# nubot-nudt/LCR-Net

Hardware: AMD Instinct MI355X
Metric: scans/s (120k-pt KITTI-shape scan -> 256-D descriptor) (higher is better)
Workload: dtype f32 (K-deep GEMMs, K >= 288 and N >= 64: fp32 operands as bf16 x 3 split, 6 of 9 products on the bf16 matrix cores, fp32 accumulate — error vs fp64 <= the fp32-MFMA kernel's; every other GEMM, KPConv and attention: fp32 MFMA); 1 GPU; configs[1]: batch of 8 synthetic 64-beam scans (~120k pts, 0.3 m voxel -> ~16k pts), voxelise + 3 subsamples + 10 radius searches + KPConv encoder + NetVLAD, seeded random weights; distinct_input_batches=4, streams=pre-processing stream (own host thread, 2 batches ahead) + 2 encoder stream(s), parallelism=scan-parallel x1, all-gather of descriptors

## Files before the change

include/lcr_hip.h:

```cpp
#ifndef LCR_HIP_H
#define LCR_HIP_H
#include <stddef.h>
#include <stdint.h>
#ifdef __cplusplus
extern "C" {
#endif

#define LCR_OK 0
#define LCR_EARG (-1)
#define LCR_ESPACE (-2)
#define LCR_EHIP (-3)

#define LCR_STATUS_KEY_OVERFLOW 1u
#define LCR_STATUS_LEN_MISMATCH 2u
#define LCR_GN_REPLICAS 8

const char* lcr_last_error(void);
void lcr_ktimer_enable(int on);
void lcr_ktimer_sample(int every);
void lcr_ktimer_kinds(unsigned mask);
int lcr_ktimer_read(int kind, int max_records, double* seconds, int64_t* meta);
int lcr_ktimer_read2(int kind, int max_records, double* seconds, double* seconds_kernel, int64_t* meta);
int lcr_stream_spin(int microseconds, void* stream);
int lcr_version(void);

int lcr_grid_subsample_ws_bytes(int64_t n_cap, int B, size_t* bytes);
int lcr_grid_subsample(const float* xyz, const int64_t* len, int B, int64_t n_cap, float voxel,
                       float* out_xyz, int64_t* out_len, uint32_t* status,
                       void* ws, size_t ws_bytes, void* stream);
int lcr_grid_subsample_ex(const float* xyz, const int64_t* len, int B, int64_t n_cap, float voxel, int key_bits_hint,
                          float* out_xyz, int64_t* out_len, uint32_t* status,
                          void* ws, size_t ws_bytes, void* stream);
int lcr_grid_subsample_rows(const float* xyz, int row_floats, const int64_t* len, int B, int64_t n_cap, float voxel, int key_bits_hint,
                            float* out_xyz, int64_t* out_len, uint32_t* status,
                            void* ws, size_t ws_bytes, void* stream);
int lcr_hashmap_order_host(const uint64_t* keys_host, int64_t n, int64_t* order_host);

int lcr_support_grid_ws_bytes(int64_t ns_cap, int B, size_t* bytes);
int lcr_support_grid_build(const float* s, const int64_t* slen, int B, int64_t ns_cap, float radius,
                           uint32_t* status, void* grid_ws, size_t grid_ws_bytes, void* stream);
int lcr_radius_query(const float* q, const int64_t* qlen, int B, int64_t nq_cap,
                     const void* grid_ws, int64_t ns_cap , float radius, int limit,
                     int64_t* out_idx64, int32_t* out_idx32, int32_t* out_cnt, void* stream);
int lcr_radius_query_ordered(const float* q, const int64_t* qlen, int B, int64_t nq_cap,
                             const void* grid_ws, int64_t ns_cap, float radius, int limit,
                             int64_t* out_idx64, int32_t* out_idx32, int32_t* out_cnt, const int32_t* q_order, void* stream);
typedef struct LcrRadiusQuery {
    const float*   q;
    const int64_t* qlen;
    int64_t        nq_cap;
    const void*    grid_ws;
    int64_t        ns_cap;
    float          radius;
    int            limit;
    int32_t*       out_idx32;
    const int32_t* q_order;
} LcrRadiusQuery;
#define LCR_RADIUS_QUERY_MULTI_MAX 12
int lcr_radius_query_multi(const LcrRadiusQuery* list, int n, int B, void* stream);
int lcr_support_grid_build_ex(const float* s, const int64_t* slen, int B, int64_t ns_cap, float radius,
                              uint32_t* status, void* grid_ws, size_t grid_ws_bytes, int32_t* order, void* stream);
int lcr_support_grid_order(const void* grid_ws, int64_t ns_cap, int B, int32_t* order, void* stream);
int lcr_radius_search_ws_bytes(int64_t nq_cap, int64_t ns_cap, int B, size_t* bytes);
int lcr_radius_search(const float* q, const float* s, const int64_t* qlen, const int64_t* slen, int B,
                      int64_t nq_cap, int64_t ns_cap, float radius, int limit,
                      int64_t* out_idx64, int32_t* out_idx32, int32_t* out_cnt, uint32_t* status,
                      void* ws, size_t ws_bytes, void* stream);

#define LCR_MAX_STAGES 8
typedef struct LcrPrecomputeLayout {
  int     num_stages, B, upsampling;
  int64_t n_raw;
  int     limits[LCR_MAX_STAGES];
  int64_t cap[LCR_MAX_STAGES];
  size_t  off_points[LCR_MAX_STAGES];
  size_t  off_lengths[LCR_MAX_STAGES];
  size_t  off_order[LCR_MAX_STAGES];
  size_t  off_neighbors[LCR_MAX_STAGES];
  size_t  off_subsampling[LCR_MAX_STAGES];
  size_t  off_upsampling[LCR_MAX_STAGES];
  size_t  out_bytes, ws_bytes;
} LcrPrecomputeLayout;
int lcr_precompute_layout(int64_t n0, int B, int num_stages, const int* limits, int upsampling, int64_t n_raw,
                          LcrPrecomputeLayout* layout);
int lcr_precompute_batch(const float* points0, const int64_t* lengths0, const LcrPrecomputeLayout* layout, float voxel_size,
                         float radius, float raw_voxel, int key_bits_hint, void* out, size_t out_bytes, void* ws, size_t ws_bytes,
                         int64_t* lengths_host, uint32_t* status_host, void* stream);
int lcr_precompute_batch_rows(const float* points0, int raw_row_floats, const int64_t* lengths0, const LcrPrecomputeLayout* layout,
                              float voxel_size, float radius, float raw_voxel, int key_bits_hint, void* out, size_t out_bytes, void* ws,
                              size_t ws_bytes, int64_t* lengths_host, uint32_t* status_host, void* stream);

int lcr_gemm_f32(const float* A, const float* B, float* C, int64_t M, int N, int K, int transA, int transB,
                 const float* bias, const float* rowdiv, const int64_t* seg_len, int S, int groups, double* stats,
                 void* stream);
int lcr_split_bf16x3(const float* w, int64_t n, uint16_t* planes, void* stream);
int lcr_split_bf16x3_tiles(const float* w, int N, int K, uint16_t* tiles, void* stream);
int lcr_gemm_f32_bsplit(const float* A, const uint16_t* Bs_tiles, float* C, int64_t M, int N, int K, const float* bias, const float* rowdiv,
                        const int64_t* seg_len, int S, int groups, double* stats, void* stream);
int lcr_gemm_f32_anorm(const float* A, const float* B, float* C, int64_t M, int N, int K, const float* bias,
                       const double* a_stats, const float* a_gamma, const float* a_beta, int a_groups, float a_eps,
                       float a_slope, const int64_t* seg_len, int S, int groups, double* stats, void* stream);
int lcr_gemm_f32_batched_ta(const float* A, const float* B, float* C, int64_t M, int N, int count, const int* k_host,
                            const int64_t* a_off_host, const int64_t* b_off_host, const int64_t* c_off_host, void* stream);
int lcr_kpconv_aggregate(const float* s_feats, const uint8_t* s_pos, const float* q_pts, const float* s_pts,
                         const void* idx, int idx_is_64, int64_t M, int64_t Ns, int H, int C,
                         const float* kernel_points_host, float sigma, float* A, float* nn,
                         const int32_t* order , void* stream);
#define LCR_KP_VALID_FIRST 1
int lcr_kpconv_aggregate_ex(const float* s_feats, const uint8_t* s_pos, const float* q_pts, const float* s_pts,
                            const void* idx, int idx_is_64, int64_t M, int64_t Ns, int H, int C,
                            const float* kernel_points_host, float sigma, float* A, float* nn,
                            const int32_t* order, int flags, void* stream);
int lcr_kpconv_fused(const float* s_feats, const uint8_t* s_pos, const float* q_pts, const float* s_pts, const void* idx,
                     int idx_is_64, int64_t M, int64_t Ns, int H, int C, const float* kernel_points_host, float sigma,
                     const float* W, const float* bias, float* out, const int64_t* seg_len, int S, int groups, double* stats,
                     const int32_t* order, void* stream);
int lcr_kpconv_cin1(const float* s_feats, const float* q_pts, const float* s_pts, const void* idx, int idx_is_64,
                    int64_t M, int64_t Ns, int H, const float* kernel_points_host, float sigma, const float* W,
                    const float* bias, int Cout, float* out, const int32_t* order, void* stream);
int lcr_maxpool(const float* x, const void* idx, int idx_is_64, int64_t M, int64_t Ns, int H, int C, float* out,
                const int32_t* order, void* stream);
int lcr_row_positive(const float* x, int64_t N, int C, uint8_t* pos, void* stream);
int lcr_groupnorm_stats(const float* x, int64_t N, int C, int groups, const int64_t* seg_len, int S, double* stats, void* stream);
int lcr_groupnorm_apply(const float* x, const double* stats, const float* gamma, const float* beta, const float* res,
                        const double* res_stats, const float* res_gamma, const float* res_beta, float* y, int64_t N, int C,
                        int groups, const int64_t* seg_len, int S, float eps, float slope, int act, uint8_t* pos, void* stream);

#define LCR_ENC_BLOCKS 10
typedef struct LcrUnaryW {
  const float *w, *b;
  const float *gn_w, *gn_b;
  const uint16_t* w_split;
} LcrUnaryW;
typedef struct LcrBlockW {
  int   cin, cout, strided;
  float sigma;
  const float* kernel_points_host;
  const float *kp_w, *kp_b;
  const float* kp_wt;
  const uint16_t* kp_wt_split;
  const float *normconv_w, *normconv_b;
  LcrUnaryW unary1, unary2, shortcut;
} LcrBlockW;
typedef struct LcrEncoderW {
  int   groups, c1_cout;
  float c1_sigma;
  const float* c1_kernel_points_host;
  const float *c1_w, *c1_b;
  const float *c1_gn_w, *c1_gn_b;
  LcrBlockW blocks[LCR_ENC_BLOCKS];
} LcrEncoderW;
int lcr_encoder_ws_bytes(const LcrEncoderW* W, const int64_t* n_host, int S, size_t* bytes);
int lcr_encoder_forward(const LcrEncoderW* W, const float* feats0, const float* const* points, const int32_t* const* neighbors,
                        const int32_t* const* subsampling, const int32_t* const* order, const int64_t* const* seg_len, int S,
                        const int64_t* n_host, const int64_t* seg_min_rows_host, const int* limits, float* const* out_feats, void* ws,
                        size_t ws_bytes, void* stream);
#define LCR_ENC_LISTS_VALID_FIRST 1u
int lcr_encoder_forward_ex(const LcrEncoderW* W, const float* feats0, const float* const* points, const int32_t* const* neighbors,
                           const int32_t* const* subsampling, const int32_t* const* order, const int64_t* const* seg_len, int S,
                           const int64_t* n_host, const int64_t* seg_min_rows_host, const int* limits, float* const* out_feats,
                           unsigned flags, void* ws, size_t ws_bytes, void* stream);

typedef struct LcrNetvladWeights {
  const float* cluster_weights;
  const float* cluster_weights2;
  const float* hidden1_weights;
  const float *bn1_w, *bn1_b, *bn1_mean, *bn1_var;
  const float *bn2_w, *bn2_b, *bn2_mean, *bn2_var;
  const float* gating_weights;
  const float *gbn_w, *gbn_b, *gbn_mean, *gbn_var;
} LcrNetvladWeights;
int lcr_netvlad_ws_bytes(int64_t n_rows, int S, size_t* bytes);
int lcr_netvlad_forward(const float* feats , const int64_t* seg_len_host, int S,
                        const LcrNetvladWeights* weights_host, float* out , void* ws, size_t ws_bytes, void* stream);

int lcr_rotary_embed(float* x, const float* theta, int64_t N, int heads, void* stream);
int lcr_attention_f32(const float* q, const float* k, const float* v, int64_t Nq, int64_t Nk, int heads, int head_dim,
                      float* out, void* stream);
int lcr_attention_seg_f32(const float* q, const float* k, const float* v, const int64_t* q_len_host, const int64_t* k_len_host, int P,
                          int heads, int head_dim, float* out, void* stream);
int lcr_attention_topk_f32(const float* q, const float* k, const float* v, const int64_t* q_len_host, const int64_t* k_len_host,
                           const int* kk_host, int P, int heads, int head_dim, float* out, void* stream);
int lcr_add_layernorm(const float* a, const float* b, const float* gamma, const float* beta, int64_t N, int D, float eps,
                      float* y, void* stream);
int lcr_relu_inplace(float* x, int64_t n, void* stream);

#define LCR_ROFORMER_MAX_BLOCKS 16
typedef struct LcrLinearW {
  const float *w, *b;
} LcrLinearW;
typedef struct LcrRoformerLayerW {
  LcrLinearW   q, k, v, lin;
  const float *ln1_w, *ln1_b;
  float        ln1_eps;
  LcrLinearW   expand, squeeze;
  const float *ln2_w, *ln2_b;
  float        ln2_eps;
} LcrRoformerLayerW;
typedef struct LcrRoformerW {
  int        d_in, d_model, d_out, heads, num_blocks;
  int        block_is_self[LCR_ROFORMER_MAX_BLOCKS];
  LcrLinearW emb1, emb2, in_proj, out_proj;
  LcrRoformerLayerW layers[LCR_ROFORMER_MAX_BLOCKS];
} LcrRoformerW;
int lcr_roformer_ws_bytes(const LcrRoformerW* W, int64_t n_rows, size_t* bytes);
int lcr_roformer_forward(const LcrRoformerW* W, const float* points, const float* feats, const int64_t* lens0_host, const int64_t* lens1_host,
                         int P, float* out, float* theta_out, void* ws, size_t ws_bytes, void* stream);

int lcr_retrieval_ws_bytes(int64_t Q, int64_t C, size_t* bytes);
int lcr_retrieval_topk(const float* queries , int64_t Q, int64_t q0, const float* database , int64_t C,
                       int D, int k, int exclude, int32_t* out_idx , float* out_d2 ,
                       void* ws, size_t ws_bytes, void* stream);

int lcr_gemm_f32_strided_batched(const float* A, const float* B, float* C, int64_t M, int N, int K, int transA, int transB,
                                 int64_t strideA, int64_t strideB, int64_t strideC, int count, void* stream);

int lcr_vote_shift(const float* xyz, const float* offsets, int64_t N, float max_range, float* out, void* stream);
int lcr_greedy_nms_ws_bytes(int64_t n_total, size_t* bytes);
int lcr_greedy_nms(const float* pts, const int64_t* len, int B, int64_t n_total, float radius, uint8_t* keep,
                   int64_t* out_len, void* ws, void* stream);
int lcr_neighbor_mean(const float* pts, const void* idx, int idx_is_64, int64_t M, int H, int64_t pad, float* out, void* stream);
int lcr_point_to_node_ws_bytes(int64_t N, int M, size_t* bytes);
int lcr_point_to_node_partition(const float* points, int64_t N, const float* nodes, int M, int K, int32_t* p2n, int64_t* knn,
                                uint8_t* knn_mask, uint8_t* node_mask, uint32_t* status, void* ws, size_t ws_bytes, void* stream);

int lcr_point_to_node_partition_stack(const float* points, const int64_t* point_off, const float* nodes, const int64_t* node_off, int C, int K,
                                      int32_t* p2n_out, int64_t* knn, uint8_t* knn_mask, uint8_t* node_mask, uint32_t* status, void* ws,
                                      size_t ws_bytes, void* stream);
int lcr_build_padded_scores(const float* raw, const uint8_t* row_mask, const uint8_t* col_mask, int64_t B, int M, int N,
                            float scale, const float* alpha, float inf_val, float* S, void* stream);
int lcr_log_sinkhorn(float* S, const uint8_t* row_mask, const uint8_t* col_mask, int64_t B, int M, int N, int iters,
                     float inf_val, float* uv_ws, void* stream);
int lcr_log_sinkhorn_ws_floats(int64_t B, int M, int N, size_t* floats);
int lcr_log_sinkhorn_form(int64_t B, int M, int N, int* form);
int lcr_log_sinkhorn_ex(float* S, const uint8_t* row_mask, const uint8_t* col_mask, int64_t B, int M, int N, int iters,
                        float inf_val, float* uv_ws, size_t uv_floats, void* stream);
int lcr_top1_matching_ws_bytes(int64_t B, int M, int N, size_t* bytes);
int lcr_top1_matching(const float* logS, int64_t B, int M, int N, const uint8_t* row_mask, const uint8_t* col_mask,
                      int64_t* total, int32_t* out_bij, float* out_score, void* ws, size_t ws_bytes, void* stream);
int lcr_top1_matching_ex(const float* logS, int64_t B, int M, int N, const uint8_t* row_mask, const uint8_t* col_mask, int mutual,
                         int64_t* total, int32_t* out_bij, float* out_score, void* ws, size_t ws_bytes, void* stream);
int lcr_patch_scores(const float* feats_a, int64_t Na, const float* feats_b, int64_t Nb, int C, const int64_t* idx_a, const int64_t* idx_b,
                     const uint8_t* mask_a, const uint8_t* mask_b, int64_t P, int K, float scale, const float* alpha, float inf_val, float* S,
                     void* stream);
int lcr_topk_matching_ws_bytes(int64_t B, int M, int N, size_t* bytes);
int lcr_topk_matching(const float* logS, int64_t B, int M, int N, const uint8_t* row_mask, const uint8_t* col_mask, int K, int mutual,
                      int64_t* total, int32_t* out_bij, float* out_score, void* ws, size_t ws_bytes, void* stream);
int lcr_topk_matching_ex(const float* logS, int64_t B, int M, int N, const uint8_t* row_mask, const uint8_t* col_mask, int K, int mutual,
                         int use_dustbin, float confidence_threshold, const float* global_scores, int64_t* total, int32_t* out_bij,
                         float* out_score, void* ws, size_t ws_bytes, void* stream);
int lcr_upsample_concat(const float* x, int64_t Nx, int C1, const void* idx, int idx_is_64, int H, const float* skip, int C2,
                        int64_t N, float* out, void* stream);
int lcr_gather_rows(const float* src, int64_t pad, int C, const int64_t* idx, int64_t R, float* out, void* stream);
int lcr_procrustes_batched(const float* src, const float* ref, const float* w, const int32_t* start, int P, float eps, float* T, void* stream);
int lcr_inlier_count(const float* T, int P, const float* src, const float* ref, int n, float radius, const int32_t* start,
                     int min_count, int32_t* counts, int32_t* best, void* stream);
int lcr_lgr_ws_bytes(int64_t n, int H, int S, size_t* bytes);
int lcr_local_global_registration(const float* src, const float* ref, const float* score, int64_t n, const int32_t* hyp_start, int H,
                                  const int32_t* seg_hyp_start, int S, float radius, int min_count, int steps, float* T_out,
                                  float* hyp_out, int32_t* counts_out, int32_t* best_out, void* ws, size_t ws_bytes, void* stream);
int lcr_local_global_registration_ex(const float* src, const float* ref, const float* score, int64_t n, const int32_t* hyp_start, int H,
                                     const int32_t* seg_hyp_start, int S, float radius, int min_count, int steps, int correspondence_limit,
                                     float* T_out, float* hyp_out, int32_t* counts_out, int32_t* best_out, void* ws, size_t ws_bytes,
                                     void* stream);
int lcr_inlier_weights(const float* T_all, const int32_t* sel, const float* src, const float* ref, const float* score, int n,
// ... 19 lines not shown
```

lcr-net_amd/_lib.py:

```python
import ctypes
import os

import torch

_PKG = os.path.dirname(os.path.abspath(__file__))
LIB_PATH = os.path.join(_PKG, "liblcr_hip.so")

_lib = None

c_f32p = ctypes.c_void_p
c_vp = ctypes.c_void_p
c_i64 = ctypes.c_int64
c_int = ctypes.c_int
c_float = ctypes.c_float
c_size_p = ctypes.POINTER(ctypes.c_size_t)
c_size_t = ctypes.c_size_t

_SIGS = {
    "lcr_last_error": (ctypes.c_char_p, []),
    "lcr_version": (c_int, []),
    "lcr_support_grid_ws_bytes": (c_int, [c_i64, c_int, c_size_p]),
    "lcr_support_grid_build": (c_int, [c_vp, c_vp, c_int, c_i64, c_float, c_vp, c_vp, ctypes.c_size_t, c_vp]),
    "lcr_precompute_layout": (c_int, [c_i64, c_int, c_int, c_vp, c_int, c_i64, c_vp]),
    "lcr_precompute_batch": (c_int, [c_vp, c_vp, c_vp, c_float, c_float, c_float, c_int, c_vp, c_size_t, c_vp, c_size_t, c_vp, c_vp, c_vp]),
    "lcr_precompute_batch_rows": (c_int, [c_vp, c_int, c_vp, c_vp, c_float, c_float, c_float, c_int, c_vp, c_size_t, c_vp, c_size_t, c_vp, c_vp, c_vp]),
    "lcr_radius_query_multi": (c_int, [c_vp, c_int, c_int, c_vp]),
    "lcr_radius_query": (c_int, [c_vp, c_vp, c_int, c_i64, c_vp, c_i64, c_float, c_int, c_vp, c_vp, c_vp, c_vp]),
    "lcr_stream_spin": (c_int, [c_int, c_vp]),
    "lcr_radius_query_ordered": (c_int, [c_vp, c_vp, c_int, c_i64, c_vp, c_i64, c_float, c_int, c_vp, c_vp, c_vp, c_vp, c_vp]),
    "lcr_radius_search_ws_bytes": (c_int, [c_i64, c_i64, c_int, c_size_p]),
    "lcr_radius_search": (c_int, [c_vp, c_vp, c_vp, c_vp, c_int, c_i64, c_i64, c_float, c_int, c_vp, c_vp, c_vp, c_vp,
                                  c_vp, ctypes.c_size_t, c_vp]),
    "lcr_grid_subsample_ws_bytes": (c_int, [c_i64, c_int, c_size_p]),
    "lcr_grid_subsample": (c_int, [c_vp, c_vp, c_int, c_i64, c_float, c_vp, c_vp, c_vp, c_vp, ctypes.c_size_t, c_vp]),
    "lcr_grid_subsample_ex": (c_int, [c_vp, c_vp, c_int, c_i64, c_float, c_int, c_vp, c_vp, c_vp, c_vp, ctypes.c_size_t, c_vp]),
    "lcr_grid_subsample_rows": (c_int, [c_vp, c_int, c_vp, c_int, c_i64, c_float, c_int, c_vp, c_vp, c_vp, c_vp, ctypes.c_size_t, c_vp]),
    "lcr_hashmap_order_host": (c_int, [c_vp, c_i64, c_vp]),
    "lcr_gemm_f32": (c_int, [c_vp, c_vp, c_vp, c_i64, c_int, c_int, c_int, c_int, c_vp, c_vp, c_vp, c_int, c_int, c_vp, c_vp]),
    "lcr_gemm_f32_anorm": (c_int, [c_vp, c_vp, c_vp, c_i64, c_int, c_int, c_vp, c_vp, c_vp, c_vp, c_int, c_float, c_float, c_vp, c_int,
                                   c_int, c_vp, c_vp]),
    "lcr_ktimer_enable": (None, [c_int]),
    "lcr_ktimer_sample": (None, [c_int]),
    "lcr_ktimer_kinds": (None, [ctypes.c_uint]),
    "lcr_ktimer_read": (c_int, [c_int, c_int, c_vp, c_vp]),
    "lcr_ktimer_read2": (c_int, [c_int, c_int, c_vp, c_vp, c_vp]),
    "lcr_encoder_ws_bytes": (c_int, [c_vp, c_vp, c_int, c_size_p]),
    "lcr_encoder_forward": (c_int, [c_vp, c_vp, c_vp, c_vp, c_vp, c_vp, c_vp, c_int, c_vp, c_vp, c_vp, c_vp, c_vp, c_size_t, c_vp]),
    "lcr_roformer_ws_bytes": (c_int, [c_vp, c_i64, c_size_p]),
    "lcr_roformer_forward": (c_int, [c_vp, c_vp, c_vp, c_vp, c_vp, c_int, c_vp, c_vp, c_vp, c_size_t, c_vp]),
    "lcr_encoder_forward_ex": (c_int, [c_vp, c_vp, c_vp, c_vp, c_vp, c_vp, c_vp, c_int, c_vp, c_vp, c_vp, c_vp, ctypes.c_uint, c_vp, c_size_t, c_vp]),
    "lcr_kpconv_aggregate": (c_int, [c_vp, c_vp, c_vp, c_vp, c_vp, c_int, c_i64, c_i64, c_int, c_int, c_vp, c_float, c_vp, c_vp, c_vp, c_vp]),
    "lcr_kpconv_fused": (c_int, [c_vp, c_vp, c_vp, c_vp, c_vp, c_int, c_i64, c_i64, c_int, c_int, c_vp, c_float, c_vp, c_vp, c_vp, c_vp, c_int,
                                 c_int, c_vp, c_vp, c_vp]),
    "lcr_kpconv_cin1": (c_int, [c_vp, c_vp, c_vp, c_vp, c_int, c_i64, c_i64, c_int, c_vp, c_float, c_vp, c_vp, c_int, c_vp, c_vp, c_vp]),
    "lcr_maxpool": (c_int, [c_vp, c_vp, c_int, c_i64, c_i64, c_int, c_int, c_vp, c_vp, c_vp]),
    "lcr_support_grid_order": (c_int, [c_vp, c_i64, c_int, c_vp, c_vp]),
    "lcr_row_positive": (c_int, [c_vp, c_i64, c_int, c_vp, c_vp]),
    "lcr_groupnorm_stats": (c_int, [c_vp, c_i64, c_int, c_int, c_vp, c_int, c_vp, c_vp]),
    "lcr_groupnorm_apply": (c_int, [c_vp, c_vp, c_vp, c_vp, c_vp, c_vp, c_vp, c_vp, c_vp, c_i64, c_int, c_int, c_vp, c_int,
                                    c_float, c_float, c_int, c_vp, c_vp]),
    "lcr_rotary_embed": (c_int, [c_vp, c_vp, c_i64, c_int, c_vp]),
    "lcr_attention_f32": (c_int, [c_vp, c_vp, c_vp, c_i64, c_i64, c_int, c_int, c_vp, c_vp]),
    "lcr_attention_seg_f32": (c_int, [c_vp, c_vp, c_vp, c_vp, c_vp, c_int, c_int, c_int, c_vp, c_vp]),
    "lcr_attention_topk_f32": (c_int, [c_vp, c_vp, c_vp, c_vp, c_vp, c_vp, c_int, c_int, c_int, c_vp, c_vp]),
    "lcr_add_layernorm": (c_int, [c_vp, c_vp, c_vp, c_vp, c_i64, c_int, c_float, c_vp, c_vp]),
    "lcr_relu_inplace": (c_int, [c_vp, c_i64, c_vp]),
    "lcr_retrieval_ws_bytes": (c_int, [c_i64, c_i64, c_size_p]),
    "lcr_retrieval_topk": (c_int, [c_vp, c_i64, c_i64, c_vp, c_i64, c_int, c_int, c_int, c_vp, c_vp, c_vp, ctypes.c_size_t, c_vp]),
    "lcr_gemm_f32_strided_batched": (c_int, [c_vp, c_vp, c_vp, c_i64, c_int, c_int, c_int, c_int, c_i64, c_i64, c_i64, c_int, c_vp]),
    "lcr_vote_shift": (c_int, [c_vp, c_vp, c_i64, c_float, c_vp, c_vp]),
    "lcr_greedy_nms_ws_bytes": (c_int, [c_i64, c_size_p]),
    "lcr_greedy_nms": (c_int, [c_vp, c_vp, c_int, c_i64, c_float, c_vp, c_vp, c_vp, c_vp]),
    "lcr_neighbor_mean": (c_int, [c_vp, c_vp, c_int, c_i64, c_int, c_i64, c_vp, c_vp]),
    "lcr_point_to_node_ws_bytes": (c_int, [c_i64, c_int, c_size_p]),
    "lcr_point_to_node_partition": (c_int, [c_vp, c_i64, c_vp, c_int, c_int, c_vp, c_vp, c_vp, c_vp, c_vp, c_vp, ctypes.c_size_t, c_vp]),
    "lcr_point_to_node_partition_stack": (c_int, [c_vp, c_vp, c_vp, c_vp, c_int, c_int, c_vp, c_vp, c_vp, c_vp, c_vp, c_vp, ctypes.c_size_t, c_vp]),
    "lcr_build_padded_scores": (c_int, [c_vp, c_vp, c_vp, c_i64, c_int, c_int, c_float, c_vp, c_float, c_vp, c_vp]),
    "lcr_log_sinkhorn": (c_int, [c_vp, c_vp, c_vp, c_i64, c_int, c_int, c_int, c_float, c_vp, c_vp]),
    "lcr_log_sinkhorn_ws_floats": (c_int, [c_i64, c_int, c_int, c_size_p]),
    "lcr_log_sinkhorn_form": (c_int, [c_i64, c_int, c_int, ctypes.POINTER(c_int)]),
    "lcr_split_bf16x3": (c_int, [c_vp, c_i64, c_vp, c_vp]),
    "lcr_split_bf16x3_tiles": (c_int, [c_vp, c_int, c_int, c_vp, c_vp]),
    "lcr_gemm_f32_bsplit": (c_int, [c_vp, c_vp, c_vp, c_i64, c_int, c_int, c_vp, c_vp, c_vp, c_int, c_int, c_vp, c_vp]),
    "lcr_log_sinkhorn_ex": (c_int, [c_vp, c_vp, c_vp, c_i64, c_int, c_int, c_int, c_float, c_vp, ctypes.c_size_t, c_vp]),
    "lcr_top1_matching_ws_bytes": (c_int, [c_i64, c_int, c_int, c_size_p]),
    "lcr_top1_matching": (c_int, [c_vp, c_i64, c_int, c_int, c_vp, c_vp, c_vp, c_vp, c_vp, c_vp, ctypes.c_size_t, c_vp]),
    "lcr_top1_matching_ex": (c_int, [c_vp, c_i64, c_int, c_int, c_vp, c_vp, c_int, c_vp, c_vp, c_vp, c_vp, ctypes.c_size_t, c_vp]),
    "lcr_topk_matching_ws_bytes": (c_int, [c_i64, c_int, c_int, c_size_p]),
    "lcr_topk_matching": (c_int, [c_vp, c_i64, c_int, c_int, c_vp, c_vp, c_int, c_int, c_vp, c_vp, c_vp, c_vp, ctypes.c_size_t, c_vp]),
    "lcr_patch_scores": (c_int, [c_vp, c_i64, c_vp, c_i64, c_int, c_vp, c_vp, c_vp, c_vp, c_i64, c_int, c_float, c_vp, c_float, c_vp, c_vp]),
    "lcr_topk_matching_ex": (c_int, [c_vp, c_i64, c_int, c_int, c_vp, c_vp, c_int, c_int, c_int, c_float, c_vp, c_vp, c_vp, c_vp, c_vp, ctypes.c_size_t,
                                     c_vp]),
    "lcr_local_global_registration_ex": (c_int, [c_vp, c_vp, c_vp, c_i64, c_vp, c_int, c_vp, c_int, c_float, c_int, c_int, c_int, c_vp, c_vp, c_vp, c_vp,
                                                 c_vp, ctypes.c_size_t, c_vp]),
    "lcr_upsample_concat": (c_int, [c_vp, c_i64, c_int, c_vp, c_int, c_int, c_vp, c_int, c_i64, c_vp, c_vp]),
    "lcr_gather_rows": (c_int, [c_vp, c_i64, c_int, c_vp, c_i64, c_vp, c_vp]),
    "lcr_procrustes_batched": (c_int, [c_vp, c_vp, c_vp, c_vp, c_int, c_float, c_vp, c_vp]),
    "lcr_inlier_count": (c_int, [c_vp, c_int, c_vp, c_vp, c_int, c_float, c_vp, c_int, c_vp, c_vp, c_vp]),
    "lcr_inlier_weights": (c_int, [c_vp, c_vp, c_vp, c_vp, c_vp, c_int, c_float, c_vp, c_vp]),
    "lcr_lgr_ws_bytes": (c_int, [c_i64, c_int, c_int, c_size_p]),
    "lcr_local_global_registration": (c_int, [c_vp, c_vp, c_vp, c_i64, c_vp, c_int, c_vp, c_int, c_float, c_int, c_int, c_vp, c_vp, c_vp, c_vp, c_vp,
                                              ctypes.c_size_t, c_vp]),
    "lcr_netvlad_ws_bytes": (c_int, [c_i64, c_int, c_size_p]),
    "lcr_netvlad_forward": (c_int, [c_vp, c_vp, c_int, c_vp, c_vp, c_vp, ctypes.c_size_t, c_vp]),
    "lcr_ransac_ws_bytes": (c_int, [c_int, c_int, c_size_p]),
    "lcr_ransac_correspondences": (c_int, [c_vp, c_vp, c_vp, c_int, c_float, c_int, c_int, ctypes.c_uint64, c_vp, c_vp, c_vp, c_vp, c_vp, c_vp, c_vp,
                                           c_vp, ctypes.c_size_t, c_vp]),
    "lcr_ransac_sample_host": (c_int, [ctypes.c_uint64, c_i64, c_i64, c_int, c_i64, c_vp]),
    "lcr_icp_ws_bytes": (c_int, [c_int, c_i64, c_i64, c_size_p]),
    "lcr_icp_point_to_point": (c_int, [c_vp, c_vp, c_vp, c_vp, c_int, c_vp, c_float, c_int, ctypes.c_double, ctypes.c_double, c_vp, c_vp, c_vp, c_vp,
                                       c_vp, c_vp, c_vp, c_vp, c_int, c_vp, ctypes.c_size_t, c_vp]),
}


_RELEASES_GIL = {"lcr_roformer_forward", "lcr_precompute_batch", "lcr_precompute_batch_rows", "lcr_encoder_forward", "lcr_encoder_forward_ex", "lcr_ktimer_read",
                 "lcr_ktimer_read2", "lcr_hashmap_order_host", "lcr_ransac_sample_host", "lcr_icp_point_to_point", "lcr_netvlad_forward", "lcr_log_sinkhorn", "lcr_log_sinkhorn_ex",
                 "lcr_local_global_registration", "lcr_local_global_registration_ex", "lcr_retrieval_topk", "lcr_stream_spin"}


def build():
    import importlib.util
    spec = importlib.util.spec_from_file_location("_lcr_build", os.path.join(_PKG, "csrc", "build.py"))
    mod = importlib.util.module_from_spec(spec)
    spec.loader.exec_module(mod)
    return mod.build()


def lib():
    global _lib
    if _lib is None:
        if not os.path.exists(LIB_PATH):
            raise RuntimeError(
                "liblcr_hip.so not found at %s — build it with `python lcr-net_amd/csrc/build.py` "
                "(there is no CPU fallback for the lcr-net_amd hot path)" % LIB_PATH)
        L = ctypes.CDLL(LIB_PATH)
        for name, (res, args) in _SIGS.items():
            if not hasattr(L, name):
                continue
            fn = getattr(L, name)
            fn.restype = res
            fn.argtypes = args
        if os.environ.get("LCR_CTYPES_KEEP_GIL", "1") != "0":
            K = ctypes.PyDLL(LIB_PATH)
            for name, (res, args) in _SIGS.items():
                if name in _RELEASES_GIL or not hasattr(K, name):
                    continue
                fn = getattr(K, name)
                fn.restype = res
                fn.argtypes = args
                setattr(L, name, fn)
        _lib = L
    return _lib


def check(rc, what):
    if rc != 0:
        msg = lib().lcr_last_error()
        raise RuntimeError("%s failed (rc=%d): %s" % (what, rc, msg.decode() if msg else ""))


def ptr(t):
    return ctypes.c_void_p(t.data_ptr()) if t is not None else ctypes.c_void_p(0)


def stream_ptr(device=None):
    idx = device.index if isinstance(device, torch.device) else None
    if idx is None:
        idx = torch.cuda.current_device() if not isinstance(device, int) else device
    return ctypes.c_void_p(torch._C._cuda_getCurrentRawStream(idx))


def require_cuda(*tensors):
    for t in tensors:
        if t is not None and not t.is_cuda:
            raise RuntimeError("lcr-net_amd ops run on the GPU only: got a %s tensor (no CPU fallback)" % t.device)


def workspace(nbytes, device):
    return torch.empty(max(int(nbytes), 256), dtype=torch.uint8, device=device)
```

lcr-net_amd/csrc/encoder.hip:

```cpp
#include <algorithm>
#include <cstdlib>
#include <cstring>

#include "common.h"

#define TURN(call) ([&]() { LaunchTurn turn_; return (call); }())

namespace lcr {

constexpr float ENC_GN_EPS = 1e-5f;
constexpr float ENC_SLOPE = 0.1f;

struct Arena {
  char*  base;
  size_t off, cap;
  template <typename T>
  T* take(size_t n) {
    const size_t o = off;
    off = align_up(off + n * sizeof(T));
    return (base && off <= cap) ? reinterpret_cast<T*>(base + o) : nullptr;
  }
};

struct StageIO {
  const float*   pts;
  const int64_t* seg;
  const int32_t* order;
  int64_t        n;
  int64_t        min_rows;
};

struct StatsPool {
  double* base;
  size_t  off, cap;
  int     S, groups;
  double* take() {
    const size_t n = static_cast<size_t>(GN_REPLICAS) * S * groups * 2;
    if (off + n > cap) return nullptr;
    double* p = base + off;
    off += n;
    return p;
  }
};

static size_t stats_doubles(int S, int groups) { return static_cast<size_t>(GN_REPLICAS) * S * groups * 2 * 44; }

static int unary_raw(const LcrUnaryW& u, const float* x, int64_t n, int cin, int cout, const StageIO& st, StatsPool& sp, Arena& ws,
                     float** y_out, double** stats_out, hipStream_t s) {
  float* y = ws.take<float>(static_cast<size_t>(n) * cout);
  double* stats = sp.take();
  if (!y || !stats) return LCR_ESPACE;
  const bool split = u.w_split && cin >= 288 && cin % 32 == 0 && cout >= 64;
  int rc = split ? TURN(lcr_gemm_f32_bsplit(x, u.w_split, y, n, cout, cin, u.b, nullptr, st.seg, sp.S, sp.groups, stats, s))
                 : TURN(lcr_gemm_f32(x, u.w, y, n, cout, cin, 0, 1, u.b, nullptr, st.seg, sp.S, sp.groups, stats, s));
  *y_out = y;
  *stats_out = stats;
  return rc;
}

static int residual_block(const LcrBlockW& b, const float* s_feats, const StageIO& q, const StageIO& sup, const void* idx, int H,
                          StatsPool& sp, Arena& ws, float* out, unsigned enc_flags, hipStream_t s) {
  const int mid = b.cout / 4, g = sp.groups;
  const int64_t M = q.n, Ns = sup.n;
  int rc;
  const float* x = s_feats;
  uint8_t* pos = ws.take<uint8_t>(static_cast<size_t>(Ns));
  if (!pos) return LCR_ESPACE;
  if (b.unary1.w) {
    float* y1;
    double* st1;
    if ((rc = unary_raw(b.unary1, s_feats, Ns, b.cin, mid, sup, sp, ws, &y1, &st1, s))) return rc;
    float* x1 = ws.take<float>(static_cast<size_t>(Ns) * mid);
    if (!x1) return LCR_ESPACE;
    if ((rc = TURN(lcr_groupnorm_apply(y1, st1, b.unary1.gn_w, b.unary1.gn_b, nullptr, nullptr, nullptr, nullptr, x1, Ns, mid, g, sup.seg, sp.S,
                                  ENC_GN_EPS, ENC_SLOPE, 1, pos, s))))
      return rc;
    x = x1;
  } else if ((rc = TURN(lcr_row_positive(s_feats, Ns, b.cin, pos, s)))) {
    return rc;
  }
  float* A = ws.take<float>(static_cast<size_t>(M) * 15 * mid);
  float* nn = ws.take<float>(static_cast<size_t>(M));
  float* kpo = ws.take<float>(static_cast<size_t>(M) * mid);
  double* stc = sp.take();
  if (!A || !nn || !kpo || !stc) return LCR_ESPACE;
  static const bool vf_env_off = getenv("LCR_KP_VALID_FIRST") && atoi(getenv("LCR_KP_VALID_FIRST")) == 0;
  const int vf_flag = ((enc_flags & LCR_ENC_LISTS_VALID_FIRST) && !vf_env_off) ? LCR_KP_VALID_FIRST : 0;
  static const bool fused32 = getenv("LCR_KPCONV_FUSED") != nullptr;
  if (fused32 && mid == 32 && sp.S <= 64) {
    if ((rc = TURN(lcr_kpconv_fused(x, pos, q.pts, sup.pts, idx, 0, M, Ns, H, mid, b.kernel_points_host, b.sigma, b.kp_w, b.kp_b, kpo, q.seg, sp.S, g,
                                    stc, q.order, s))))
      return rc;
  } else {
    if ((rc = TURN(lcr_kpconv_aggregate_ex(x, pos, q.pts, sup.pts, idx, 0, M, Ns, H, mid, b.kernel_points_host, b.sigma, A, nn, q.order, vf_flag, s)))) return rc;
    if (b.kp_wt_split && mid >= 64) {
      if ((rc = TURN(lcr_gemm_f32_bsplit(A, b.kp_wt_split, kpo, M, mid, 15 * mid, b.kp_b, nn, q.seg, sp.S, g, stc, s)))) return rc;
    } else if ((rc = TURN(b.kp_wt ? lcr_gemm_f32(A, b.kp_wt, kpo, M, mid, 15 * mid, 0, 1, b.kp_b, nn, q.seg, sp.S, g, stc, s)
                                  : lcr_gemm_f32(A, b.kp_w, kpo, M, mid, 15 * mid, 0, 0, b.kp_b, nn, q.seg, sp.S, g, stc, s)))) return rc;
  }
  float* y;
  double* sty;
  static const bool no_anorm = getenv("LCR_NO_NORM_ON_LOAD") != nullptr;
  if (!no_anorm && mid <= 256 && mid % 4 == 0 && b.cout > 32 && q.min_rows >= 64) {
    y = ws.take<float>(static_cast<size_t>(M) * b.cout);
    sty = sp.take();
    if (!y || !sty) return LCR_ESPACE;
    if ((rc = TURN(lcr_gemm_f32_anorm(kpo, b.unary2.w, y, M, b.cout, mid, b.unary2.b, stc, b.normconv_w, b.normconv_b, g, ENC_GN_EPS, ENC_SLOPE,
                                      q.seg, sp.S, g, sty, s))))
      return rc;
  } else {
    float* x2 = ws.take<float>(static_cast<size_t>(M) * mid);
    if (!x2) return LCR_ESPACE;
    if ((rc = TURN(lcr_groupnorm_apply(kpo, stc, b.normconv_w, b.normconv_b, nullptr, nullptr, nullptr, nullptr, x2, M, mid, g, q.seg, sp.S, ENC_GN_EPS,
                                  ENC_SLOPE, 1, nullptr, s))))
      return rc;
    if ((rc = unary_raw(b.unary2, x2, M, mid, b.cout, q, sp, ws, &y, &sty, s))) return rc;
  }
  const float* res = s_feats;
  if (b.strided) {
    float* pooled = ws.take<float>(static_cast<size_t>(M) * b.cin);
    if (!pooled) return LCR_ESPACE;
    if ((rc = TURN(lcr_maxpool(s_feats, idx, 0, M, Ns, H, b.cin, pooled, q.order, s)))) return rc;
    res = pooled;
  }
  const double* str = nullptr;
  if (b.shortcut.w) {
    float* r;
    double* st;
    if ((rc = unary_raw(b.shortcut, res, M, b.cin, b.cout, q, sp, ws, &r, &st, s))) return rc;
    res = r;
    str = st;
  }
  return TURN(lcr_groupnorm_apply(y, sty, b.unary2.gn_w, b.unary2.gn_b, res, str, str ? b.shortcut.gn_w : nullptr, str ? b.shortcut.gn_b : nullptr, out,
                             M, b.cout, g, q.seg, sp.S, ENC_GN_EPS, ENC_SLOPE, 1, nullptr, s));
}

static size_t block_ws_bytes(const LcrBlockW& b, int64_t M, int64_t Ns) {
  Arena a{nullptr, 0, ~size_t(0)};
  const int mid = b.cout / 4;
  a.take<uint8_t>(Ns);
  a.take<float>(static_cast<size_t>(Ns) * mid);
  a.take<float>(static_cast<size_t>(Ns) * mid);
  a.take<float>(static_cast<size_t>(M) * 15 * mid);
  a.take<float>(M);
  a.take<float>(static_cast<size_t>(M) * mid);
  a.take<float>(static_cast<size_t>(M) * mid);
  a.take<float>(static_cast<size_t>(M) * b.cout);
  a.take<float>(static_cast<size_t>(M) * b.cin);
  a.take<float>(static_cast<size_t>(M) * b.cout);
  return a.off;
}

static const int BLOCK_Q[LCR_ENC_BLOCKS] = {0, 1, 1, 1, 2, 2, 2, 3, 3, 3};
static const int BLOCK_S[LCR_ENC_BLOCKS] = {0, 0, 1, 1, 1, 2, 2, 2, 3, 3};

}

using namespace lcr;

extern "C" int lcr_encoder_ws_bytes(const LcrEncoderW* W, const int64_t* n_host, int S, size_t* bytes) {
  if (!W || !n_host || !bytes || S < 1) return LCR_EARG;
  size_t blk = 0, pp = 0;
  for (int i = 0; i < LCR_ENC_BLOCKS; ++i) {
    blk = std::max(blk, block_ws_bytes(W->blocks[i], n_host[BLOCK_Q[i]], n_host[BLOCK_S[i]]));
    pp = std::max(pp, align_up(sizeof(float) * static_cast<size_t>(n_host[BLOCK_Q[i]]) * W->blocks[i].cout));
  }
  pp = std::max(pp, align_up(sizeof(float) * static_cast<size_t>(n_host[0]) * W->c1_cout * 2));
  *bytes = blk + 2 * pp + align_up(sizeof(double) * stats_doubles(S, W->groups)) + 4096;
  return LCR_OK;
}

extern "C" int lcr_encoder_forward(const LcrEncoderW* W, const float* feats0, const float* const* points, const int32_t* const* neighbors,
                                   const int32_t* const* subsampling, const int32_t* const* order, const int64_t* const* seg_len, int S,
                                   const int64_t* n_host, const int64_t* seg_min_rows_host, const int* limits, float* const* out_feats,
                                   void* ws, size_t ws_bytes, void* stream) {
  return lcr_encoder_forward_ex(W, feats0, points, neighbors, subsampling, order, seg_len, S, n_host, seg_min_rows_host, limits, out_feats, 0u, ws,
                                ws_bytes, stream);
}

extern "C" int lcr_encoder_forward_ex(const LcrEncoderW* W, const float* feats0, const float* const* points, const int32_t* const* neighbors,
                                      const int32_t* const* subsampling, const int32_t* const* order, const int64_t* const* seg_len, int S,
                                      const int64_t* n_host, const int64_t* seg_min_rows_host, const int* limits, float* const* out_feats,
                                      unsigned flags, void* ws, size_t ws_bytes, void* stream) {
  if (!W || !feats0 || !points || !neighbors || !subsampling || !seg_len || !n_host || !limits || !out_feats || !ws || S < 1) {
    set_error("lcr_encoder_forward: bad argument");
    return LCR_EARG;
  }
  size_t need = 0;
  lcr_encoder_ws_bytes(W, n_host, S, &need);
  if (ws_bytes < need) {
    set_error("lcr_encoder_forward: workspace too small (%zu < %zu)", ws_bytes, need);
    return LCR_ESPACE;
  }
  hipStream_t s = static_cast<hipStream_t>(stream);
  StageIO st[4];
  for (int i = 0; i < 4; ++i) st[i] = StageIO{points[i], seg_len[i], order ? order[i] : nullptr, n_host[i], seg_min_rows_host ? seg_min_rows_host[i] : 0};
  Arena top{static_cast<char*>(ws), 0, ws_bytes};
  StatsPool sp{top.take<double>(stats_doubles(S, W->groups)), 0, stats_doubles(S, W->groups), S, W->groups};
  size_t pp = 0;
  for (int i = 0; i < LCR_ENC_BLOCKS; ++i) pp = std::max(pp, sizeof(float) * static_cast<size_t>(n_host[BLOCK_Q[i]]) * W->blocks[i].cout);
  pp = std::max(pp, sizeof(float) * static_cast<size_t>(n_host[0]) * W->c1_cout * 2);
  float* ping = reinterpret_cast<float*>(top.take<char>(pp));
  float* pong = reinterpret_cast<float*>(top.take<char>(pp));
  const size_t scratch0 = top.off;
  if (!sp.base || !ping || !pong) return LCR_ESPACE;
  hipMemsetAsync(sp.base, 0, sizeof(double) * sp.cap, s);

  int rc;
  float* cur;
  {
    const int64_t n0 = n_host[0];
    float* raw = ping;
    float* f = ping + static_cast<size_t>(n0) * W->c1_cout;
    double* stt = sp.take();
    if ((rc = TURN(lcr_kpconv_cin1(feats0, st[0].pts, st[0].pts, neighbors[0], 0, n0, n0, limits[0], W->c1_kernel_points_host, W->c1_sigma, W->c1_w,
                              W->c1_b, W->c1_cout, raw, st[0].order, s))))
      return rc;
    if ((rc = TURN(lcr_groupnorm_stats(raw, n0, W->c1_cout, W->groups, st[0].seg, S, stt, s)))) return rc;
    if ((rc = TURN(lcr_groupnorm_apply(raw, stt, W->c1_gn_w, W->c1_gn_b, nullptr, nullptr, nullptr, nullptr, f, n0, W->c1_cout, W->groups, st[0].seg, S,
                                  ENC_GN_EPS, ENC_SLOPE, 1, nullptr, s))))
      return rc;
    cur = f;
  }
  static const int STAGE_LAST[4] = {0, 3, 6, 9};
  for (int i = 0; i < LCR_ENC_BLOCKS; ++i) {
    const int qs = BLOCK_Q[i], ss = BLOCK_S[i];
    const bool strided = qs != ss;
    const void* idx = strided ? static_cast<const void*>(subsampling[ss]) : static_cast<const void*>(neighbors[qs]);
    const int H = limits[ss];
    float* out = nullptr;
    for (int k = 0; k < 4; ++k)
      if (STAGE_LAST[k] == i) out = out_feats[k];
    if (!out) out = (cur >= ping && cur < ping + pp / sizeof(float)) ? pong : ping;
    Arena scratch{static_cast<char*>(ws), scratch0, ws_bytes};
    if ((rc = residual_block(W->blocks[i], cur, st[qs], st[ss], idx, H, sp, scratch, out, flags, s))) {
      if (rc == LCR_ESPACE) set_error("lcr_encoder_forward: block %d ran out of workspace", i);
      return rc;
    }
    cur = out;
  }
  return check_launch("lcr_encoder_forward");
}
```

lcr-net_amd/csrc/gemm_f32.hip:

```cpp
#include <cstdio>
#include <cstdlib>
#include <map>
#include <mutex>
#include <type_traits>

#include "common.h"

namespace lcr {

typedef float floatx16 __attribute__((ext_vector_type(16)));

constexpr int GM_BK = 32;
constexpr int GM_T = 256;

constexpr int GM_MAX_BATCH = 64;
struct GemmBatch {
  int     count;
  int     strided;
  int     k[GM_MAX_BATCH];
  int64_t a_off[GM_MAX_BATCH], b_off[GM_MAX_BATCH], c_off[GM_MAX_BATCH];
};

struct GemmEpilogue {
  const float*   bias;
// ... 411 lines not shown
    lb_t[0].store(Bs[0]);
  } else {
    sstore(0, 0);
  }
  __syncthreads();
  const int half = lane >> 5;
  const int a_off = ARM ? (wm * 32 + (lane & 31)) * LDR + half * 16 : half * (NEWP ? 16 : 1) * LDA + wm * 32 + (lane & 31);
  const int b_off = BRM ? (wn * (32 * NT) + (lane & 31)) * LDR + half * 16 : half * (NEWP ? 16 : 1) * LDB + wn * (32 * NT) + (lane & 31);
  auto fetch4_a = [&](const float* as, int q, float (&o)[4]) {
    if (ARM) {
      const float4 v = *reinterpret_cast<const float4*>(as + 4 * q);
      o[0] = v.x, o[1] = v.y, o[2] = v.z, o[3] = v.w;
    } else {
#pragma unroll
      for (int i = 0; i < 4; ++i) o[i] = as[(4 * q + i) * LDA];
    }
  };
  auto fetch4_b = [&](const float* bs, int q, float (&o)[4]) {
    if (BRM) {
      const float4 v = *reinterpret_cast<const float4*>(bs + 4 * q);
      o[0] = v.x, o[1] = v.y, o[2] = v.z, o[3] = v.w;
    } else {
#pragma unroll
      for (int i = 0; i < 4; ++i) o[i] = bs[(4 * q + i) * LDB];
    }
  };
  if constexpr (SHORT) {
    constexpr int KKS = GM_BK / 2, PFS = 4;
    for (int t = 0; t < nk; ++t) {
      if (t > 0) {
        gload(k_begin + t * GM_BK, 0);
        __syncthreads();
        if constexpr (ANORM) {
          sstore_a0();
          lb_t[0].store(Bs[0]);
        } else {
          sstore(0, 0);
        }
        __syncthreads();
      }
      const float* as = As[0] + a_off;
      const float* bs = Bs[0] + b_off;
      static_assert(NEWP, "the light form is only instantiated for single-accumulator tiles");
      float af[2][4], bf[2][4];
      fetch4_a(as, 0, af[0]);
      fetch4_b(bs, 0, bf[0]);
      fetch4_a(as, 1, af[1]);
      fetch4_b(bs, 1, bf[1]);
#pragma unroll
      for (int q = 0; q < KKS / 4; ++q) {
#pragma unroll
        for (int i = 0; i < 4; ++i) acc[0] = __builtin_amdgcn_mfma_f32_32x32x2f32(af[q & 1][i], bf[q & 1][i], acc[0], 0, 0, 0);
        if (q + 2 < KKS / 4) {
          fetch4_a(as, q + 2, af[q & 1]);
          fetch4_b(bs, q + 2, bf[q & 1]);
        }
      }
    }
  } else {
  constexpr int KK = GM_BK / 2;
  constexpr int PF = NT == 1 ? KK : (NT == 2 ? 8 : 4);
  constexpr int PA = BM * 8 / GM_T, PB = BN * 8 / GM_T;
  constexpr int ST0 = KK - (PA + PB) - 1 > 2 ? (KK - (PA + PB)) / 2 : 1;
  auto step = [&](auto buf_c, auto full_c, int t) {
    constexpr int BUF = decltype(buf_c)::value;
    constexpr bool FULL = decltype(full_c)::value;
    if (FULL || t + 2 < nk) gload(k_begin + (t + 2) * GM_BK, BUF);
    const bool do_store = FULL || t + 1 < nk;
    const float* as = As[BUF] + a_off;
    const float* bs = Bs[BUF] + b_off;
    float af[PF], bf[PF][NT];
    if constexpr (NEWP) {
#pragma unroll
      for (int q = 0; q < KK / 4; ++q) {
        float a4[4], b4[4];
        fetch4_a(as, q, a4);
        fetch4_b(bs, q, b4);
#pragma unroll
        for (int i = 0; i < 4; ++i) {
          af[4 * q + i] = a4[i];
          bf[4 * q + i][0] = b4[i];
        }
      }
    } else {
#pragma unroll
      for (int d = 0; d < PF; ++d) {
        af[d] = as[d * 2 * LDA];
#pragma unroll
        for (int j = 0; j < NT; ++j) bf[d][j] = bs[d * 2 * LDB + j * 32];
      }
    }
    __builtin_amdgcn_sched_barrier(0);
#pragma unroll
    for (int kk = 0; kk < KK; ++kk) {
      const int sl = kk % PF;
#pragma unroll
      for (int j = 0; j < NT; ++j) {
        if (NACC == 2 && (kk & 1)) acc2[j] = __builtin_amdgcn_mfma_f32_32x32x2f32(af[sl], bf[sl][j], acc2[j], 0, 0, 0);
        else acc[j] = __builtin_amdgcn_mfma_f32_32x32x2f32(af[sl], bf[sl][j], acc[j], 0, 0, 0);
      }
      if (kk + PF < KK) {
        af[sl] = as[(kk + PF) * 2 * LDA];
#pragma unroll
        for (int j = 0; j < NT; ++j) bf[sl][j] = bs[(kk + PF) * 2 * LDB + j * 32];
      }
      const int piece = kk - ST0;
      if (do_store && piece >= 0 && piece < PA + PB) {
        if (piece < PA) {
          if (TA) la_n[1 - BUF].store_piece(As[1 - BUF], piece);
          else la_t[1 - BUF].store_piece(As[1 - BUF], piece);
        } else {
          if (TB) lb_t[1 - BUF].store_piece(Bs[1 - BUF], piece - PA);
          else lb_n[1 - BUF].store_piece(Bs[1 - BUF], piece - PA);
        }
      }
    }
    __syncthreads();
  };
  int t = 0;
  for (; t + 3 < nk; t += 2) {
    step(std::integral_constant<int, 0>{}, std::true_type{}, t);
    step(std::integral_constant<int, 1>{}, std::true_type{}, t + 1);
  }
  for (; t < nk; t += 2) {
    step(std::integral_constant<int, 0>{}, std::false_type{}, t);
    if (t + 1 >= nk) break;
    step(std::integral_constant<int, 1>{}, std::false_type{}, t + 1);
  }

  }

  if (NACC == 2) {
#pragma unroll
    for (int j = 0; j < NT; ++j)
#pragma unroll
      for (int r = 0; r < 16; ++r) acc[j][r] += acc2[j][r];
  }

  gemm_epilogue<BM, BN, WM, WN, NT>(acc, C, M, N, m0, n0, m_tile, ep, bias_v, blk_first, blk_seg_start, blk_seg_end, wm, wn, lane);
}

template <int N_OUTSTANDING>
__device__ __forceinline__ void wait_vmcnt() {
  asm volatile("s_waitcnt vmcnt(%0)" ::"n"(N_OUTSTANDING) : "memory");
}
__device__ __forceinline__ void glds16(const float* base, unsigned off, unsigned lds_dst) {
  unsigned keep;
  asm volatile("s_mov_b32 %0, m0\n\ts_mov_b32 m0, %3\n\ts_nop 0\n\tglobal_load_lds_dwordx4 %1, %2\n\ts_mov_b32 m0, %0"
               : "=&s"(keep)
               : "v"(off), "s"(base), "s"(lds_dst)
               : "memory");
}

template <int BM, int BN, int WM, int WN>
__global__ __launch_bounds__(GM_T, (BM == 64 ? 3 : 2)) void k_gemm_f32_deep(const float* __restrict__ A, const float* __restrict__ B, float* __restrict__ C,
                                                            int64_t M, int N, int K, GemmEpilogue ep) {
  static_assert(WM * WN == 4 && BM == 32 * WM && BN == 32 * WN, "one 32x32 accumulator per wavefront");
  constexpr int LA = BM / 32, LB = BN / 32, LPW = LA + LB;
  constexpr int STAGE_A = BM * 128, STAGE = (BM + BN) * 128;
  constexpr int NS = 3;
  __shared__ __attribute__((aligned(1024))) char lds[NS * STAGE];
  const int lane = threadIdx.x & 63, w = __builtin_amdgcn_readfirstlane(threadIdx.x >> 6);
  const int wm = w / WN, wn = w % WN;
  const int ntn = (N + BN - 1) / BN;
  const int xcd = blockIdx.x & 7, slot = blockIdx.x >> 3;
  const int64_t m_tile = static_cast<int64_t>(slot / ntn) * 8 + xcd;
  const int64_t m0 = m_tile * BM;
  const int n0 = (slot % ntn) * BN;
  if (m0 >= M) return;
  const unsigned lds_base = static_cast<unsigned>(reinterpret_cast<uintptr_t>(lds));

  unsigned oa[LA], ob[LB];
#pragma unroll
  for (int j = 0; j < LA; ++j) {
    const int row = (w * LA + j) * 8 + (lane >> 3);
    const int c = (lane & 7) ^ ((row >> 1) & 7);
    int64_t gr = m0 + row;
    gr = gr < M ? gr : M - 1;
    oa[j] = static_cast<unsigned>((gr * K + c * 4) * 4);
  }
#pragma unroll
  for (int j = 0; j < LB; ++j) {
    const int row = (w * LB + j) * 8 + (lane >> 3);
    const int c = (lane & 7) ^ ((row >> 1) & 7);
    int gr = n0 + row;
    gr = gr < N ? gr : N - 1;
    ob[j] = static_cast<unsigned>((static_cast<int64_t>(gr) * K + c * 4) * 4);
  }
  const unsigned dst_a = lds_base + w * LA * 1024, dst_b = lds_base + STAGE_A + w * LB * 1024;
  const float* Ak = A;
  const float* Bk = B;
  auto issue_one = [&](int stage, int j) {
    if (j < LA) glds16(Ak, oa[j], dst_a + stage * STAGE + j * 1024);
    else glds16(Bk, ob[j - LA], dst_b + stage * STAGE + (j - LA) * 1024);
  };
  auto advance = [&] {
    Ak += GM_BK;
    Bk += GM_BK;
  };
  auto issue = [&](int stage) {
#pragma unroll
    for (int j = 0; j < LPW; ++j) issue_one(stage, j);
    advance();
  };

  const int half = lane >> 5;
  const int ra = wm * 32 + (lane & 31), rb = wn * 32 + (lane & 31);
  int offa[4], offb[4];
#pragma unroll
  for (int q = 0; q < 4; ++q) {
    offa[q] = ra * 128 + (((4 * half + q) ^ ((ra >> 1) & 7)) << 4);
    offb[q] = STAGE_A + rb * 128 + (((4 * half + q) ^ ((rb >> 1) & 7)) << 4);
  }
  float4 fa[4], fb[4];
  floatx16 acc;
#pragma unroll
  for (int r = 0; r < 16; ++r) acc[r] = 0.f;
  const int nk = K / GM_BK;

  issue(0);
  if (nk > 1) issue(1);
  if (nk > 2) issue(2);
  float bias_v[1];
  {
    const int col = n0 + wn * 32 + (lane & 31);
    bias_v[0] = (ep.bias && col < N) ? ep.bias[col] : 0.f;
  }
  int blk_first = 0;
  int64_t blk_seg_start = 0, blk_seg_end = 0;
  if (ep.stats != nullptr) {
    blk_seg_end = ep.seg_len[0];
    while (blk_first + 1 < ep.S && m0 >= blk_seg_end) {
      ++blk_first;
      blk_seg_start = blk_seg_end;
      blk_seg_end += ep.seg_len[blk_first];
    }
  }
  if (nk > 2) wait_vmcnt<2 * LPW>();
  else if (nk > 1) wait_vmcnt<LPW>();
  else wait_vmcnt<0>();
  __syncthreads();
#pragma unroll
  for (int q = 0; q < 4; ++q) {
    fa[q] = *reinterpret_cast<const float4*>(lds + offa[q]);
    fb[q] = *reinterpret_cast<const float4*>(lds + offb[q]);
  }

  auto mfma = [&](float a, float b) { acc = __builtin_amdgcn_mfma_f32_32x32x2f32(a, b, acc, 0, 0, 0); };
  auto mfma4 = [&](const float4& a, const float4& b) {
    mfma(a.x, b.x);
    mfma(a.y, b.y);
    mfma(a.z, b.z);
    mfma(a.w, b.w);
  };
  auto pin = [] { __builtin_amdgcn_sched_barrier(0); };
  auto step = [&](auto st_c, auto full_c, int t) {
    constexpr int ST = decltype(st_c)::value;
    constexpr bool FULL = decltype(full_c)::value;
    constexpr int NXT = (ST + 1) % NS;
    float4 na[4], nb[4];
    mfma4(fa[0], fb[0]);
    const bool more = FULL || t + 1 < nk;
    const bool load = FULL || t + 3 < nk;
    pin();
    if (more) {
      if (FULL || t + 2 < nk) wait_vmcnt<LPW>();
      else wait_vmcnt<0>();
      __syncthreads();
    }
    const float a1[4] = {fa[1].x, fa[1].y, fa[1].z, fa[1].w}, b1[4] = {fb[1].x, fb[1].y, fb[1].z, fb[1].w};
    const float a2[4] = {fa[2].x, fa[2].y, fa[2].z, fa[2].w}, b2[4] = {fb[2].x, fb[2].y, fb[2].z, fb[2].w};
#pragma unroll
    for (int q = 0; q < 4; ++q) {
      if (more) {
        na[q] = *reinterpret_cast<const float4*>(lds + NXT * STAGE + offa[q]);
        nb[q] = *reinterpret_cast<const float4*>(lds + NXT * STAGE + offb[q]);
      }
      pin();
      mfma(a1[q], b1[q]);
      pin();
    }
#pragma unroll
    for (int q = 0; q < 4; ++q) {
      if (more && load) {
#pragma unroll
        for (int j = q; j < LPW; j += 4) issue_one(ST, j);
      }
      pin();
      mfma(a2[q], b2[q]);
      pin();
    }
    if (more && load) advance();
    mfma4(fa[3], fb[3]);
    if (more) {
#pragma unroll
      for (int q = 0; q < 4; ++q) fa[q] = na[q], fb[q] = nb[q];
    }
  };
  using I0 = std::integral_constant<int, 0>;
  using I1 = std::integral_constant<int, 1>;
  using I2 = std::integral_constant<int, 2>;
  int t = 0;
  for (; t + 6 <= nk; t += 3) {
    step(I0{}, std::true_type{}, t);
    step(I1{}, std::true_type{}, t + 1);
    step(I2{}, std::true_type{}, t + 2);
  }
  for (; t < nk; t += 3) {
    step(I0{}, std::false_type{}, t);
    if (t + 1 < nk) step(I1{}, std::false_type{}, t + 1);
    if (t + 2 < nk) step(I2{}, std::false_type{}, t + 2);
  }

  floatx16 accs[1] = {acc};
  gemm_epilogue<BM, BN, WM, WN, 1>(accs, C, M, N, m0, n0, m_tile, ep, bias_v, blk_first, blk_seg_start, blk_seg_end, wm, wn, lane);
}

template <int BM, int BN, int WM, int WN>
static int launch_gemm_deep(const float* A, const float* B, float* C, int64_t M, int N, int K, const GemmEpilogue& ep, hipStream_t st) {
  const int mt8 = (div_up(M, BM) + 7) / 8 * 8;
  LCR_LAUNCH_TIMED((k_gemm_f32_deep<BM, BN, WM, WN>), dim3(mt8 * div_up(N, BN)), dim3(GM_T), 0, st, A, B, C, M, N, K, ep);
  return check_launch("lcr_gemm_f32");
}

typedef __bf16 bf16x8_t __attribute__((ext_vector_type(8)));
typedef __bf16 bf16x2_t __attribute__((ext_vector_type(2)));
typedef float f32x2_t __attribute__((ext_vector_type(2)));
typedef float f32x4_t __attribute__((ext_vector_type(4)));
typedef uint32_t u32x4_t __attribute__((ext_vector_type(4)));

__device__ __forceinline__ uint32_t pk_bf16(float a, float b) {
  f32x2_t v = {a, b};
  return __builtin_bit_cast(uint32_t, __builtin_convertvector(v, bf16x2_t));
}
__device__ __forceinline__ void split2(float x0, float x1, uint32_t& h1, uint32_t& h2, uint32_t& h3) {
  h1 = pk_bf16(x0, x1);
  const float r0 = fsub(x0, __uint_as_float(h1 << 16)), r1 = fsub(x1, __uint_as_float(h1 & 0xffff0000u));
  h2 = pk_bf16(r0, r1);
  const float s0 = fsub(r0, __uint_as_float(h2 << 16)), s1 = fsub(r1, __uint_as_float(h2 & 0xffff0000u));
  h3 = pk_bf16(s0, s1);
}

__global__ __launch_bounds__(256) void k_split_bf16x3(const float* __restrict__ w, int64_t n, uint16_t* __restrict__ planes) {
  for (int64_t i = (blockIdx.x * static_cast<int64_t>(blockDim.x) + threadIdx.x) * 2; i < n; i += static_cast<int64_t>(gridDim.x) * blockDim.x * 2) {
    const float x0 = w[i], x1 = i + 1 < n ? w[i + 1] : 0.f;
    uint32_t h1, h2, h3;
    split2(x0, x1, h1, h2, h3);
    planes[i] = static_cast<uint16_t>(h1), planes[n + i] = static_cast<uint16_t>(h2), planes[2 * n + i] = static_cast<uint16_t>(h3);
    if (i + 1 < n) planes[i + 1] = static_cast<uint16_t>(h1 >> 16), planes[n + i + 1] = static_cast<uint16_t>(h2 >> 16), planes[2 * n + i + 1] = static_cast<uint16_t>(h3 >> 16);
  }
}

__global__ __launch_bounds__(256) void k_split_bf16x3_tiles(const float* __restrict__ w, int N, int K, uint16_t* __restrict__ tiles) {
  const int KS = K / GM_BK;
  const int64_t blk = blockIdx.x;
  const int ct = static_cast<int>(blk / KS), ks = static_cast<int>(blk % KS);
  const int row = threadIdx.x >> 2, kc = threadIdx.x & 3;
  const int n = ct * 64 + row;
  u32x4_t p1 = {0u, 0u, 0u, 0u}, p2 = p1, p3 = p1;
  if (n < N) {
    const float* src = w + static_cast<int64_t>(n) * K + ks * GM_BK + kc * 8;
    const float4 x0 = ld4(src), x1 = ld4(src + 4);
    uint32_t h1, h2, h3;
    split2(x0.x, x0.y, h1, h2, h3), p1.x = h1, p2.x = h2, p3.x = h3;
    split2(x0.z, x0.w, h1, h2, h3), p1.y = h1, p2.y = h2, p3.y = h3;
    split2(x1.x, x1.y, h1, h2, h3), p1.z = h1, p2.z = h2, p3.z = h3;
    split2(x1.z, x1.w, h1, h2, h3), p1.w = h1, p2.w = h2, p3.w = h3;
  }
  char* dst = reinterpret_cast<char*>(tiles) + blk * 12288 + row * 64 + ((kc ^ ((row >> 2) & 3)) << 4);
  *reinterpret_cast<u32x4_t*>(dst) = p1;
  *reinterpret_cast<u32x4_t*>(dst + 4096) = p2;
  *reinterpret_cast<u32x4_t*>(dst + 8192) = p3;
}

template <int ABL, int NWM, int D = 2>
__global__ __launch_bounds__(128 * NWM, 2) void k_gemm_f32_bsplit_p(const float* __restrict__ A, const uint16_t* __restrict__ Bs, float* __restrict__ C,
                                                             int64_t M, int N, int K, GemmEpilogue ep) {
  constexpr int BM = 32 * NWM, BN = 64, RS = 64, T = 128 * NWM, PLA = BM * RS, STGA = 3 * PLA, PL = 64 * RS;
  constexpr int NPB = (768 + T - 1) / T;
  constexpr int STG = 3 * PL + (NPB * T - 768) * 16;
  __shared__ __attribute__((aligned(16))) char sA[2 * STGA];
  __shared__ __attribute__((aligned(16))) char sB[2 * STG];
  const int lane = threadIdx.x & 63, w = __builtin_amdgcn_readfirstlane(threadIdx.x >> 6);
  const int wm = w >> 1, wn = w & 1;
  const int ntn = (N + BN - 1) / BN;
  const int xcd = blockIdx.x & 7, slot = blockIdx.x >> 3;
  const int64_t m_tile = static_cast<int64_t>(slot / ntn) * 8 + xcd;
  const int64_t m0 = m_tile * BM;
  const int n0 = (slot % ntn) * BN;
  if (m0 >= M) return;
  const int srow = threadIdx.x >> 3, spc = threadIdx.x & 7;
  const float* ap[2];
  int soff[2];
#pragma unroll
  for (int j = 0; j < 2; ++j) {
    const int r = srow + j * (T / 8);
    int64_t ga = m0 + r;
    ga = ga < M ? ga : M - 1;
    ap[j] = A + ga * K + spc * 4;
    soff[j] = r * RS + (((spc >> 1) ^ ((r >> 2) & 3)) << 4) + (spc & 1) * 8;
  }
  const char* bp = reinterpret_cast<const char*>(Bs) + static_cast<int64_t>(n0 / 64) * (K / GM_BK) * 12288;
  int bsrc[NPB], bdst[NPB];
#pragma unroll
  for (int j = 0; j < NPB; ++j) {
    const int q = threadIdx.x + T * j;
    bsrc[j] = (q < 768 ? q : threadIdx.x) * 16;
    bdst[j] = q * 16;
  }
  const int fsw = ((lane & 31) >> 2) & 3, fc0 = ((lane >> 5) ^ fsw) << 4, fc1 = (((lane >> 5) + 2) ^ fsw) << 4;
  const int fa = (wm * 32 + (lane & 31)) * RS, fb = (wn * 32 + (lane & 31)) * RS;
  floatx16 acc, acc2;
#pragma unroll
  for (int r = 0; r < 16; ++r) acc[r] = 0.f, acc2[r] = 0.f;
  const int nk = K / GM_BK;
  f32x4_t ra[D][2];
  u32x4_t rb[D][NPB];
  auto fetch = [&](auto st_c, int t) {
    constexpr int st = decltype(st_c)::value;
    const int tt = t < nk ? t : nk - 1;
    ra[st][0] = *reinterpret_cast<const f32x4_t*>(ap[0] + tt * GM_BK), ra[st][1] = *reinterpret_cast<const f32x4_t*>(ap[1] + tt * GM_BK);
#pragma unroll
    for (int j = 0; j < NPB; ++j) rb[st][j] = *reinterpret_cast<const u32x4_t*>(bp + static_cast<int64_t>(tt) * 12288 + bsrc[j]);
  };
  auto park = [&](auto st_c, int lds_stage) {
    constexpr int st = decltype(st_c)::value;
    char* da = sA + lds_stage * STGA;
    char* db = sB + lds_stage * STG;
#pragma unroll
    for (int j = 0; j < 2; ++j) {
      uint32_t h1, h2, h3, g1, g2, g3;
      if constexpr (ABL & 2) {
        h1 = __float_as_uint(ra[st][j].x), h2 = __float_as_uint(ra[st][j].y), h3 = h1, g1 = __float_as_uint(ra[st][j].z), g2 = __float_as_uint(ra[st][j].w), g3 = g1;
      } else {
        split2(ra[st][j].x, ra[st][j].y, h1, h2, h3);
        split2(ra[st][j].z, ra[st][j].w, g1, g2, g3);
      }
      if constexpr (ABL & 4) {
        asm volatile("" ::"v"(h1), "v"(h2), "v"(h3), "v"(g1), "v"(g2), "v"(g3));
      } else {
        *reinterpret_cast<uint2*>(da + soff[j]) = make_uint2(h1, g1);
        *reinterpret_cast<uint2*>(da + PLA + soff[j]) = make_uint2(h2, g2);
        *reinterpret_cast<uint2*>(da + 2 * PLA + soff[j]) = make_uint2(h3, g3);
      }
    }
#pragma unroll
    for (int j = 0; j < NPB; ++j) {
      const u32x4_t v = rb[st][j];
      if constexpr (ABL & 4) {
        asm volatile("" ::"v"(v));
      } else {
        *reinterpret_cast<u32x4_t*>(db + bdst[j]) = v;
      }
    }
  };
  using I0 = std::integral_constant<int, 0>;
  fetch(I0{}, 0);
  if constexpr (D > 1) fetch(std::integral_constant<int, 1 % D>{}, 1);
  if constexpr (D > 2) fetch(std::integral_constant<int, 2 % D>{}, 2);
  if constexpr (D > 3) fetch(std::integral_constant<int, 3 % D>{}, 3);
  float bias_v[1];
  {
    const int col = n0 + wn * 32 + (lane & 31);
    bias_v[0] = (ep.bias && col < N) ? ep.bias[col] : 0.f;
  }
  int blk_first = 0;
  int64_t blk_seg_start = 0, blk_seg_end = 0;
  if (ep.stats != nullptr) {
    blk_seg_end = ep.seg_len[0];
    while (blk_first + 1 < ep.S && m0 >= blk_seg_end) {
      ++blk_first;
      blk_seg_start = blk_seg_end;
      blk_seg_end += ep.seg_len[blk_first];
    }
  }
  park(I0{}, 0);
  fetch(I0{}, D);
  __syncthreads();
  auto step = [&](auto lds_c, auto reg_c, int t) {
    constexpr int P = decltype(lds_c)::value;
    using NX = std::integral_constant<int, (decltype(reg_c)::value + 1) % D>;
    const char* la = sA + P * STGA + fa;
    const char* lb = sB + P * STG + fb;
    bf16x8_t a0[3], b0[3], a1[3], b1[3];
    auto mm = [&](const bf16x8_t& x, const bf16x8_t& y, floatx16& c) {
      if constexpr (ABL & 1) {
        asm volatile("" ::"v"(x), "v"(y));
      } else {
        c = __builtin_amdgcn_mfma_f32_32x32x16_bf16(x, y, c, 0, 0, 0);
      }
    };
    if constexpr (ABL & 16) {
      u32x4_t z = {static_cast<uint32_t>(t), 0u, 0u, 0u};
      asm volatile("" : "+v"(z));
#pragma unroll
      for (int p = 0; p < 3; ++p) a0[p] = b0[p] = a1[p] = b1[p] = __builtin_bit_cast(bf16x8_t, z);
      (void)la, (void)lb;
    } else {
#pragma unroll
      for (int p = 0; p < 3; ++p) {
        a0[p] = __builtin_bit_cast(bf16x8_t, *reinterpret_cast<const u32x4_t*>(la + p * PLA + fc0));
        b0[p] = __builtin_bit_cast(bf16x8_t, *reinterpret_cast<const u32x4_t*>(lb + p * PL + fc0));
      }
#pragma unroll
      for (int p = 0; p < 3; ++p) {
        a1[p] = __builtin_bit_cast(bf16x8_t, *reinterpret_cast<const u32x4_t*>(la + p * PLA + fc1));
        b1[p] = __builtin_bit_cast(bf16x8_t, *reinterpret_cast<const u32x4_t*>(lb + p * PL + fc1));
      }
    }
    mm(a0[2], b0[0], acc);
    mm(a0[0], b0[2], acc2);
    mm(a0[1], b0[1], acc);
    mm(a0[1], b0[0], acc2);
    mm(a0[0], b0[1], acc);
    mm(a0[0], b0[0], acc2);
    park(NX{}, P ^ 1);
    mm(a1[2], b1[0], acc);
    mm(a1[0], b1[2], acc2);
    mm(a1[1], b1[1], acc);
    mm(a1[1], b1[0], acc2);
    mm(a1[0], b1[1], acc);
    mm(a1[0], b1[0], acc2);
    if constexpr (!(ABL & 8)) fetch(NX{}, t + 1 + D);
    __syncthreads();
  };
  static_assert(D == 2 || D == 4, "register stages");
  using I1 = std::integral_constant<int, 1>;
  using I2 = std::integral_constant<int, 2>;
  using I3 = std::integral_constant<int, 3>;
  int t = 0;
  if constexpr (D == 2) {
    for (; t + 2 <= nk; t += 2) {
      step(I0{}, I0{}, t);
      step(I1{}, I1{}, t + 1);
    }
    if (t < nk) step(I0{}, I0{}, t);
  } else {
    for (; t + 4 <= nk; t += 4) {
      step(I0{}, I0{}, t);
      step(I1{}, I1{}, t + 1);
      step(I0{}, I2{}, t + 2);
      step(I1{}, I3{}, t + 3);
    }
    if (t < nk) step(I0{}, I0{}, t);
    if (t + 1 < nk) step(I1{}, I1{}, t + 1);
    if (t + 2 < nk) step(I0{}, I2{}, t + 2);
  }
#pragma unroll
  for (int r = 0; r < 16; ++r) acc[r] += acc2[r];
  floatx16 accs[1] = {acc};
  gemm_epilogue<BM, BN, NWM, 2, 1>(accs, C, M, N, m0, n0, m_tile, ep, bias_v, blk_first, blk_seg_start, blk_seg_end, wm, wn, lane);
}

struct GemmStreamK {
  float*    partial;
  uint32_t* arrived;
  int       U;
};

template <int BM, int BN, int WM, int WN>
__global__ __launch_bounds__(GM_T, 3) void k_gemm_f32_sk(const float* __restrict__ A, const float* __restrict__ B, float* __restrict__ C,
                                                         int64_t M, int N, int K, GemmEpilogue ep, GemmStreamK sk) {
  static_assert(WM * WN == 4 && BM == 32 * WM, "one 32-row MFMA tile per wavefront along M");
  constexpr int LDA = BM + 1, LDB = BN + 4;
  constexpr int NT = BN / (32 * WN);
  __shared__ __attribute__((aligned(16))) float As[2][GM_BK * LDA];
  __shared__ __attribute__((aligned(16))) float Bs[2][GM_BK * LDB];
  const int lane = threadIdx.x & 63, w = __builtin_amdgcn_readfirstlane(threadIdx.x >> 6);
  const int wm = w / WN, wn = w % WN;
  const int ntn = (N + BN - 1) / BN;
  const int64_t mt = (M + BM - 1) / BM;
  const int xcd = blockIdx.x & 7, u = blockIdx.x >> 3;
  const int64_t mt_x = mt > xcd ? (mt - xcd + 7) / 8 : 0;
  const int nk = (K + GM_BK - 1) / GM_BK;
// ... 194 lines not shown

static int launch_gemm_sk(const float* A, const float* B, float* C, int64_t M, int N, int K, const GemmEpilogue& ep, hipStream_t st) {
  const int cus = sk_cu_count();
  const int64_t iters = static_cast<int64_t>(div_up(M, 64)) * div_up(N, 64) * div_up(K, GM_BK);
  int per_cu = 3;
  while (per_cu > 1 && iters / (static_cast<int64_t>(cus) * per_cu) < 24) --per_cu;
  if (getenv("LCR_SK_PER_CU")) per_cu = atoi(getenv("LCR_SK_PER_CU"));
  int U = cus * per_cu / 8;
  if (U < 1) U = 1;
  if (8 * U > SK_MAX_GRID) U = SK_MAX_GRID / 8;
  int dev = 0;
  hipGetDevice(&dev);
  GemmStreamK sk;
  {
    std::lock_guard<std::mutex> lk(g_sk_mu);
    SkScratch& sc = g_sk_scratch[{dev, st}];
    if (!sc.partial) {
      if (hipMalloc(reinterpret_cast<void**>(&sc.partial), sizeof(float) * 2 * 16 * GM_T * SK_MAX_GRID) != hipSuccess ||
          hipMalloc(reinterpret_cast<void**>(&sc.arrived), sizeof(uint32_t) * SK_MAX_TILES) != hipSuccess) {
        set_error("lcr_gemm_f32: cannot allocate the stream-K scratch");
        return LCR_EHIP;
      }
      hipMemsetAsync(sc.arrived, 0, sizeof(uint32_t) * SK_MAX_TILES, st);
    }
    sk.partial = sc.partial;
    sk.arrived = sc.arrived;
    sk.U = U;
  }
  LCR_LAUNCH_TIMED((k_gemm_f32_sk<64, 64, 2, 2>), dim3(8 * U), dim3(GM_T), 0, st, A, B, C, M, N, K, ep, sk);
  return check_launch("lcr_gemm_f32");
}

}

using namespace lcr;

static int g_force_tile = 0;
extern "C" void lcr_gemm_debug_force_tile(int t) { g_force_tile = t; }
static int g_force_streamk = -1;
static int g_force_deep = -1;
extern "C" void lcr_gemm_debug_deep(int mode) { g_force_deep = mode; }
extern "C" void lcr_gemm_debug_streamk(int mode) { g_force_streamk = mode; }

static int gemm_impl(const float* A, const float* B, float* C, int64_t M, int N, int K, int transA, int transB, const float* bias,
                     const float* rowdiv, const int64_t* seg_len, int S, int groups, double* stats, void* stream);

extern "C" int lcr_gemm_f32_anorm(const float* A, const float* B, float* C, int64_t M, int N, int K, const float* bias,
                                  const double* a_stats, const float* a_gamma, const float* a_beta, int a_groups, float a_eps,
                                  float a_slope, const int64_t* seg_len, int S, int groups, double* stats, void* stream) {
  if (!A || !B || !C || M < 0 || N <= 32 || K <= 0 || K > AN_KMAX || K % 4 != 0 || !a_stats || !a_gamma || !a_beta || a_groups < 1 ||
      K % a_groups != 0 || a_groups > 64 || !seg_len || S < 1 || reinterpret_cast<uintptr_t>(A) % 16 != 0 || reinterpret_cast<uintptr_t>(B) % 16 != 0) {
    set_error("lcr_gemm_f32_anorm: needs 32 < N, K <= 256, K % 4 == 0, a_groups dividing K, a segment table and 16-byte aligned operands");
    return LCR_EARG;
  }
  if (stats) {
    const int gs = groups >= 1 && N % groups == 0 ? N / groups : 3;
    if ((gs & (gs - 1)) != 0) {
      set_error("lcr_gemm_f32_anorm: statistics need groups dividing N into power-of-two sized groups");
      return LCR_EARG;
    }
  }
  hipStream_t st = static_cast<hipStream_t>(stream);
  KernelTimerScope timed(KT_GEMM, st, M, N, K);
  if (M == 0) return LCR_OK;
  GemmEpilogue ep{bias, nullptr, seg_len, S, groups, stats};
  ANorm an{a_stats, a_gamma, a_beta, a_groups, a_eps, a_slope};
  const int mt8 = (div_up(M, 64) + 7) / 8 * 8;
  LCR_LAUNCH_TIMED((k_gemm_f32<64, 64, 2, 2, false, true, true, true, true>), dim3(mt8 * div_up(N, 64)), dim3(GM_T), 0, st, A, B, C, M,
                     N, K, ep, GemmBatch{}, an);
  return check_launch("lcr_gemm_f32_anorm");
}

extern "C" int lcr_gemm_f32(const float* A, const float* B, float* C, int64_t M, int N, int K, int transA, int transB, const float* bias,
                            const float* rowdiv, const int64_t* seg_len, int S, int groups, double* stats, void* stream) {
  return gemm_impl(A, B, C, M, N, K, transA, transB, bias, rowdiv, seg_len, S, groups, stats, stream);
}

static int gemm_impl(const float* A, const float* B, float* C, int64_t M, int N, int K, int transA, int transB, const float* bias,
                     const float* rowdiv, const int64_t* seg_len, int S, int groups, double* stats, void* stream) {
  if (!A || !B || !C || M < 0 || N <= 0 || K <= 0) {
    set_error("lcr_gemm_f32: bad argument");
    return LCR_EARG;
  }
  if (stats && (!seg_len || S < 1 || groups < 1 || N % groups != 0)) {
    set_error("lcr_gemm_f32: statistics need seg_len, S >= 1 and groups dividing N");
    return LCR_EARG;
  }
  if (stats) {
    const int gs = N / groups;
    if ((gs & (gs - 1)) != 0) {
      set_error("lcr_gemm_f32: channels per group must be a power of two");
      return LCR_EARG;
    }
  }
  hipStream_t st = static_cast<hipStream_t>(stream);
  KernelTimerScope timed(KT_GEMM, st, M, N, K);
  if (M == 0) return LCR_OK;
  GemmEpilogue ep{bias, rowdiv, seg_len, S, groups, stats};
  const int64_t lda = transA ? M : K, ldb = transB ? K : N;
  const bool vec = (lda % 4 == 0) && (ldb % 4 == 0) && (reinterpret_cast<uintptr_t>(A) % 16 == 0) && (reinterpret_cast<uintptr_t>(B) % 16 == 0);
  if (!vec) return launch_gemm<128, 64, 4, 1, false>(A, B, C, M, N, K, transA, transB, ep, st);
  switch (g_force_tile) {
    case 1: return launch_gemm<128, 128, 4, 1, true>(A, B, C, M, N, K, transA, transB, ep, st);
    case 2: return launch_gemm<128, 64, 4, 1, true>(A, B, C, M, N, K, transA, transB, ep, st);
    case 3: return launch_gemm<128, 32, 4, 1, true>(A, B, C, M, N, K, transA, transB, ep, st);
    case 4: return launch_gemm<64, 64, 2, 2, true>(A, B, C, M, N, K, transA, transB, ep, st);
    case 5: return launch_gemm<64, 128, 2, 2, true>(A, B, C, M, N, K, transA, transB, ep, st);
    default: break;
  }
  const int64_t b128 = (M + 127) / 128, nb128 = (N + 127) / 128;
  static const bool no_short = getenv("LCR_GEMM_NO_SHORT") != nullptr;
  static const int short_k = getenv("LCR_GEMM_SHORT_K") ? atoi(getenv("LCR_GEMM_SHORT_K")) : 256;
  static const int deep_env = getenv("LCR_GEMM_DEEP") ? atoi(getenv("LCR_GEMM_DEEP")) : 1;
  const int deep_mode = g_force_deep >= 0 ? g_force_deep : deep_env;
  const bool deep_ok = !transA && transB && K % GM_BK == 0 && !g_force_tile && M * K < (int64_t(1) << 30) && static_cast<int64_t>(N) * K < (int64_t(1) << 30);
  auto deep = [&] {
    if (N <= 32) return launch_gemm_deep<128, 32, 4, 1>(A, B, C, M, N, K, ep, st);
    return launch_gemm_deep<64, 64, 2, 2>(A, B, C, M, N, K, ep, st);
  };
  if (deep_mode == 2 && deep_ok) return deep();
  if (!no_short && K <= short_k && !transA) {
    if (N <= 32) return launch_gemm<128, 32, 4, 1, true, true>(A, B, C, M, N, K, transA, transB, ep, st);
    return launch_gemm<64, 64, 2, 2, true, true>(A, B, C, M, N, K, transA, transB, ep, st);
  }
  if (deep_mode && deep_ok) return deep();
  if (N <= 32) return launch_gemm<128, 32, 4, 1, true>(A, B, C, M, N, K, transA, transB, ep, st);
  static const int sk_env = getenv("LCR_GEMM_STREAMK") ? atoi(getenv("LCR_GEMM_STREAMK")) : 0;
  const int sk_mode = g_force_streamk >= 0 ? g_force_streamk : sk_env;
  const bool sk_legal = !transA && !transB && K >= 64 && static_cast<int64_t>(div_up(M, 64)) * div_up(N, 64) <= SK_MAX_TILES;
  if (sk_mode && sk_legal && (sk_mode == 2 || sk_worth(M, N, K))) return launch_gemm_sk(A, B, C, M, N, K, ep, st);
  if (K >= 512 && b128 * nb128 >= 512) return launch_gemm<128, 128, 4, 1, true>(A, B, C, M, N, K, transA, transB, ep, st);
  return launch_gemm<64, 64, 2, 2, true>(A, B, C, M, N, K, transA, transB, ep, st);
}

extern "C" int lcr_split_bf16x3(const float* w, int64_t n, uint16_t* planes, void* stream) {
  if (!w || !planes || n < 0) {
    set_error("lcr_split_bf16x3: bad argument");
    return LCR_EARG;
  }
  if (n == 0) return LCR_OK;
  hipLaunchKernelGGL(k_split_bf16x3, dim3(min(div_up(n, 512), 2048)), dim3(256), 0, static_cast<hipStream_t>(stream), w, n, planes);
  return check_launch("lcr_split_bf16x3");
}

extern "C" int lcr_split_bf16x3_tiles(const float* w, int N, int K, uint16_t* tiles, void* stream) {
  if (!w || !tiles || N < 1 || K < GM_BK || K % GM_BK != 0 || reinterpret_cast<uintptr_t>(w) % 16 != 0 || reinterpret_cast<uintptr_t>(tiles) % 16 != 0) {
    set_error("lcr_split_bf16x3_tiles: needs K %% 32 == 0 and 16-byte aligned buffers");
    return LCR_EARG;
  }
  hipLaunchKernelGGL(k_split_bf16x3_tiles, dim3(div_up(N, 64) * (K / GM_BK)), dim3(256), 0, static_cast<hipStream_t>(stream), w, N, K, tiles);
  return check_launch("lcr_split_bf16x3_tiles");
}

extern "C" int lcr_gemm_f32_bsplit(const float* A, const uint16_t* Bs, float* C, int64_t M, int N, int K, const float* bias, const float* rowdiv,
                                   const int64_t* seg_len, int S, int groups, double* stats, void* stream) {
  if (!A || !Bs || !C || M < 0 || N <= 0 || K <= 0 || K % GM_BK != 0 || reinterpret_cast<uintptr_t>(A) % 16 != 0 || reinterpret_cast<uintptr_t>(Bs) % 16 != 0 ||
      K < GM_BK) {
    set_error("lcr_gemm_f32_bsplit: needs K %% 32 == 0 and 16-byte aligned operands");
    return LCR_EARG;
  }
  if (stats && (!seg_len || S < 1 || groups < 1 || N % groups != 0 || ((N / groups) & (N / groups - 1)) != 0)) {
    set_error("lcr_gemm_f32_bsplit: statistics need seg_len, S >= 1 and groups dividing N into power-of-two sized groups");
    return LCR_EARG;
  }
  hipStream_t st = static_cast<hipStream_t>(stream);
  KernelTimerScope timed(KT_GEMM, st, M, N, K);
  if (M == 0) return LCR_OK;
  GemmEpilogue ep{bias, rowdiv, seg_len, S, groups, stats};
  const int mt8 = (div_up(M, 64) + 7) / 8 * 8;
  static const int abl = getenv("LCR_SPLIT_ABL") ? atoi(getenv("LCR_SPLIT_ABL")) : 0;
  const dim3 grid(mt8 * div_up(N, 64)), block(256);
  switch (abl) {
    case 1: LCR_LAUNCH_TIMED((k_gemm_f32_bsplit_p<1, 2>), grid, block, 0, st, A, Bs, C, M, N, K, ep); break;
    case 2: LCR_LAUNCH_TIMED((k_gemm_f32_bsplit_p<2, 2>), grid, block, 0, st, A, Bs, C, M, N, K, ep); break;
    case 4: LCR_LAUNCH_TIMED((k_gemm_f32_bsplit_p<4, 2>), grid, block, 0, st, A, Bs, C, M, N, K, ep); break;
    case 8: LCR_LAUNCH_TIMED((k_gemm_f32_bsplit_p<8, 2>), grid, block, 0, st, A, Bs, C, M, N, K, ep); break;
    case 16: LCR_LAUNCH_TIMED((k_gemm_f32_bsplit_p<16, 2>), grid, block, 0, st, A, Bs, C, M, N, K, ep); break;
    case 23: LCR_LAUNCH_TIMED((k_gemm_f32_bsplit_p<23, 2>), grid, block, 0, st, A, Bs, C, M, N, K, ep); break;
    case 30: LCR_LAUNCH_TIMED((k_gemm_f32_bsplit_p<30, 2>), grid, block, 0, st, A, Bs, C, M, N, K, ep); break;
    default: LCR_LAUNCH_TIMED((k_gemm_f32_bsplit_p<0, 2>), grid, block, 0, st, A, Bs, C, M, N, K, ep); break;
  }
  return check_launch("lcr_gemm_f32_bsplit");
}

extern "C" int lcr_gemm_f32_batched_ta(const float* A, const float* B, float* C, int64_t M, int N, int count, const int* k_host,
                                       const int64_t* a_off_host, const int64_t* b_off_host, const int64_t* c_off_host, void* stream) {
  if (!A || !B || !C || M <= 0 || N <= 0 || count < 1 || count > GM_MAX_BATCH || !k_host || !a_off_host || !b_off_host || !c_off_host) {
    set_error("lcr_gemm_f32_batched_ta: bad argument (count <= %d)", GM_MAX_BATCH);
    return LCR_EARG;
  }
  GemmBatch bt = {};
  bt.count = count;
  for (int i = 0; i < count; ++i) {
    bt.k[i] = k_host[i];
    bt.a_off[i] = a_off_host[i];
    bt.b_off[i] = b_off_host[i];
    bt.c_off[i] = c_off_host[i];
    if (a_off_host[i] % 4 || b_off_host[i] % 4 || k_host[i] < 1) {
      set_error("lcr_gemm_f32_batched_ta: offsets must be multiples of 4 floats and K >= 1");
      return LCR_EARG;
    }
  }
  if ((M % 4) || (N % 4)) {
    set_error("lcr_gemm_f32_batched_ta: M and N must be multiples of 4");
    return LCR_EARG;
  }
  GemmEpilogue ep{nullptr, nullptr, nullptr, 0, 0, nullptr};
  return launch_gemm<64, 64, 2, 2, true>(A, B, C, M, N,  1, 1, 0, ep, static_cast<hipStream_t>(stream), &bt);
}

extern "C" int lcr_gemm_f32_strided_batched(const float* A, const float* B, float* C, int64_t M, int N, int K, int transA, int transB,
                                            int64_t strideA, int64_t strideB, int64_t strideC, int count, void* stream) {
  if (!A || !B || !C || M <= 0 || N <= 0 || K <= 0 || count < 1 || count > 65535 || (strideA % 4) || (strideB % 4)) {
    set_error("lcr_gemm_f32_strided_batched: bad argument");
    return LCR_EARG;
  }
  const int64_t lda = transA ? M : K, ldb = transB ? K : N;
  if ((lda % 4) || (ldb % 4)) {
    set_error("lcr_gemm_f32_strided_batched: leading dimensions must be multiples of 4");
    return LCR_EARG;
  }
  GemmBatch bt = {};
  bt.count = count;
  bt.strided = 1;
  bt.k[0] = K;
  bt.a_off[0] = strideA;
  bt.b_off[0] = strideB;
  bt.c_off[0] = strideC;
  GemmEpilogue ep{nullptr, nullptr, nullptr, 0, 0, nullptr};
  static const int batch_tile = getenv("LCR_GEMM_BATCH_TILE") ? atoi(getenv("LCR_GEMM_BATCH_TILE")) : 64;
  if (batch_tile == 128 && M >= 128 && N >= 128) return launch_gemm<128, 128, 4, 1, true>(A, B, C, M, N, K, transA, transB, ep, static_cast<hipStream_t>(stream), &bt);
  static const bool batch_short = !(getenv("LCR_GEMM_BATCH_SHORT") && atoi(getenv("LCR_GEMM_BATCH_SHORT")) == 0);
  if (batch_short && K <= 256 && !transA) return launch_gemm<64, 64, 2, 2, true, true>(A, B, C, M, N, K, transA, transB, ep, static_cast<hipStream_t>(stream), &bt);
  return launch_gemm<64, 64, 2, 2, true>(A, B, C, M, N, K, transA, transB, ep, static_cast<hipStream_t>(stream), &bt);
}
```

lcr-net_amd/csrc/kpconv.hip:

```cpp
#include <algorithm>
#include <cstdlib>

#include "common.h"

namespace lcr {

constexpr int KP_K = 15;
constexpr int KP_HMAX = 128;
constexpr int KP_WAVES = 4;

struct KPoints {
  float p[KP_K][3];
};

__device__ __forceinline__ void wave_lds_sync() {
  __builtin_amdgcn_fence(__ATOMIC_RELEASE, "wavefront");
  __builtin_amdgcn_wave_barrier();
  __builtin_amdgcn_fence(__ATOMIC_ACQUIRE, "wavefront");
}

typedef float floatx4 __attribute__((ext_vector_type(4)));

struct XcdBand {
  int64_t begin, end, stride;
};
__device__ __forceinline__ XcdBand xcd_band(int64_t M, int wave_in_block, int waves_per_block) {
  const int xcd = blockIdx.x & 7, slot = blockIdx.x >> 3, nslots = gridDim.x >> 3;
  const int64_t per = (M + 7) / 8;
  XcdBand b;
  b.begin = xcd * per + static_cast<int64_t>(slot) * waves_per_block + wave_in_block;
  b.end = min(M, (xcd + 1) * per);
  b.stride = static_cast<int64_t>(nslots) * waves_per_block;
  return b;
}

template <int V> struct VecOf;
template <> struct VecOf<4> { typedef float4 type; };
template <> struct VecOf<2> { typedef float2 type; };
__device__ __forceinline__ float vget(const float4& v, int i) { return i == 0 ? v.x : i == 1 ? v.y : i == 2 ? v.z : v.w; }
__device__ __forceinline__ float vget(const float2& v, int i) { return i == 0 ? v.x : v.y; }
__device__ __forceinline__ float4 vmake(const float (&a)[4]) { return make_float4(a[0], a[1], a[2], a[3]); }
__device__ __forceinline__ float2 vmake(const float (&a)[2]) { return make_float2(a[0], a[1]); }

template <typename IdxT, int C, bool OFF32>
__global__ __launch_bounds__(KP_WAVES * 64) void k_kpconv_aggregate_vec(const float* __restrict__ s_feats, const uint8_t* __restrict__ s_pos,
                                                                        const float* __restrict__ q_pts, const float* __restrict__ s_pts,
                                                                        const IdxT* __restrict__ idx, int64_t M, int64_t Ns, int H, KPoints kp,
                                                                        float sigma, float* __restrict__ A, float* __restrict__ nn,
                                                                        const int32_t* __restrict__ order, int valid_first) {
  constexpr int V = C >= 64 ? 4 : 2;
  constexpr int NL = C / (16 * V);
  constexpr int D = NL == 1 ? 4 : 2;
  typedef typename VecOf<V>::type VecT;
  constexpr int PAD = 4 * D + 4;
  __shared__ __attribute__((aligned(16))) float4 s_rel[KP_WAVES][KP_HMAX + PAD];
  const int lane = threadIdx.x & 63, w = __builtin_amdgcn_readfirstlane(threadIdx.x >> 6);
  const int sub = lane >> 4, col = lane & 15;
  const float inv_sigma = 1.f / sigma;
  float kx = 0.f, ky = 0.f, kz = 0.f;
#pragma unroll
  for (int k = 0; k < KP_K; ++k)
    if (col == k) {
      kx = kp.p[k][0];
      ky = kp.p[k][1];
      kz = kp.p[k][2];
    }
  const XcdBand band = xcd_band(M, w, KP_WAVES);
  for (int64_t t = band.begin; t < band.end; t += band.stride) {
    const int64_t m = order ? order[t] : t;
    const float qx = q_pts[3 * m], qy = q_pts[3 * m + 1], qz = q_pts[3 * m + 2];
    int n = 0, cnt = 0;
    for (int h0 = 0; h0 < H; h0 += 64) {
      const int h = h0 + lane;
      bool ok, positive = false;
      uint64_t mk;
      if (OFF32 && sizeof(IdxT) == 4) {
        const uint32_t ju = h < H ? static_cast<uint32_t>(reinterpret_cast<const int32_t*>(idx)[static_cast<uint32_t>(m) * static_cast<uint32_t>(H) + static_cast<uint32_t>(h)])
                                  : static_cast<uint32_t>(Ns);
        ok = ju < static_cast<uint32_t>(Ns);
        mk = wave_ballot(ok);
        if (ok) {
          const int slot = n + mbcnt_lt(mk);
          const float* sp = reinterpret_cast<const float*>(reinterpret_cast<const char*>(s_pts) + ju * 12u);
          s_rel[w][slot] = make_float4(sp[0] - qx, sp[1] - qy, sp[2] - qz, __uint_as_float(ju * static_cast<uint32_t>(C * 4)));
          positive = s_pos[ju] != 0;
        }
      } else {
        int64_t j = Ns;
        if (h < H) j = static_cast<int64_t>(idx[m * H + h]);
        ok = j >= 0 && j < Ns;
        mk = wave_ballot(ok);
        if (ok) {
          const int slot = n + mbcnt_lt(mk);
          s_rel[w][slot] = make_float4(s_pts[3 * j] - qx, s_pts[3 * j + 1] - qy, s_pts[3 * j + 2] - qz,
                                       __uint_as_float(OFF32 ? static_cast<uint32_t>(j) * static_cast<uint32_t>(C * 4) : static_cast<uint32_t>(j)));
          positive = s_pos[j] != 0;
        }
      }
      n += __popcll(mk);
      cnt += __popcll(wave_ballot(positive));
      if (valid_first && mk != ~0ull) break;
    }
    if (lane < PAD) s_rel[w][n + lane] = make_float4(1e6f, 1e6f, 1e6f, __uint_as_float(0u));
    wave_lds_sync();

    floatx4 acc[NL][V];
#pragma unroll
    for (int q = 0; q < NL; ++q)
#pragma unroll
      for (int v = 0; v < V; ++v) acc[q][v] = floatx4{0.f, 0.f, 0.f, 0.f};
    const int steps = (n + 3) >> 2;
    float4 p[D];
    VecT f[D][NL];
    auto fetch = [&](int s, float4& pp, VecT (&ff)[NL]) {
      pp = s_rel[w][4 * s + sub];
      if (OFF32) {
        const uint32_t off = __float_as_uint(pp.w) + static_cast<uint32_t>(V * col * 4);
#pragma unroll
        for (int q = 0; q < NL; ++q) ff[q] = *reinterpret_cast<const VecT*>(reinterpret_cast<const char*>(s_feats) + (off + static_cast<uint32_t>(q * 16 * V * 4)));
      } else {
        const float* r = s_feats + static_cast<int64_t>(__float_as_uint(pp.w)) * C + V * col;
#pragma unroll
        for (int q = 0; q < NL; ++q) ff[q] = *reinterpret_cast<const VecT*>(r + q * 16 * V);
      }
    };
    if (n > 0) {
      auto compute = [&](int s, const float4& pp, const VecT (&ff)[NL]) {
        const float ex = pp.x - kx, ey = pp.y - ky, ez = pp.z - kz;
        const float wv = fmaxf(fmaf(-__builtin_amdgcn_sqrtf(fmaf(ez, ez, fmaf(ey, ey, ex * ex))), inv_sigma, 1.f), 0.f);
#pragma unroll
        for (int q = 0; q < NL; ++q)
#pragma unroll
          for (int v = 0; v < V; ++v) acc[q][v] = __builtin_amdgcn_mfma_f32_16x16x4f32(wv, vget(ff[q], v), acc[q][v], 0, 0, 0);
      };
#pragma unroll
      for (int d = 0; d < D; ++d) fetch(d, p[d], f[d]);
      int s0 = 0;
      for (; s0 + D <= steps; s0 += D) {
#pragma unroll
        for (int d = 0; d < D; ++d) {
          compute(s0 + d, p[d], f[d]);
          fetch(s0 + d + D, p[d], f[d]);
        }
      }
#pragma unroll
      for (int d = 0; d < D - 1; ++d)
        if (s0 + d < steps) compute(s0 + d, p[d], f[d]);
    }
    float* out = A + m * (KP_K * C) + V * col;
#pragma unroll
    for (int r = 0; r < 4; ++r) {
      const int k = 4 * sub + r;
      if (k < KP_K) {
#pragma unroll
        for (int q = 0; q < NL; ++q) {
          float a[V];
#pragma unroll
          for (int v = 0; v < V; ++v) a[v] = acc[q][v][r];
          *reinterpret_cast<VecT*>(out + k * C + q * 16 * V) = vmake(a);
        }
      }
    }
    if (lane == 0) nn[m] = static_cast<float>(cnt > 1 ? cnt : 1);
    wave_lds_sync();
  }
}

constexpr int KF_C = 32, KF_Q = 16, KF_QW = KF_Q / KP_WAVES, KF_KK = KP_K * KF_C, KF_LD = KF_KK + 4, KF_KW = KF_KK / KP_WAVES;
constexpr int KF_MAX_SEG = 64;

template <typename IdxT>
__global__ __launch_bounds__(KP_WAVES * 64, 3) void k_kpconv_fused32(const float* __restrict__ s_feats, const uint8_t* __restrict__ s_pos,
                                                                     const float* __restrict__ q_pts, const float* __restrict__ s_pts,
                                                                     const IdxT* __restrict__ idx, int64_t M, int64_t Ns, int H, KPoints kp,
                                                                     float sigma, const float* __restrict__ W, const float* __restrict__ bias,
                                                                     float* __restrict__ out, const int64_t* __restrict__ seg_len, int S,
                                                                     int groups, double* __restrict__ stats, const int32_t* __restrict__ order) {
  constexpr int C = KF_C, V = 2, D = 4;
  __shared__ __attribute__((aligned(16))) float s_D[KF_Q * KF_LD];
  __shared__ __attribute__((aligned(16))) float s_P[KP_WAVES][KF_Q][C];
  __shared__ __attribute__((aligned(16))) float4 s_rel[KP_WAVES][KP_HMAX + 8];
  __shared__ int64_t s_m[KF_Q], s_start[KF_MAX_SEG + 1];
  __shared__ float s_nn[KF_Q];
  __shared__ int s_seg[KF_Q];
  const int lane = threadIdx.x & 63, w = __builtin_amdgcn_readfirstlane(threadIdx.x >> 6);
  const int sub = lane >> 4, col = lane & 15;
  const float inv_sigma = 1.f / sigma;
  float kx = 0.f, ky = 0.f, kz = 0.f;
#pragma unroll
  for (int k = 0; k < KP_K; ++k)
    if (col == k) {
      kx = kp.p[k][0];
      ky = kp.p[k][1];
      kz = kp.p[k][2];
    }
  const bool real_k = col < KP_K;
  if (threadIdx.x == 0) {
    int64_t o = 0;
    for (int i = 0; i < S; ++i) {
      s_start[i] = o;
      o += seg_len ? seg_len[i] : M;
    }
    s_start[S] = o;
  }
  float breg[KF_KW / 4][2];
  {
    const float* wr = W + static_cast<int64_t>(KF_KW * w + (KF_KW / 4) * sub) * C + col;
#pragma unroll
    for (int st = 0; st < KF_KW / 4; ++st) {
      breg[st][0] = wr[st * C];
      breg[st][1] = wr[st * C + 16];
    }
  }
  const int eq = threadIdx.x >> 4, ec = (threadIdx.x & 15) * 2;
  const float2 bias2 = bias ? *reinterpret_cast<const float2*>(bias + ec) : make_float2(0.f, 0.f);
  int my_seg = -1;
  double rs[2] = {0.0, 0.0}, rss[2] = {0.0, 0.0};
  const int gs = stats ? C / groups : 1;
  double* rep = stats ? stats + static_cast<int64_t>(blockIdx.x % GN_REPLICAS) * S * groups * 2 : nullptr;
  auto flush_thread = [&]() {
    if (my_seg < 0 || !rep) return;
#pragma unroll
    for (int j = 0; j < 2; ++j) {
      double* d = rep + (static_cast<int64_t>(my_seg) * groups + (ec + j) / gs) * 2;
      atomicAdd(d, rs[j]);
      atomicAdd(d + 1, rss[j]);
    }
  };
  __syncthreads();

  const int xcd = blockIdx.x & 7, slot = blockIdx.x >> 3, nslots = gridDim.x >> 3;
  const int64_t per = (M + 7) / 8;
  const int64_t band_begin = xcd * per, band_end = min(M, band_begin + per);
  for (int64_t t0 = band_begin + static_cast<int64_t>(slot) * KF_Q; t0 < band_end; t0 += static_cast<int64_t>(nslots) * KF_Q) {
    for (int i = 0; i < KF_QW; ++i) {
      const int ql = w * KF_QW + i;
      const int64_t t = t0 + ql;
      if (t >= band_end) {
        if (lane == 0) s_m[ql] = -1;
        continue;
      }
      const int64_t m = order ? order[t] : t;
      const float qx = q_pts[3 * m], qy = q_pts[3 * m + 1], qz = q_pts[3 * m + 2];
      int n = 0, cnt = 0;
      for (int h0 = 0; h0 < H; h0 += 64) {
        const int h = h0 + lane;
        int64_t j = Ns;
        if (h < H) j = static_cast<int64_t>(idx[m * H + h]);
        const bool ok = j >= 0 && j < Ns;
        const uint64_t mk = wave_ballot(ok);
        bool positive = false;
        if (ok) {
          const int sl = n + mbcnt_lt(mk);
          s_rel[w][sl] = make_float4(s_pts[3 * j] - qx, s_pts[3 * j + 1] - qy, s_pts[3 * j + 2] - qz, __uint_as_float(static_cast<uint32_t>(j)));
          positive = s_pos[j] != 0;
        }
        n += __popcll(mk);
        cnt += __popcll(wave_ballot(positive));
      }
      wave_lds_sync();
      floatx4 acc[V];
#pragma unroll
      for (int v = 0; v < V; ++v) acc[v] = floatx4{0.f, 0.f, 0.f, 0.f};
      const int steps = (n + 3) >> 2;
      float4 p[D];
      float2 f[D];
      auto fetch = [&](int st, float4& pp, float2& ff) {
        const int h = 4 * st + sub;
        pp = s_rel[w][h < n ? h : n - 1];
        ff = *reinterpret_cast<const float2*>(s_feats + static_cast<int64_t>(__float_as_uint(pp.w)) * C + V * col);
      };
      if (n > 0) {
        auto compute = [&](int st, const float4& pp, const float2& ff) {
          const float ex = pp.x - kx, ey = pp.y - ky, ez = pp.z - kz;
          float wv = fmaxf(fmaf(-__builtin_amdgcn_sqrtf(fmaf(ez, ez, fmaf(ey, ey, ex * ex))), inv_sigma, 1.f), 0.f);
          wv = (real_k && 4 * st + sub < n) ? wv : 0.f;
          acc[0] = __builtin_amdgcn_mfma_f32_16x16x4f32(wv, ff.x, acc[0], 0, 0, 0);
          acc[1] = __builtin_amdgcn_mfma_f32_16x16x4f32(wv, ff.y, acc[1], 0, 0, 0);
        };
#pragma unroll
        for (int d = 0; d < D; ++d) fetch(d, p[d], f[d]);
        int s0 = 0;
        for (; s0 + D <= steps; s0 += D) {
#pragma unroll
          for (int d = 0; d < D; ++d) {
            compute(s0 + d, p[d], f[d]);
            fetch(s0 + d + D, p[d], f[d]);
          }
        }
#pragma unroll
        for (int d = 0; d < D - 1; ++d)
          if (s0 + d < steps) compute(s0 + d, p[d], f[d]);
      }
      float* drow = s_D + ql * KF_LD + V * col;
#pragma unroll
      for (int r = 0; r < 4; ++r) {
        const int k = 4 * sub + r;
        if (k < KP_K) *reinterpret_cast<float2*>(drow + k * C) = make_float2(acc[0][r], acc[1][r]);
      }
      if (lane == 0) {
        int sg = 0;
        while (sg + 1 < S && m >= s_start[sg + 1]) ++sg;
        s_m[ql] = m;
        s_nn[ql] = static_cast<float>(cnt > 1 ? cnt : 1);
        s_seg[ql] = sg;
      }
// ... 146 lines not shown
      a[15] += f > 0.f ? 1.f : 0.f;
      const float dx = px - qx, dy = py - qy, dz = pz - qz;
#pragma unroll
      for (int k = 0; k < KP_K; ++k) {
        const float ex = dx - kp.p[k][0], ey = dy - kp.p[k][1], ez = dz - kp.p[k][2];
        a[k] = fmaf(fmaxf(fmaf(-__builtin_amdgcn_sqrtf(fmaf(ez, ez, fmaf(ey, ey, ex * ex))), inv_sigma, 1.f), 0.f), f, a[k]);
      }
    };
    if (r0.j >= 0 && r0.j < Ns) add(n0.f, n0.x, n0.y, n0.z);
    for (int h = lane + 64; h < H; h += 64) {
      const int64_t j = static_cast<int64_t>(idx[m * H + h]);
      if (j >= 0 && j < Ns) add(s_feats[j], s_pts[3 * j], s_pts[3 * j + 1], s_pts[3 * j + 2]);
    }
    {
      const bool u5 = lane & 32, u4 = lane & 16, u3 = lane & 8, u2 = lane & 4;
      float b8[8], b4[4], b2[2], b1;
#pragma unroll
      for (int i = 0; i < 8; ++i) b8[i] = (u5 ? a[i + 8] : a[i]) + __shfl_xor(u5 ? a[i] : a[i + 8], 32);
#pragma unroll
      for (int i = 0; i < 4; ++i) b4[i] = (u4 ? b8[i + 4] : b8[i]) + __shfl_xor(u4 ? b8[i] : b8[i + 4], 16);
#pragma unroll
      for (int i = 0; i < 2; ++i) b2[i] = (u3 ? b4[i + 2] : b4[i]) + __shfl_xor(u3 ? b4[i] : b4[i + 2], 8);
      b1 = (u2 ? b2[1] : b2[0]) + __shfl_xor(u2 ? b2[0] : b2[1], 4);
      b1 += __shfl_xor(b1, 2);
      b1 += __shfl_xor(b1, 1);
      if ((lane & 3) == 0) s_a[w][(u5 ? 8 : 0) + (u4 ? 4 : 0) + (u3 ? 2 : 0) + (u2 ? 1 : 0)] = b1;
    }
    wave_lds_sync();
    const float cntf = s_a[w][15];
    const float div = cntf > 1.f ? cntf : 1.f;
    float av[KP_K];
#pragma unroll
    for (int k = 0; k < KP_K; ++k) av[k] = s_a[w][k];
#pragma unroll
    for (int q = 0; q < MAXO; ++q) {
      const int o = lane + 64 * q;
      if (o < Cout) {
        float v = 0.f;
#pragma unroll
        for (int k = 0; k < KP_K; ++k) v = fmaf(av[k], wreg[q][k], v);
        v = v / div;
        if (bias) v += breg[q];
        out[m * Cout + o] = v;
      }
    }
    wave_lds_sync();
    r0 = r1;
    n0 = n1;
    r1 = r2;
  }
}

template <typename IdxT>
__global__ __launch_bounds__(256) void k_maxpool(const float* __restrict__ x, const IdxT* __restrict__ idx, int64_t M, int64_t Ns, int H, int C,
                                                 float* __restrict__ out, const int32_t* __restrict__ order) {
  __shared__ int32_t s_idx[4][KP_HMAX];
  const int lane = threadIdx.x & 63, w = __builtin_amdgcn_readfirstlane(threadIdx.x >> 6);
  const XcdBand band = xcd_band(M, w, 4);
  for (int64_t t = band.begin; t < band.end; t += band.stride) {
    const int64_t m = order ? order[t] : t;
    int n = 0;
    bool any_shadow = false;
    for (int h0 = 0; h0 < H; h0 += 64) {
      const int h = h0 + lane;
      int64_t j = Ns;
      if (h < H) j = static_cast<int64_t>(idx[m * H + h]);
      const bool ok = j >= 0 && j < Ns;
      const uint64_t mk = wave_ballot(ok);
      if (ok) s_idx[w][n + mbcnt_lt(mk)] = static_cast<int32_t>(j);
      any_shadow |= (wave_ballot(h < H && !ok) != 0ull);
      n += __popcll(mk);
    }
    wave_lds_sync();
    const float init = any_shadow ? 0.f : -INFINITY;
    if ((C & 255) == 0) {
      for (int c = lane * 4; c < C; c += 256) {
        float4 v = make_float4(init, init, init, init);
        for (int h0 = 0; h0 < n; h0 += 8) {
          float4 f[8];
#pragma unroll
          for (int u = 0; u < 8; ++u)
            f[u] = *reinterpret_cast<const float4*>(x + static_cast<int64_t>(s_idx[w][h0 + u < n ? h0 + u : n - 1]) * C + c);
#pragma unroll
          for (int u = 0; u < 8; ++u) {
            v.x = fmaxf(v.x, f[u].x);
            v.y = fmaxf(v.y, f[u].y);
            v.z = fmaxf(v.z, f[u].z);
            v.w = fmaxf(v.w, f[u].w);
          }
        }
        *reinterpret_cast<float4*>(out + m * C + c) = v;
      }
    } else if ((C & 127) == 0) {
      for (int c = lane * 2; c < C; c += 128) {
        float2 v = make_float2(init, init);
        for (int h0 = 0; h0 < n; h0 += 8) {
          float2 f[8];
#pragma unroll
          for (int u = 0; u < 8; ++u)
            f[u] = *reinterpret_cast<const float2*>(x + static_cast<int64_t>(s_idx[w][h0 + u < n ? h0 + u : n - 1]) * C + c);
#pragma unroll
          for (int u = 0; u < 8; ++u) {
            v.x = fmaxf(v.x, f[u].x);
            v.y = fmaxf(v.y, f[u].y);
          }
        }
        *reinterpret_cast<float2*>(out + m * C + c) = v;
      }
    } else {
      for (int c = lane; c < C; c += 64) {
        float v = init;
        for (int h0 = 0; h0 < n; h0 += 8) {
          float f[8];
#pragma unroll
          for (int u = 0; u < 8; ++u) f[u] = x[static_cast<int64_t>(s_idx[w][h0 + u < n ? h0 + u : n - 1]) * C + c];
#pragma unroll
          for (int u = 0; u < 8; ++u) v = fmaxf(v, f[u]);
        }
        out[m * C + c] = v;
      }
    }
    wave_lds_sync();
  }
}

__global__ __launch_bounds__(256) void k_row_pos(const float* __restrict__ x, int64_t N, int C, uint8_t* __restrict__ pos) {
  const int lane = threadIdx.x & 63, w = __builtin_amdgcn_readfirstlane(threadIdx.x >> 6);
  for (int64_t n = static_cast<int64_t>(blockIdx.x) * 4 + w; n < N; n += static_cast<int64_t>(gridDim.x) * 4) {
    float s = 0.f;
    for (int c = lane; c < C; c += 64) s += x[n * C + c];
    s = wave_sum(s);
    if (lane == 0) pos[n] = s > 0.f ? 1 : 0;
  }
}

static KPoints load_kp(const float* kp_host) {
  KPoints k;
  for (int i = 0; i < KP_K; ++i)
    for (int d = 0; d < 3; ++d) k.p[i][d] = kp_host[3 * i + d];
  return k;
}

static int grid_for(int64_t rows, int per_block) { return static_cast<int>(std::min<int64_t>((rows + per_block - 1) / per_block, 256 * 16)); }
static int grid_for_xcd(int64_t rows, int per_block) {
  const int64_t per_xcd = ((rows + 7) / 8 + per_block - 1) / per_block;
  return 8 * static_cast<int>(std::max<int64_t>(1, std::min<int64_t>(per_xcd, 256 * 2)));
}

static int g_agg_force_off64 = 0;

template <typename IdxT>
static int launch_aggregate(const float* s_feats, const uint8_t* s_pos, const float* q_pts, const float* s_pts, const IdxT* idx, int64_t M,
                            int64_t Ns, int H, int C, const KPoints& kp, float sigma, float* A, float* nn, const int32_t* order, int vf,
                            hipStream_t st) {
  dim3 grid(grid_for_xcd(M, KP_WAVES)), block(KP_WAVES * 64);
  const bool off32 = Ns * C < (int64_t(1) << 30) && M * H < (int64_t(1) << 30) && !g_agg_force_off64;
#define LCR_AGG(CC)                                                                                                                          \
  if (off32) LCR_LAUNCH_TIMED((k_kpconv_aggregate_vec<IdxT, CC, true>), grid, block, 0, st, s_feats, s_pos, q_pts, s_pts, idx, M, Ns, H, kp, sigma, A, nn, order, vf); \
  else LCR_LAUNCH_TIMED((k_kpconv_aggregate_vec<IdxT, CC, false>), grid, block, 0, st, s_feats, s_pos, q_pts, s_pts, idx, M, Ns, H, kp, sigma, A, nn, order, vf);      \
  break
  switch (C) {
    case 32: LCR_AGG(32);
    case 64: LCR_AGG(64);
    case 128: LCR_AGG(128);
    case 256: LCR_AGG(256);
    default: set_error("lcr_kpconv_aggregate: C must be 32, 64, 128 or 256 (got %d)", C); return LCR_EARG;
  }
#undef LCR_AGG
  return check_launch("lcr_kpconv_aggregate");
}

}

using namespace lcr;

extern "C" void lcr_kpconv_debug_off64(int on) { g_agg_force_off64 = on; }

extern "C" int lcr_kpconv_aggregate(const float* s_feats, const uint8_t* s_pos, const float* q_pts, const float* s_pts, const void* idx,
                                    int idx_is_64, int64_t M, int64_t Ns, int H, int C, const float* kernel_points_host, float sigma,
                                    float* A, float* nn, const int32_t* order, void* stream) {
  return lcr_kpconv_aggregate_ex(s_feats, s_pos, q_pts, s_pts, idx, idx_is_64, M, Ns, H, C, kernel_points_host, sigma, A, nn, order, 0, stream);
}

extern "C" int lcr_kpconv_aggregate_ex(const float* s_feats, const uint8_t* s_pos, const float* q_pts, const float* s_pts, const void* idx,
                                       int idx_is_64, int64_t M, int64_t Ns, int H, int C, const float* kernel_points_host, float sigma,
                                       float* A, float* nn, const int32_t* order, int flags, void* stream) {
  if (!s_feats || !s_pos || !q_pts || !s_pts || !idx || !kernel_points_host || !A || !nn || M < 0 || Ns < 0 || H < 1 || H > KP_HMAX ||
      !(sigma > 0.f)) {
    set_error("lcr_kpconv_aggregate: bad argument (H must be in [1,%d])", KP_HMAX);
    return LCR_EARG;
  }
  if (M == 0) return LCR_OK;
  const KPoints kp = load_kp(kernel_points_host);
  hipStream_t st = static_cast<hipStream_t>(stream);
  KernelTimerScope timed(KT_AGGREGATE, st, M, Ns, H, C, idx_is_64 ? 8 : 4);
  const int vf = (flags & LCR_KP_VALID_FIRST) ? 1 : 0;
  return idx_is_64 ? launch_aggregate(s_feats, s_pos, q_pts, s_pts, static_cast<const int64_t*>(idx), M, Ns, H, C, kp, sigma, A, nn, order, vf, st)
                   : launch_aggregate(s_feats, s_pos, q_pts, s_pts, static_cast<const int32_t*>(idx), M, Ns, H, C, kp, sigma, A, nn, order, vf, st);
}

extern "C" int lcr_kpconv_fused(const float* s_feats, const uint8_t* s_pos, const float* q_pts, const float* s_pts, const void* idx,
                                int idx_is_64, int64_t M, int64_t Ns, int H, int C, const float* kernel_points_host, float sigma,
                                const float* W, const float* bias, float* out, const int64_t* seg_len, int S, int groups, double* stats,
                                const int32_t* order, void* stream) {
  if (!s_feats || !s_pos || !q_pts || !s_pts || !idx || !kernel_points_host || !W || !out || M < 0 || Ns < 0 || H < 1 || H > KP_HMAX ||
      !(sigma > 0.f) || C != KF_C) {
    set_error("lcr_kpconv_fused: bad argument (C must be %d, H in [1,%d])", KF_C, KP_HMAX);
    return LCR_EARG;
  }
  if (stats && (!seg_len || S < 1 || S > KF_MAX_SEG || groups < 1 || C % groups != 0)) {
    set_error("lcr_kpconv_fused: statistics need seg_len, 1 <= S <= %d and groups dividing C", KF_MAX_SEG);
    return LCR_EARG;
  }
  if (M == 0) return LCR_OK;
  const KPoints kp = load_kp(kernel_points_host);
  hipStream_t st = static_cast<hipStream_t>(stream);
  KernelTimerScope timed(KT_KPCONV_FUSED, st, M, Ns, H, C, idx_is_64 ? 8 : 4);
  static const int n_cu = [] {
    int dev = 0, cus = 0;
    if (hipGetDevice(&dev) != hipSuccess || hipDeviceGetAttribute(&cus, hipDeviceAttributeMultiprocessorCount, dev) != hipSuccess || cus <= 0)
      cus = 256;
    return cus;
  }();
  const int64_t tiles_per_band = ((M + 7) / 8 + KF_Q - 1) / KF_Q;
  const int grid = 8 * static_cast<int>(std::max<int64_t>(1, std::min<int64_t>(tiles_per_band, (3 * n_cu + 7) / 8)));
  const int Sx = stats ? S : 1;
  if (idx_is_64)
    hipLaunchKernelGGL((k_kpconv_fused32<int64_t>), dim3(grid), dim3(KP_WAVES * 64), 0, st, s_feats, s_pos, q_pts, s_pts,
                       static_cast<const int64_t*>(idx), M, Ns, H, kp, sigma, W, bias, out, stats ? seg_len : nullptr, Sx, groups, stats, order);
  else
    hipLaunchKernelGGL((k_kpconv_fused32<int32_t>), dim3(grid), dim3(KP_WAVES * 64), 0, st, s_feats, s_pos, q_pts, s_pts,
                       static_cast<const int32_t*>(idx), M, Ns, H, kp, sigma, W, bias, out, stats ? seg_len : nullptr, Sx, groups, stats, order);
  return check_launch("lcr_kpconv_fused");
}

extern "C" int lcr_kpconv_cin1(const float* s_feats, const float* q_pts, const float* s_pts, const void* idx, int idx_is_64, int64_t M,
                               int64_t Ns, int H, const float* kernel_points_host, float sigma, const float* W, const float* bias, int Cout,
                               float* out, const int32_t* order, void* stream) {
  if (!s_feats || !q_pts || !s_pts || !idx || !kernel_points_host || !W || !out || M < 0 || H < 1 || Cout < 1 || Cout > 256 || !(sigma > 0.f)) {
    set_error("lcr_kpconv_cin1: bad argument");
    return LCR_EARG;
  }
  if (M == 0) return LCR_OK;
  const KPoints kp = load_kp(kernel_points_host);
  hipStream_t st = static_cast<hipStream_t>(stream);
  dim3 grid(grid_for_xcd(M, KP_WAVES)), block(KP_WAVES * 64);
#define LCR_CIN1(IDX, MAXO) \
  hipLaunchKernelGGL((k_kpconv_cin1<IDX, MAXO>), grid, block, 0, st, s_feats, q_pts, s_pts, static_cast<const IDX*>(idx), M, Ns, H, kp, sigma, W, bias, Cout, out, order)
  if (idx_is_64) {
    if (Cout <= 64) LCR_CIN1(int64_t, 1);
    else LCR_CIN1(int64_t, 4);
  } else {
    if (Cout <= 64) LCR_CIN1(int32_t, 1);
    else LCR_CIN1(int32_t, 4);
  }
#undef LCR_CIN1
  return check_launch("lcr_kpconv_cin1");
}

extern "C" int lcr_maxpool(const float* x, const void* idx, int idx_is_64, int64_t M, int64_t Ns, int H, int C, float* out,
                           const int32_t* order, void* stream) {
  if (!x || !idx || !out || M < 0 || H < 1 || H > KP_HMAX || C < 1) {
    set_error("lcr_maxpool: bad argument");
    return LCR_EARG;
  }
  if (M == 0) return LCR_OK;
  hipStream_t st = static_cast<hipStream_t>(stream);
  dim3 grid(grid_for_xcd(M, 4)), block(256);
  if (idx_is_64) hipLaunchKernelGGL((k_maxpool<int64_t>), grid, block, 0, st, x, static_cast<const int64_t*>(idx), M, Ns, H, C, out, order);
  else hipLaunchKernelGGL((k_maxpool<int32_t>), grid, block, 0, st, x, static_cast<const int32_t*>(idx), M, Ns, H, C, out, order);
  return check_launch("lcr_maxpool");
}

extern "C" int lcr_row_positive(const float* x, int64_t N, int C, uint8_t* pos, void* stream) {
  if (!x || !pos || N < 0 || C < 1) {
    set_error("lcr_row_positive: bad argument");
    return LCR_EARG;
  }
  if (N == 0) return LCR_OK;
  hipLaunchKernelGGL(k_row_pos, dim3(grid_for(N, 4)), dim3(256), 0, static_cast<hipStream_t>(stream), x, N, C, pos);
  return check_launch("lcr_row_positive");
}
```

lcr-net_amd/functional.py:

```python
import ctypes
import os
import threading

import numpy as np
import torch

from . import _lib

GN_EPS = 1e-5
GN_REPLICAS = 8


class KernelTimer:
    KINDS = {"gemm": 0, "kpconv_aggregate": 1, "radius_query": 2, "attention": 3, "kpconv_fused": 4, "sinkhorn": 5}

    def __init__(self, names):
        self.names = set(names)
        self._cache = None

    def summary(self):
        return {k: [(b, m) for b, _, m in v] for k, v in self.records().items()}

    def records(self):
        if self._cache is None:
            out = {}
            L = _lib.lib()
            for name in self.names:
                kind = self.KINDS[name]
                n = L.lcr_ktimer_read2(kind, 0, None, None, None)
                sec = (ctypes.c_double * max(n, 1))()
                ksec = (ctypes.c_double * max(n, 1))()
                meta = (ctypes.c_int64 * (5 * max(n, 1)))()
                L.lcr_ktimer_read2(kind, n, ctypes.cast(sec, ctypes.c_void_p), ctypes.cast(ksec, ctypes.c_void_p), ctypes.cast(meta, ctypes.c_void_p))
                width = 3 if name == "gemm" else 5
                out[name] = [(sec[i], ksec[i] if ksec[i] >= 0 else None, tuple(int(meta[5 * i + k]) for k in range(width))) for i in range(n)]
            self._cache = out
        return self._cache


def set_timer(timer, sample_every=1):
    _lib.lib().lcr_ktimer_sample(int(sample_every))
    mask = 0
    for name in (timer.names if timer is not None else ()):
        mask |= 1 << KernelTimer.KINDS[name]
    _lib.lib().lcr_ktimer_kinds(mask if timer is not None else 0xffffffff)
    _lib.lib().lcr_ktimer_enable(1 if timer is not None else 0)


def _timed(name, fn, meta=None):
    return fn()


def _seg(seg_len, n, device):
    if seg_len is None:
        return torch.full((1,), int(n), dtype=torch.int64, device=device)
    return seg_len


def host_values(values, dtype, device):
    return torch.tensor(values, dtype=dtype).pin_memory().to(device, non_blocking=True)


def host_tensor(t, device):
    if not torch.is_tensor(t):
        t = torch.from_numpy(t)
    return t.pin_memory().to(device, non_blocking=True)


def _idx_args(idx):
    if idx.dtype == torch.int64:
        return 1
    if idx.dtype == torch.int32:
        return 0
    raise RuntimeError("neighbor indices must be int32 or int64")


class _StatsArena(threading.local):
    buf = None
    off = 0


_ARENA = _StatsArena()


class stats_arena:

    def __init__(self, device, entries=1 << 18):
        self.device, self.entries = device, entries

    def __enter__(self):
        self.prev = (_ARENA.buf, _ARENA.off)
        _ARENA.buf = torch.zeros(self.entries, dtype=torch.float64, device=self.device)
        _ARENA.off = 0
        return self

    def __exit__(self, *exc):
        _ARENA.buf, _ARENA.off = self.prev
        return False


def _zero_stats(S, groups, device):
    n = GN_REPLICAS * S * groups * 2
    buf = _ARENA.buf
    if buf is not None and buf.device == device and _ARENA.off + n <= buf.numel():
        v = buf[_ARENA.off:_ARENA.off + n].view(GN_REPLICAS, S, groups, 2)
        _ARENA.off += n
        return v
    return torch.zeros((GN_REPLICAS, S, groups, 2), dtype=torch.float64, device=device)


def gemm(a, b, trans_b=False, trans_a=False, bias=None, rowdiv=None, seg_len=None, groups=0):
    _lib.require_cuda(a, b)
    assert a.dtype == torch.float32 and b.dtype == torch.float32 and a.is_contiguous() and b.is_contiguous()
    M, K = (a.shape[1], a.shape[0]) if trans_a else (a.shape[0], a.shape[1])
    N = b.shape[0] if trans_b else b.shape[1]
    assert (b.shape[1] if trans_b else b.shape[0]) == K, "inner dimensions differ"
    c = torch.empty((M, N), dtype=torch.float32, device=a.device)
    stats = None
    S = 0
    if groups:
        seg_len = _seg(seg_len, M, a.device)
        S = seg_len.numel()
        stats = _zero_stats(S, groups, a.device)
    _timed("gemm", lambda: _lib.check(_lib.lib().lcr_gemm_f32(
        _lib.ptr(a), _lib.ptr(b), _lib.ptr(c), M, N, K, int(trans_a), int(trans_b), _lib.ptr(bias), _lib.ptr(rowdiv),
        _lib.ptr(seg_len) if groups else None, S, int(groups), _lib.ptr(stats), _lib.stream_ptr(a.device)), "lcr_gemm_f32"),
        meta=(M, N, K))
    return c, stats


_GEMM_SPLIT = [os.environ.get("LCR_GEMM_SPLIT", "1") not in ("", "0")]


def gemm_split_enabled():
    return _GEMM_SPLIT[0]


def set_gemm_split(on):
    _GEMM_SPLIT[0] = bool(on)


def gemm_split_ok(N, K):
    return K >= 288 and K % 32 == 0 and N >= 64


derived_lock = threading.RLock()


class WeightStamp:
    __slots__ = ("ref", "ptr", "ver", "dev")

    def __init__(self, t):
        import weakref
        self.ref, self.ptr, self.ver, self.dev = weakref.ref(t), t.data_ptr(), t._version, t.device

    def same(self, t):
        return self.ref is not None and self.ref() is t and self.ptr == t.data_ptr() and self.ver == t._version and self.dev == t.device

    def __reduce__(self):
        return (_dead_stamp, ())


def _dead_stamp():
    s = WeightStamp.__new__(WeightStamp)
    s.ref, s.ptr, s.ver, s.dev = None, 0, -1, None
    return s


def drop_derived(module, *names):
    for n in names:
        if n in module.__dict__:
            module.__dict__[n] = None



def publish_derived(t):
    torch.cuda.current_stream(t.device).synchronize()
    return t


def split_bf16x3(w):
    w = w.detach().contiguous()
    N, K = w.shape
    assert K % 32 == 0
    tiles = torch.empty(((N + 63) // 64, K // 32, 3, 64, 32), dtype=torch.int16, device=w.device)
    _lib.check(_lib.lib().lcr_split_bf16x3_tiles(_lib.ptr(w), int(N), int(K), _lib.ptr(tiles), _lib.stream_ptr(w.device)), "lcr_split_bf16x3_tiles")
    tiles.lcr_n = int(N)
    return tiles


def unsplit_bf16x3(tiles):
    CT, KS = tiles.shape[0], tiles.shape[1]
    t = tiles.view(CT, KS, 3, 64, 4, 8)
    row = torch.arange(64, device=tiles.device)
    phys = torch.arange(4, device=tiles.device)[None, :] ^ ((row >> 2) & 3)[:, None]
    t = torch.gather(t, 4, phys.view(1, 1, 1, 64, 4, 1).expand(CT, KS, 3, 64, 4, 8))
    t = t.reshape(CT, KS, 3, 64, 32).permute(2, 0, 3, 1, 4).reshape(3, CT * 64, KS * 32)
    return t[:, :tiles.lcr_n].contiguous().view(torch.bfloat16).float()


def gemm_bsplit(a, planes, bias=None, rowdiv=None, seg_len=None, groups=0):
    _lib.require_cuda(a, planes)
    assert a.dtype == torch.float32 and a.is_contiguous() and planes.dtype == torch.int16 and planes.is_contiguous() and planes.dim() == 5
    M, K = a.shape
    N = planes.lcr_n
    assert planes.shape[1] * 32 == K and planes.shape[0] == (N + 63) // 64, "inner dimensions differ"
    c = torch.empty((M, N), dtype=torch.float32, device=a.device)
    stats, S = None, 0
    if groups:
        seg_len = _seg(seg_len, M, a.device)
        S = seg_len.numel()
        stats = _zero_stats(S, groups, a.device)
    _lib.check(_lib.lib().lcr_gemm_f32_bsplit(_lib.ptr(a), _lib.ptr(planes), _lib.ptr(c), M, N, K, _lib.ptr(bias), _lib.ptr(rowdiv),
                                              _lib.ptr(seg_len) if groups else None, S, int(groups), _lib.ptr(stats), _lib.stream_ptr(a.device)),
               "lcr_gemm_f32_bsplit")
    return c, stats


ANORM_MAX_K, ANORM_MIN_SEG_ROWS = 256, 64


def gemm_anorm_ok(K, N):
    return K <= ANORM_MAX_K and K % 4 == 0 and N > 32


def gemm_anorm(a, a_stats, a_gamma, a_beta, a_groups, weight, bias=None, seg_len=None, groups=0, slope=0.1):
    _lib.require_cuda(a, weight)
    assert a.dtype == torch.float32 and weight.dtype == torch.float32 and a.is_contiguous() and weight.is_contiguous()
    M, K = a.shape
    N = weight.shape[0]
    assert weight.shape[1] == K and gemm_anorm_ok(K, N)
    c = torch.empty((M, N), dtype=torch.float32, device=a.device)
    seg_len = _seg(seg_len, M, a.device)
    S = seg_len.numel()
    stats = _zero_stats(S, groups, a.device) if groups else None
    _timed("gemm", lambda: _lib.check(_lib.lib().lcr_gemm_f32_anorm(
        _lib.ptr(a), _lib.ptr(weight), _lib.ptr(c), M, N, K, _lib.ptr(bias), _lib.ptr(a_stats), _lib.ptr(a_gamma), _lib.ptr(a_beta),
        int(a_groups), GN_EPS, float(slope), _lib.ptr(seg_len), S, int(groups), _lib.ptr(stats), _lib.stream_ptr(a.device)),
        "lcr_gemm_f32_anorm"), meta=(M, N, K))
    return c, stats


def groupnorm_stats(x, groups, seg_len=None):
    seg_len = _seg(seg_len, x.shape[0], x.device)
    stats = _zero_stats(seg_len.numel(), groups, x.device)
    _lib.check(_lib.lib().lcr_groupnorm_stats(_lib.ptr(x), x.shape[0], x.shape[1], groups, _lib.ptr(seg_len), seg_len.numel(),
                                              _lib.ptr(stats), _lib.stream_ptr(x.device)), "lcr_groupnorm_stats")
    return stats


def groupnorm_apply(x, stats, gamma, beta, groups, seg_len=None, res=None, res_norm=None, slope=0.1, act=True, want_pos=False):
    seg_len = _seg(seg_len, x.shape[0], x.device)
    y = torch.empty_like(x)
    pos = torch.empty((x.shape[0],), dtype=torch.uint8, device=x.device) if want_pos else None
    rs, rg, rb = res_norm if res_norm is not None else (None, None, None)
    _lib.check(_lib.lib().lcr_groupnorm_apply(_lib.ptr(x), _lib.ptr(stats), _lib.ptr(gamma), _lib.ptr(beta), _lib.ptr(res), _lib.ptr(rs),
                                              _lib.ptr(rg), _lib.ptr(rb), _lib.ptr(y), x.shape[0], x.shape[1], groups, _lib.ptr(seg_len),
                                              seg_len.numel(), GN_EPS, float(slope), int(act), _lib.ptr(pos),
                                              _lib.stream_ptr(x.device)), "lcr_groupnorm_apply")
    return (y, pos) if want_pos else y


def row_positive(x):
    pos = torch.empty((x.shape[0],), dtype=torch.uint8, device=x.device)
    _lib.check(_lib.lib().lcr_row_positive(_lib.ptr(x), x.shape[0], x.shape[1], _lib.ptr(pos), _lib.stream_ptr(x.device)), "lcr_row_positive")
    return pos


def _kp_host(kernel_points):
    kp = np.ascontiguousarray(kernel_points, dtype=np.float32)
    assert kp.shape == (15, 3)
    return kp


def kpconv_aggregate(s_feats, s_pos, q_points, s_points, idx, kernel_points_host, sigma, order=None):
    _lib.require_cuda(s_feats, q_points, s_points, idx)
    M, H = idx.shape
    Ns, C = s_feats.shape
    assert idx.is_contiguous() and s_feats.is_contiguous() and q_points.is_contiguous() and s_points.is_contiguous()
    A = torch.empty((M, 15 * C), dtype=torch.float32, device=s_feats.device)
    nn = torch.empty((M,), dtype=torch.float32, device=s_feats.device)
    kp = _kp_host(kernel_points_host)
    _timed("kpconv_aggregate", lambda: _lib.check(_lib.lib().lcr_kpconv_aggregate(
        _lib.ptr(s_feats), _lib.ptr(s_pos), _lib.ptr(q_points), _lib.ptr(s_points), _lib.ptr(idx), _idx_args(idx), M, Ns, H, C,
        ctypes.c_void_p(kp.ctypes.data), float(sigma), _lib.ptr(A), _lib.ptr(nn), _lib.ptr(order), _lib.stream_ptr(s_feats.device)),
        "lcr_kpconv_aggregate"), meta=(M, Ns, H, C, idx.element_size()))
    return A, nn


KPCONV_FUSED_C = 32


def kpconv_fused(s_feats, s_pos, q_points, s_points, idx, kernel_points_host, sigma, weights, bias, seg_len=None, groups=0, order=None):
    _lib.require_cuda(s_feats, q_points, s_points, idx)
    M, H = idx.shape
    Ns, C = s_feats.shape
    assert C == KPCONV_FUSED_C and tuple(weights.shape) == (15, C, C) and weights.is_contiguous()
    assert idx.is_contiguous() and s_feats.is_contiguous() and q_points.is_contiguous() and s_points.is_contiguous()
    out = torch.empty((M, C), dtype=torch.float32, device=s_feats.device)
    stats, S = None, 0
    if groups:
        seg_len = _seg(seg_len, M, s_feats.device)
        S = seg_len.numel()
        stats = _zero_stats(S, groups, s_feats.device)
    kp = _kp_host(kernel_points_host)
    _timed("kpconv_fused", lambda: _lib.check(_lib.lib().lcr_kpconv_fused(
        _lib.ptr(s_feats), _lib.ptr(s_pos), _lib.ptr(q_points), _lib.ptr(s_points), _lib.ptr(idx), _idx_args(idx), M, Ns, H, C,
        ctypes.c_void_p(kp.ctypes.data), float(sigma), _lib.ptr(weights), _lib.ptr(bias), _lib.ptr(out),
        _lib.ptr(seg_len) if groups else None, S, int(groups), _lib.ptr(stats), _lib.ptr(order), _lib.stream_ptr(s_feats.device)),
        "lcr_kpconv_fused"), meta=(M, Ns, H, C, idx.element_size()))
    return out, stats


def kpconv_cin1(s_feats, q_points, s_points, idx, kernel_points_host, sigma, weights, bias, order=None):
    M, H = idx.shape
    Ns = s_feats.shape[0]
    Cout = weights.shape[-1]
    out = torch.empty((M, Cout), dtype=torch.float32, device=s_feats.device)
    kp = _kp_host(kernel_points_host)
    _lib.check(_lib.lib().lcr_kpconv_cin1(_lib.ptr(s_feats), _lib.ptr(q_points), _lib.ptr(s_points), _lib.ptr(idx), _idx_args(idx), M, Ns, H,
                                          ctypes.c_void_p(kp.ctypes.data), float(sigma), _lib.ptr(weights), _lib.ptr(bias), Cout,
                                          _lib.ptr(out), _lib.ptr(order), _lib.stream_ptr(s_feats.device)), "lcr_kpconv_cin1")
    return out


def maxpool(x, idx, order=None):
    M, H = idx.shape
    out = torch.empty((M, x.shape[1]), dtype=torch.float32, device=x.device)
    _lib.check(_lib.lib().lcr_maxpool(_lib.ptr(x), _lib.ptr(idx), _idx_args(idx), M, x.shape[0], H, x.shape[1], _lib.ptr(out),
                                      _lib.ptr(order), _lib.stream_ptr(x.device)), "lcr_maxpool")
    return out


class NetvladWeights(ctypes.Structure):
    _fields_ = [(n, ctypes.c_void_p) for n in (
        "cluster_weights", "cluster_weights2", "hidden1_weights", "bn1_w", "bn1_b", "bn1_mean", "bn1_var",
        "bn2_w", "bn2_b", "bn2_mean", "bn2_var", "gating_weights", "gbn_w", "gbn_b", "gbn_mean", "gbn_var")]


def netvlad_forward(feats, seg_len_host, weights_struct):
    _lib.require_cuda(feats)
    seg = np.ascontiguousarray(seg_len_host, dtype=np.int64)
    S = int(seg.shape[0])
    assert int(seg.sum()) == feats.shape[0] and feats.shape[1] == 1024 and feats.is_contiguous()
    nbytes = ctypes.c_size_t(0)
    _lib.check(_lib.lib().lcr_netvlad_ws_bytes(feats.shape[0], S, ctypes.byref(nbytes)), "lcr_netvlad_ws_bytes")
    ws = _lib.workspace(nbytes.value, feats.device)
    out = torch.empty((S, 256), dtype=torch.float32, device=feats.device)
    _lib.check(_lib.lib().lcr_netvlad_forward(_lib.ptr(feats), ctypes.c_void_p(seg.ctypes.data), S, ctypes.byref(weights_struct),
                                              _lib.ptr(out), _lib.ptr(ws), ws.numel(), _lib.stream_ptr(feats.device)),
               "lcr_netvlad_forward")
    return out


def linear(x, weight, bias=None, relu=False):
    y = gemm(x.contiguous(), weight, trans_b=True, bias=bias)[0]
    if relu:
        _lib.check(_lib.lib().lcr_relu_inplace(_lib.ptr(y), y.numel(), _lib.stream_ptr(y.device)), "lcr_relu_inplace")
    return y


def relu_(x):
    _lib.check(_lib.lib().lcr_relu_inplace(_lib.ptr(x), x.numel(), _lib.stream_ptr(x.device)), "lcr_relu_inplace")
    return x


def rotary_embed_(x, theta, heads):
    assert x.is_contiguous() and theta.is_contiguous() and x.shape[1] == heads * 32 and theta.shape[1] == heads * 16
    _lib.check(_lib.lib().lcr_rotary_embed(_lib.ptr(x), _lib.ptr(theta), x.shape[0], heads, _lib.stream_ptr(x.device)), "lcr_rotary_embed")
    return x


def attention(q, k, v, heads, q_lens=None, k_lens=None):
    assert q.is_contiguous() and k.is_contiguous() and v.is_contiguous()
    out = torch.empty_like(q)
    if q_lens is not None:
        P = len(q_lens)
        assert len(k_lens) == P and sum(q_lens) == q.shape[0] and sum(k_lens) == k.shape[0]
        ql, kl = (ctypes.c_int64 * P)(*[int(x) for x in q_lens]), (ctypes.c_int64 * P)(*[int(x) for x in k_lens])
        _lib.check(_lib.lib().lcr_attention_seg_f32(_lib.ptr(q), _lib.ptr(k), _lib.ptr(v), ctypes.cast(ql, ctypes.c_void_p),
                                                    ctypes.cast(kl, ctypes.c_void_p), P, heads, q.shape[1] // heads, _lib.ptr(out),
                                                    _lib.stream_ptr(q.device)), "lcr_attention_seg_f32")
        return out
    _lib.check(_lib.lib().lcr_attention_f32(_lib.ptr(q), _lib.ptr(k), _lib.ptr(v), q.shape[0], k.shape[0], heads, q.shape[1] // heads,
                                            _lib.ptr(out), _lib.stream_ptr(q.device)), "lcr_attention_f32")
    return out


ATTENTION_TOPK_MAX_KEYS = 4096


def attention_topk(q, k, v, heads, q_lens, k_lens, kks):
    assert q.is_contiguous() and k.is_contiguous() and v.is_contiguous()
    P = len(q_lens)
    assert len(k_lens) == P and len(kks) == P and sum(q_lens) == q.shape[0] and sum(k_lens) == k.shape[0]
    out = torch.empty_like(q)
    ql, kl = (ctypes.c_int64 * P)(*[int(x) for x in q_lens]), (ctypes.c_int64 * P)(*[int(x) for x in k_lens])
    kk = (ctypes.c_int * P)(*[int(x) for x in kks])
    _lib.check(_lib.lib().lcr_attention_topk_f32(_lib.ptr(q), _lib.ptr(k), _lib.ptr(v), ctypes.cast(ql, ctypes.c_void_p), ctypes.cast(kl, ctypes.c_void_p),
                                                 ctypes.cast(kk, ctypes.c_void_p), P, heads, q.shape[1] // heads, _lib.ptr(out), _lib.stream_ptr(q.device)),
               "lcr_attention_topk_f32")
    return out


def add_layernorm(a, b, gamma, beta, eps=1e-5):
    y = torch.empty_like(a)
    _lib.check(_lib.lib().lcr_add_layernorm(_lib.ptr(a), _lib.ptr(b), _lib.ptr(gamma), _lib.ptr(beta), a.shape[0], a.shape[1], float(eps),
                                            _lib.ptr(y), _lib.stream_ptr(a.device)), "lcr_add_layernorm")
    return y


def _L():
    return _lib.lib()


def _sp(t):
    return _lib.stream_ptr(t.device)


def vote_shift(xyz, offsets, max_range):
    out = torch.empty_like(xyz)
    _lib.check(_L().lcr_vote_shift(_lib.ptr(xyz.contiguous()), _lib.ptr(offsets.contiguous()), xyz.shape[0], float(max_range), _lib.ptr(out),
                                   _sp(xyz)), "lcr_vote_shift")
    return out


def greedy_nms(points, lengths, radius):
    n, B = points.shape[0], lengths.numel()
    keep = torch.empty((n,), dtype=torch.uint8, device=points.device)
    out_len = torch.empty((B,), dtype=torch.int64, device=points.device)
    nbytes = ctypes.c_size_t(0)
    _lib.check(_L().lcr_greedy_nms_ws_bytes(n, ctypes.byref(nbytes)), "lcr_greedy_nms_ws_bytes")
    ws = _lib.workspace(nbytes.value, points.device)
    _lib.check(_L().lcr_greedy_nms(_lib.ptr(points.contiguous()), _lib.ptr(lengths), B, n, float(radius), _lib.ptr(keep), _lib.ptr(out_len),
                                   _lib.ptr(ws), _sp(points)), "lcr_greedy_nms")
# ... 289 lines not shown
```

lcr-net_amd/modules/kpconv/kpconv.py:

```python
import math
import os

import torch
import torch.nn as nn

from ... import functional as F
from ...weights import base_kernel_points


_FUSED = bool(os.environ.get("LCR_KPCONV_FUSED"))


class KPConv(nn.Module):
    def __init__(self, in_channels, out_channels, kernel_size, radius, sigma, bias=False, dimension=3, inf=1e6, eps=1e-9):
        super().__init__()
        assert kernel_size == 15 and dimension == 3, "the HIP path implements the 15-point rigid 3-D kernel of the reference config"
        self.kernel_size, self.in_channels, self.out_channels = kernel_size, in_channels, out_channels
        self.radius, self.sigma, self.dimension = radius, sigma, dimension
        self.inf, self.eps = inf, eps
        self.weights = nn.Parameter(torch.zeros(kernel_size, in_channels, out_channels))
        if bias:
            self.bias = nn.Parameter(torch.zeros(out_channels))
        else:
            self.register_parameter("bias", None)
        nn.init.kaiming_uniform_(self.weights, a=math.sqrt(5))
        if self.bias is not None:
            fan_in, _ = nn.init._calculate_fan_in_and_fan_out(self.weights)
            bound = 1 / math.sqrt(fan_in)
            nn.init.uniform_(self.bias, -bound, bound)
        self.register_buffer("kernel_points", torch.from_numpy(base_kernel_points() * radius).float())
        self._kp_cache = None
        self._wt_cache = None

    def weights_t(self):
        w = self.weights
        c = self._wt_cache
        if c is None or not c[0].same(w):
            with F.derived_lock:
                c = self._wt_cache
                if c is None or not c[0].same(w):
                    wt = w.detach().reshape(self.kernel_size * self.in_channels, self.out_channels).t().contiguous()
                    c = self._wt_cache = (F.WeightStamp(w), F.publish_derived(wt) if wt.is_cuda else wt)
        return c[1]

    def weights_t_split(self):
        wt = self.weights_t()
        c = getattr(self, "_wts_cache", None)
        if c is None or c[0] is not wt:
            with F.derived_lock:
                c = getattr(self, "_wts_cache", None)
                if c is None or c[0] is not wt:
                    c = self._wts_cache = (wt, F.publish_derived(F.split_bf16x3(wt)))
        return c[1]

    def kernel_points_host(self):
        kp = self.kernel_points
        c = self._kp_cache
        if c is None or not c[0].same(kp):
            c = self._kp_cache = (F.WeightStamp(kp), kp.detach().cpu().numpy().copy())
        return c[1]

    def _apply(self, fn, *args, **kwargs):
        F.drop_derived(self, "_kp_cache", "_wt_cache", "_wts_cache")
        return super()._apply(fn, *args, **kwargs)

    def forward_raw(self, s_feats, q_points, s_points, neighbor_indices, s_pos=None, seg_len=None, groups=0, order=None):
        kp = self.kernel_points_host()
        if self.in_channels == 1:
            out = F.kpconv_cin1(s_feats.contiguous().view(-1), q_points, s_points, neighbor_indices, kp, self.sigma,
                                self.weights, self.bias, order=order)
            stats = F.groupnorm_stats(out, groups, seg_len) if groups else None
            return out, stats
        if s_pos is None:
            s_pos = F.row_positive(s_feats)
        if (_FUSED and self.in_channels == self.out_channels == F.KPCONV_FUSED_C and neighbor_indices.shape[1] <= 128
                and (seg_len is None or seg_len.numel() <= 64)):
            return F.kpconv_fused(s_feats, s_pos, q_points, s_points, neighbor_indices, kp, self.sigma, self.weights, self.bias,
                                  seg_len=seg_len, groups=groups, order=order)
        A, nn_cnt = F.kpconv_aggregate(s_feats, s_pos, q_points, s_points, neighbor_indices, kp, self.sigma, order=order)
        wt = self.weights_t()
        if F.gemm_split_enabled() and F.gemm_split_ok(wt.shape[0], wt.shape[1]):
            return F.gemm_bsplit(A, self.weights_t_split(), bias=self.bias, rowdiv=nn_cnt, seg_len=seg_len, groups=groups)
        return F.gemm(A, wt, trans_b=True, bias=self.bias, rowdiv=nn_cnt, seg_len=seg_len, groups=groups)

    def forward(self, s_feats, q_points, s_points, neighbor_indices):
        return self.forward_raw(s_feats, q_points, s_points, neighbor_indices)[0]

    def __repr__(self):
        return (f"KPConv(kernel_size: {self.kernel_size}, in_channels: {self.in_channels}, out_channels: {self.out_channels}, "
                f"radius: {self.radius:g}, sigma: {self.sigma:g}, bias: {self.bias is not None})")
```

Before: 2883 scans/s.

## Skip zero kernel-point blocks in KPConv GEMM via per-row aggregation masks

The KPConv aggregation kernel now emits a 15-bit per-row mask marking which kernel-point blocks of the aggregated A matrix are nonzero. The deep fp32 GEMM and the bf16x3 split GEMM read that mask and replace loads of all-zero K-blocks with a shared zero buffer or an out-of-range buffer load, which cuts global memory traffic for A. The MFMA work is unchanged. This costs an extra mask write in the aggregation kernel, a per-tile branch and mask reads in the GEMMs, and extra template instantiations. A gate function decides when the masked path is used.

```diff
diff --git a/include/lcr_hip.h b/include/lcr_hip.h
--- a/include/lcr_hip.h
+++ b/include/lcr_hip.h
@@ -97,6 +97,12 @@
 int lcr_split_bf16x3_tiles(const float* w, int N, int K, uint16_t* tiles, void* stream);
 int lcr_gemm_f32_bsplit(const float* A, const uint16_t* Bs_tiles, float* C, int64_t M, int N, int K, const float* bias, const float* rowdiv,
                         const int64_t* seg_len, int S, int groups, double* stats, void* stream);
+int lcr_gemm_f32_masked(const float* A, const float* B, float* C, int64_t M, int N, int K, const float* bias, const float* rowdiv,
+                        const int64_t* seg_len, int S, int groups, double* stats, const uint16_t* row_mask, int block_k, void* stream);
+int lcr_gemm_f32_bsplit_masked(const float* A, const uint16_t* Bs_tiles, float* C, int64_t M, int N, int K, const float* bias,
+                               const float* rowdiv, const int64_t* seg_len, int S, int groups, double* stats, const uint16_t* row_mask,
+                               int block_k, void* stream);
+int lcr_kpconv_mask_ok(int64_t M, int N, int K, int split);
 int lcr_gemm_f32_anorm(const float* A, const float* B, float* C, int64_t M, int N, int K, const float* bias,
                        const double* a_stats, const float* a_gamma, const float* a_beta, int a_groups, float a_eps,
                        float a_slope, const int64_t* seg_len, int S, int groups, double* stats, void* stream);
@@ -111,6 +117,10 @@
                             const void* idx, int idx_is_64, int64_t M, int64_t Ns, int H, int C,
                             const float* kernel_points_host, float sigma, float* A, float* nn,
                             const int32_t* order, int flags, void* stream);
+int lcr_kpconv_aggregate_mask(const float* s_feats, const uint8_t* s_pos, const float* q_pts, const float* s_pts,
+                              const void* idx, int idx_is_64, int64_t M, int64_t Ns, int H, int C,
+                              const float* kernel_points_host, float sigma, float* A, float* nn, uint16_t* mask,
+                              const int32_t* order, int flags, void* stream);
 int lcr_kpconv_fused(const float* s_feats, const uint8_t* s_pos, const float* q_pts, const float* s_pts, const void* idx,
                      int idx_is_64, int64_t M, int64_t Ns, int H, int C, const float* kernel_points_host, float sigma,
                      const float* W, const float* bias, float* out, const int64_t* seg_len, int S, int groups, double* stats,
diff --git a/lcr-net_amd/_lib.py b/lcr-net_amd/_lib.py
--- a/lcr-net_amd/_lib.py
+++ b/lcr-net_amd/_lib.py
@@ -50,6 +50,8 @@
     "lcr_roformer_forward": (c_int, [c_vp, c_vp, c_vp, c_vp, c_vp, c_int, c_vp, c_vp, c_vp, c_size_t, c_vp]),
     "lcr_encoder_forward_ex": (c_int, [c_vp, c_vp, c_vp, c_vp, c_vp, c_vp, c_vp, c_int, c_vp, c_vp, c_vp, c_vp, ctypes.c_uint, c_vp, c_size_t, c_vp]),
     "lcr_kpconv_aggregate": (c_int, [c_vp, c_vp, c_vp, c_vp, c_vp, c_int, c_i64, c_i64, c_int, c_int, c_vp, c_float, c_vp, c_vp, c_vp, c_vp]),
+    "lcr_kpconv_aggregate_mask": (c_int, [c_vp, c_vp, c_vp, c_vp, c_vp, c_int, c_i64, c_i64, c_int, c_int, c_vp, c_float, c_vp, c_vp, c_vp, c_vp,
+                                          c_int, c_vp]),
     "lcr_kpconv_fused": (c_int, [c_vp, c_vp, c_vp, c_vp, c_vp, c_int, c_i64, c_i64, c_int, c_int, c_vp, c_float, c_vp, c_vp, c_vp, c_vp, c_int,
                                  c_int, c_vp, c_vp, c_vp]),
     "lcr_kpconv_cin1": (c_int, [c_vp, c_vp, c_vp, c_vp, c_int, c_i64, c_i64, c_int, c_vp, c_float, c_vp, c_vp, c_int, c_vp, c_vp, c_vp]),
@@ -82,6 +84,9 @@
     "lcr_split_bf16x3": (c_int, [c_vp, c_i64, c_vp, c_vp]),
     "lcr_split_bf16x3_tiles": (c_int, [c_vp, c_int, c_int, c_vp, c_vp]),
     "lcr_gemm_f32_bsplit": (c_int, [c_vp, c_vp, c_vp, c_i64, c_int, c_int, c_vp, c_vp, c_vp, c_int, c_int, c_vp, c_vp]),
+    "lcr_gemm_f32_bsplit_masked": (c_int, [c_vp, c_vp, c_vp, c_i64, c_int, c_int, c_vp, c_vp, c_vp, c_int, c_int, c_vp, c_vp, c_int, c_vp]),
+    "lcr_gemm_f32_masked": (c_int, [c_vp, c_vp, c_vp, c_i64, c_int, c_int, c_vp, c_vp, c_vp, c_int, c_int, c_vp, c_vp, c_int, c_vp]),
+    "lcr_kpconv_mask_ok": (c_int, [c_i64, c_int, c_int, c_int]),
     "lcr_log_sinkhorn_ex": (c_int, [c_vp, c_vp, c_vp, c_i64, c_int, c_int, c_int, c_float, c_vp, ctypes.c_size_t, c_vp]),
     "lcr_top1_matching_ws_bytes": (c_int, [c_i64, c_int, c_int, c_size_p]),
     "lcr_top1_matching": (c_int, [c_vp, c_i64, c_int, c_int, c_vp, c_vp, c_vp, c_vp, c_vp, c_vp, ctypes.c_size_t, c_vp]),
diff --git a/lcr-net_amd/csrc/encoder.hip b/lcr-net_amd/csrc/encoder.hip
--- a/lcr-net_amd/csrc/encoder.hip
+++ b/lcr-net_amd/csrc/encoder.hip
@@ -82,8 +82,9 @@
   float* A = ws.take<float>(static_cast<size_t>(M) * 15 * mid);
   float* nn = ws.take<float>(static_cast<size_t>(M));
   float* kpo = ws.take<float>(static_cast<size_t>(M) * mid);
+  uint16_t* kmask = ws.take<uint16_t>(static_cast<size_t>(M));
   double* stc = sp.take();
-  if (!A || !nn || !kpo || !stc) return LCR_ESPACE;
+  if (!A || !nn || !kpo || !kmask || !stc) return LCR_ESPACE;
   static const bool vf_env_off = getenv("LCR_KP_VALID_FIRST") && atoi(getenv("LCR_KP_VALID_FIRST")) == 0;
   const int vf_flag = ((enc_flags & LCR_ENC_LISTS_VALID_FIRST) && !vf_env_off) ? LCR_KP_VALID_FIRST : 0;
   static const bool fused32 = getenv("LCR_KPCONV_FUSED") != nullptr;
@@ -92,9 +93,17 @@
                                     stc, q.order, s))))
       return rc;
   } else {
-    if ((rc = TURN(lcr_kpconv_aggregate_ex(x, pos, q.pts, sup.pts, idx, 0, M, Ns, H, mid, b.kernel_points_host, b.sigma, A, nn, q.order, vf_flag, s)))) return rc;
-    if (b.kp_wt_split && mid >= 64) {
-      if ((rc = TURN(lcr_gemm_f32_bsplit(A, b.kp_wt_split, kpo, M, mid, 15 * mid, b.kp_b, nn, q.seg, sp.S, g, stc, s)))) return rc;
+    const bool split = b.kp_wt_split && mid >= 64;
+    if (!((split || b.kp_wt) && lcr_kpconv_mask_ok(M, mid, 15 * mid, split))) kmask = nullptr;
+    if ((rc = TURN(lcr_kpconv_aggregate_mask(x, pos, q.pts, sup.pts, idx, 0, M, Ns, H, mid, b.kernel_points_host, b.sigma, A, nn, kmask, q.order, vf_flag,
+                                             s))))
+      return rc;
+    if (split) {
+      if ((rc = TURN(kmask ? lcr_gemm_f32_bsplit_masked(A, b.kp_wt_split, kpo, M, mid, 15 * mid, b.kp_b, nn, q.seg, sp.S, g, stc, kmask, mid, s)
+                           : lcr_gemm_f32_bsplit(A, b.kp_wt_split, kpo, M, mid, 15 * mid, b.kp_b, nn, q.seg, sp.S, g, stc, s))))
+        return rc;
+    } else if (kmask) {
+      if ((rc = TURN(lcr_gemm_f32_masked(A, b.kp_wt, kpo, M, mid, 15 * mid, b.kp_b, nn, q.seg, sp.S, g, stc, kmask, mid, s)))) return rc;
     } else if ((rc = TURN(b.kp_wt ? lcr_gemm_f32(A, b.kp_wt, kpo, M, mid, 15 * mid, 0, 1, b.kp_b, nn, q.seg, sp.S, g, stc, s)
                                   : lcr_gemm_f32(A, b.kp_w, kpo, M, mid, 15 * mid, 0, 0, b.kp_b, nn, q.seg, sp.S, g, stc, s)))) return rc;
   }
@@ -144,6 +153,7 @@
   a.take<float>(static_cast<size_t>(M) * 15 * mid);
   a.take<float>(M);
   a.take<float>(static_cast<size_t>(M) * mid);
+  a.take<uint16_t>(static_cast<size_t>(M));
   a.take<float>(static_cast<size_t>(M) * mid);
   a.take<float>(static_cast<size_t>(M) * b.cout);
   a.take<float>(static_cast<size_t>(M) * b.cin);
diff --git a/lcr-net_amd/csrc/gemm_f32.hip b/lcr-net_amd/csrc/gemm_f32.hip
--- a/lcr-net_amd/csrc/gemm_f32.hip
+++ b/lcr-net_amd/csrc/gemm_f32.hip
@@ -587,9 +587,19 @@
                : "memory");
 }
 
-template <int BM, int BN, int WM, int WN>
+__device__ __forceinline__ void glds16_v(const float* addr, unsigned lds_dst) {
+  unsigned keep;
+  asm volatile("s_mov_b32 %0, m0\n\ts_mov_b32 m0, %2\n\ts_nop 0\n\tglobal_load_lds_dwordx4 %1, off\n\ts_mov_b32 m0, %0"
+               : "=&s"(keep)
+               : "v"(addr), "s"(lds_dst)
+               : "memory");
+}
+__device__ __attribute__((aligned(16))) float g_zero16[4];
+
+template <int BM, int BN, int WM, int WN, bool MASK = false>
 __global__ __launch_bounds__(GM_T, (BM == 64 ? 3 : 2)) void k_gemm_f32_deep(const float* __restrict__ A, const float* __restrict__ B, float* __restrict__ C,
-                                                            int64_t M, int N, int K, GemmEpilogue ep) {
+                                                            int64_t M, int N, int K, GemmEpilogue ep, const uint16_t* __restrict__ amask,
+                                                            int kshift) {
   static_assert(WM * WN == 4 && BM == 32 * WM && BN == 32 * WN, "one 32x32 accumulator per wavefront");
   constexpr int LA = BM / 32, LB = BN / 32, LPW = LA + LB;
   constexpr int STAGE_A = BM * 128, STAGE = (BM + BN) * 128;
@@ -606,6 +616,7 @@
   const unsigned lds_base = static_cast<unsigned>(reinterpret_cast<uintptr_t>(lds));
 
   unsigned oa[LA], ob[LB];
+  uint32_t rmask[MASK ? LA : 1];
 #pragma unroll
   for (int j = 0; j < LA; ++j) {
     const int row = (w * LA + j) * 8 + (lane >> 3);
@@ -613,6 +624,7 @@
     int64_t gr = m0 + row;
     gr = gr < M ? gr : M - 1;
     oa[j] = static_cast<unsigned>((gr * K + c * 4) * 4);
+    if constexpr (MASK) rmask[j] = amask[gr];
   }
 #pragma unroll
   for (int j = 0; j < LB; ++j) {
@@ -625,13 +637,25 @@
   const unsigned dst_a = lds_base + w * LA * 1024, dst_b = lds_base + STAGE_A + w * LB * 1024;
   const float* Ak = A;
   const float* Bk = B;
+  int kt = 0;
   auto issue_one = [&](int stage, int j) {
-    if (j < LA) glds16(Ak, oa[j], dst_a + stage * STAGE + j * 1024);
-    else glds16(Bk, ob[j - LA], dst_b + stage * STAGE + (j - LA) * 1024);
+    if (j < LA) {
+      if constexpr (MASK) {
+        const float* src = ((rmask[j] >> (kt >> kshift)) & 1u)
+                               ? reinterpret_cast<const float*>(reinterpret_cast<const char*>(A) + (oa[j] + static_cast<unsigned>(kt * GM_BK * 4)))
+                               : g_zero16;
+        glds16_v(src, dst_a + stage * STAGE + j * 1024);
+      } else {
+        glds16(Ak, oa[j], dst_a + stage * STAGE + j * 1024);
+      }
+    } else {
+      glds16(Bk, ob[j - LA], dst_b + stage * STAGE + (j - LA) * 1024);
+    }
   };
   auto advance = [&] {
     Ak += GM_BK;
     Bk += GM_BK;
+    if constexpr (MASK) ++kt;
   };
   auto issue = [&](int stage) {
 #pragma unroll
@@ -752,9 +776,13 @@
 }
 
 template <int BM, int BN, int WM, int WN>
-static int launch_gemm_deep(const float* A, const float* B, float* C, int64_t M, int N, int K, const GemmEpilogue& ep, hipStream_t st) {
+static int launch_gemm_deep(const float* A, const float* B, float* C, int64_t M, int N, int K, const GemmEpilogue& ep, hipStream_t st,
+                            const uint16_t* amask = nullptr, int kshift = 0) {
   const int mt8 = (div_up(M, BM) + 7) / 8 * 8;
-  LCR_LAUNCH_TIMED((k_gemm_f32_deep<BM, BN, WM, WN>), dim3(mt8 * div_up(N, BN)), dim3(GM_T), 0, st, A, B, C, M, N, K, ep);
+  if (amask)
+    LCR_LAUNCH_TIMED((k_gemm_f32_deep<BM, BN, WM, WN, true>), dim3(mt8 * div_up(N, BN)), dim3(GM_T), 0, st, A, B, C, M, N, K, ep, amask, kshift);
+  else
+    LCR_LAUNCH_TIMED((k_gemm_f32_deep<BM, BN, WM, WN>), dim3(mt8 * div_up(N, BN)), dim3(GM_T), 0, st, A, B, C, M, N, K, ep, amask, kshift);
   return check_launch("lcr_gemm_f32");
 }
 
@@ -808,9 +836,10 @@
   *reinterpret_cast<u32x4_t*>(dst + 8192) = p3;
 }
 
-template <int ABL, int NWM, int D = 2>
+template <int ABL, int NWM, int D = 2, bool MASK = false>
 __global__ __launch_bounds__(128 * NWM, 2) void k_gemm_f32_bsplit_p(const float* __restrict__ A, const uint16_t* __restrict__ Bs, float* __restrict__ C,
-                                                             int64_t M, int N, int K, GemmEpilogue ep) {
+                                                             int64_t M, int N, int K, GemmEpilogue ep, const uint16_t* __restrict__ amask,
+                                                             int kshift) {
   constexpr int BM = 32 * NWM, BN = 64, RS = 64, T = 128 * NWM, PLA = BM * RS, STGA = 3 * PLA, PL = 64 * RS;
   constexpr int NPB = (768 + T - 1) / T;
   constexpr int STG = 3 * PL + (NPB * T - 768) * 16;
@@ -827,12 +856,19 @@
   const int srow = threadIdx.x >> 3, spc = threadIdx.x & 7;
   const float* ap[2];
   int soff[2];
+  uint32_t aoff[2], rmask[2];
 #pragma unroll
   for (int j = 0; j < 2; ++j) {
     const int r = srow + j * (T / 8);
     int64_t ga = m0 + r;
     ga = ga < M ? ga : M - 1;
     ap[j] = A + ga * K + spc * 4;
+    if constexpr (MASK) {
+      aoff[j] = static_cast<uint32_t>((ga * K + spc * 4) * 4);
+      rmask[j] = amask[ga];
+    } else {
+      aoff[j] = rmask[j] = 0;
+    }
     soff[j] = r * RS + (((spc >> 1) ^ ((r >> 2) & 3)) << 4) + (spc & 1) * 8;
   }
   const char* bp = reinterpret_cast<const char*>(Bs) + static_cast<int64_t>(n0 / 64) * (K / GM_BK) * 12288;
@@ -851,10 +887,21 @@
   const int nk = K / GM_BK;
   f32x4_t ra[D][2];
   u32x4_t rb[D][NPB];
+  __amdgpu_buffer_rsrc_t arsrc;
+  if constexpr (MASK) arsrc = __builtin_amdgcn_make_buffer_rsrc(const_cast<float*>(A), 0, static_cast<int>(M * K * 4), 0x00020000);
   auto fetch = [&](auto st_c, int t) {
     constexpr int st = decltype(st_c)::value;
     const int tt = t < nk ? t : nk - 1;
-    ra[st][0] = *reinterpret_cast<const f32x4_t*>(ap[0] + tt * GM_BK), ra[st][1] = *reinterpret_cast<const f32x4_t*>(ap[1] + tt * GM_BK);
+    if constexpr (MASK) {
+      const int kb = tt >> kshift;
+#pragma unroll
+      for (int j = 0; j < 2; ++j) {
+        const uint32_t o = ((rmask[j] >> kb) & 1u) ? aoff[j] + static_cast<uint32_t>(tt * GM_BK * 4) : 0x80000000u;
+        ra[st][j] = __builtin_bit_cast(f32x4_t, __builtin_amdgcn_raw_buffer_load_b128(arsrc, static_cast<int>(o), 0, 0));
+      }
+    } else {
+      ra[st][0] = *reinterpret_cast<const f32x4_t*>(ap[0] + tt * GM_BK), ra[st][1] = *reinterpret_cast<const f32x4_t*>(ap[1] + tt * GM_BK);
+    }
 #pragma unroll
     for (int j = 0; j < NPB; ++j) rb[st][j] = *reinterpret_cast<const u32x4_t*>(bp + static_cast<int64_t>(tt) * 12288 + bsrc[j]);
   };
@@ -1355,8 +1402,8 @@
   return check_launch("lcr_split_bf16x3_tiles");
 }
 
-extern "C" int lcr_gemm_f32_bsplit(const float* A, const uint16_t* Bs, float* C, int64_t M, int N, int K, const float* bias, const float* rowdiv,
-                                   const int64_t* seg_len, int S, int groups, double* stats, void* stream) {
+static int bsplit_impl(const float* A, const uint16_t* Bs, float* C, int64_t M, int N, int K, const float* bias, const float* rowdiv,
+                       const int64_t* seg_len, int S, int groups, double* stats, const uint16_t* amask, int kshift, void* stream) {
   if (!A || !Bs || !C || M < 0 || N <= 0 || K <= 0 || K % GM_BK != 0 || reinterpret_cast<uintptr_t>(A) % 16 != 0 || reinterpret_cast<uintptr_t>(Bs) % 16 != 0 ||
       K < GM_BK) {
     set_error("lcr_gemm_f32_bsplit: needs K %% 32 == 0 and 16-byte aligned operands");
@@ -1373,17 +1420,76 @@
   const int mt8 = (div_up(M, 64) + 7) / 8 * 8;
   static const int abl = getenv("LCR_SPLIT_ABL") ? atoi(getenv("LCR_SPLIT_ABL")) : 0;
   const dim3 grid(mt8 * div_up(N, 64)), block(256);
+  if (amask) {
+    LCR_LAUNCH_TIMED((k_gemm_f32_bsplit_p<0, 2, 2, true>), grid, block, 0, st, A, Bs, C, M, N, K, ep, amask, kshift);
+    return check_launch("lcr_gemm_f32_bsplit_masked");
+  }
   switch (abl) {
-    case 1: LCR_LAUNCH_TIMED((k_gemm_f32_bsplit_p<1, 2>), grid, block, 0, st, A, Bs, C, M, N, K, ep); break;
-    case 2: LCR_LAUNCH_TIMED((k_gemm_f32_bsplit_p<2, 2>), grid, block, 0, st, A, Bs, C, M, N, K, ep); break;
-    case 4: LCR_LAUNCH_TIMED((k_gemm_f32_bsplit_p<4, 2>), grid, block, 0, st, A, Bs, C, M, N, K, ep); break;
-    case 8: LCR_LAUNCH_TIMED((k_gemm_f32_bsplit_p<8, 2>), grid, block, 0, st, A, Bs, C, M, N, K, ep); break;
-    case 16: LCR_LAUNCH_TIMED((k_gemm_f32_bsplit_p<16, 2>), grid, block, 0, st, A, Bs, C, M, N, K, ep); break;
-    case 23: LCR_LAUNCH_TIMED((k_gemm_f32_bsplit_p<23, 2>), grid, block, 0, st, A, Bs, C, M, N, K, ep); break;
-    case 30: LCR_LAUNCH_TIMED((k_gemm_f32_bsplit_p<30, 2>), grid, block, 0, st, A, Bs, C, M, N, K, ep); break;
-    default: LCR_LAUNCH_TIMED((k_gemm_f32_bsplit_p<0, 2>), grid, block, 0, st, A, Bs, C, M, N, K, ep); break;
+    case 1: LCR_LAUNCH_TIMED((k_gemm_f32_bsplit_p<1, 2>), grid, block, 0, st, A, Bs, C, M, N, K, ep, amask, kshift); break;
+    case 2: LCR_LAUNCH_TIMED((k_gemm_f32_bsplit_p<2, 2>), grid, block, 0, st, A, Bs, C, M, N, K, ep, amask, kshift); break;
+    case 4: LCR_LAUNCH_TIMED((k_gemm_f32_bsplit_p<4, 2>), grid, block, 0, st, A, Bs, C, M, N, K, ep, amask, kshift); break;
+    case 8: LCR_LAUNCH_TIMED((k_gemm_f32_bsplit_p<8, 2>), grid, block, 0, st, A, Bs, C, M, N, K, ep, amask, kshift); break;
+    case 16: LCR_LAUNCH_TIMED((k_gemm_f32_bsplit_p<16, 2>), grid, block, 0, st, A, Bs, C, M, N, K, ep, amask, kshift); break;
+    case 23: LCR_LAUNCH_TIMED((k_gemm_f32_bsplit_p<23, 2>), grid, block, 0, st, A, Bs, C, M, N, K, ep, amask, kshift); break;
+    case 30: LCR_LAUNCH_TIMED((k_gemm_f32_bsplit_p<30, 2>), grid, block, 0, st, A, Bs, C, M, N, K, ep, amask, kshift); break;
+    default: LCR_LAUNCH_TIMED((k_gemm_f32_bsplit_p<0, 2>), grid, block, 0, st, A, Bs, C, M, N, K, ep, amask, kshift); break;
   }
   return check_launch("lcr_gemm_f32_bsplit");
+}
+
+extern "C" int lcr_gemm_f32_bsplit(const float* A, const uint16_t* Bs, float* C, int64_t M, int N, int K, const float* bias, const float* rowdiv,
+                                   const int64_t* seg_len, int S, int groups, double* stats, void* stream) {
+  return bsplit_impl(A, Bs, C, M, N, K, bias, rowdiv, seg_len, S, groups, stats, nullptr, 0, stream);
+}
+
+static int mask_kshift(int K, int block_k) {
+  for (int s = 0; s <= 3; ++s)
+    if (block_k == (GM_BK << s)) return K <= 16 * block_k ? s : -1;
+  return -1;
+}
+
+extern "C" int lcr_gemm_f32_bsplit_masked(const float* A, const uint16_t* Bs, float* C, int64_t M, int N, int K, const float* bias,
+                                          const float* rowdiv, const int64_t* seg_len, int S, int groups, double* stats, const uint16_t* row_mask,
+                                          int block_k, void* stream) {
+  const int ks = mask_kshift(K, block_k);
+  if (!row_mask || ks < 0 || M * static_cast<int64_t>(K) >= (int64_t(1) << 29)) {
+    set_error("lcr_gemm_f32_bsplit_masked: needs a row mask, block_k = 32 << s (s <= 3) with K <= 16 block_k, and M*K < 2^29");
+    return LCR_EARG;
+  }
+  return bsplit_impl(A, Bs, C, M, N, K, bias, rowdiv, seg_len, S, groups, stats, row_mask, ks, stream);
+}
+
+extern "C" int lcr_kpconv_mask_ok(int64_t M, int N, int K, int split) {
+  static const bool off = getenv("LCR_KP_MASK") && atoi(getenv("LCR_KP_MASK")) == 0;
+  if (off || M <= 0 || N <= 0 || K % 15 != 0 || mask_kshift(K, K / 15) < 0) return 0;
+  if (split) return M * static_cast<int64_t>(K) < (int64_t(1) << 29);
+  static const int deep_env = getenv("LCR_GEMM_DEEP") ? atoi(getenv("LCR_GEMM_DEEP")) : 1;
+  const int deep_mode = g_force_deep >= 0 ? g_force_deep : deep_env;
+  const int short_k = getenv("LCR_GEMM_SHORT_K") ? atoi(getenv("LCR_GEMM_SHORT_K")) : 256;
+  const bool short_form = getenv("LCR_GEMM_NO_SHORT") == nullptr && K <= short_k;
+  return deep_mode && !g_force_tile && (deep_mode == 2 || !short_form) && M * static_cast<int64_t>(K) < (int64_t(1) << 30) &&
+         static_cast<int64_t>(N) * K < (int64_t(1) << 30);
+}
+
+extern "C" int lcr_gemm_f32_masked(const float* A, const float* B, float* C, int64_t M, int N, int K, const float* bias, const float* rowdiv,
+                                   const int64_t* seg_len, int S, int groups, double* stats, const uint16_t* row_mask, int block_k, void* stream) {
+  const int ks = mask_kshift(K, block_k);
+  if (!A || !B || !C || !row_mask || M < 0 || N <= 0 || K <= 0 || K % GM_BK != 0 || ks < 0 || M * static_cast<int64_t>(K) >= (int64_t(1) << 30) ||
+      static_cast<int64_t>(N) * K >= (int64_t(1) << 30) || reinterpret_cast<uintptr_t>(A) % 16 != 0 || reinterpret_cast<uintptr_t>(B) % 16 != 0) {
+    set_error("lcr_gemm_f32_masked: needs a row mask, block_k = 32 << s (s <= 3) with K <= 16 block_k, K %% 32 == 0, M*K and N*K < 2^30, "
+              "16-byte aligned operands");
+    return LCR_EARG;
+  }
+  if (stats && (!seg_len || S < 1 || groups < 1 || N % groups != 0 || ((N / groups) & (N / groups - 1)) != 0)) {
+    set_error("lcr_gemm_f32_masked: statistics need seg_len, S >= 1 and groups dividing N into power-of-two sized groups");
+    return LCR_EARG;
+  }
+  hipStream_t st = static_cast<hipStream_t>(stream);
+  KernelTimerScope timed(KT_GEMM, st, M, N, K);
+  if (M == 0) return LCR_OK;
+  GemmEpilogue ep{bias, rowdiv, seg_len, S, groups, stats};
+  if (N <= 32) return launch_gemm_deep<128, 32, 4, 1>(A, B, C, M, N, K, ep, st, row_mask, ks);
+  return launch_gemm_deep<64, 64, 2, 2>(A, B, C, M, N, K, ep, st, row_mask, ks);
 }
 
 extern "C" int lcr_gemm_f32_batched_ta(const float* A, const float* B, float* C, int64_t M, int N, int count, const int* k_host,
diff --git a/lcr-net_amd/csrc/kpconv.hip b/lcr-net_amd/csrc/kpconv.hip
--- a/lcr-net_amd/csrc/kpconv.hip
+++ b/lcr-net_amd/csrc/kpconv.hip
@@ -42,12 +42,13 @@
 __device__ __forceinline__ float4 vmake(const float (&a)[4]) { return make_float4(a[0], a[1], a[2], a[3]); }
 __device__ __forceinline__ float2 vmake(const float (&a)[2]) { return make_float2(a[0], a[1]); }
 
-template <typename IdxT, int C, bool OFF32>
+template <typename IdxT, int C, bool OFF32, bool MASK = false>
 __global__ __launch_bounds__(KP_WAVES * 64) void k_kpconv_aggregate_vec(const float* __restrict__ s_feats, const uint8_t* __restrict__ s_pos,
                                                                         const float* __restrict__ q_pts, const float* __restrict__ s_pts,
                                                                         const IdxT* __restrict__ idx, int64_t M, int64_t Ns, int H, KPoints kp,
                                                                         float sigma, float* __restrict__ A, float* __restrict__ nn,
-                                                                        const int32_t* __restrict__ order, int valid_first) {
+                                                                        const int32_t* __restrict__ order, int valid_first,
+                                                                        uint16_t* __restrict__ mask) {
   constexpr int V = C >= 64 ? 4 : 2;
   constexpr int NL = C / (16 * V);
   constexpr int D = NL == 1 ? 4 : 2;
@@ -147,11 +148,29 @@
       for (int d = 0; d < D - 1; ++d)
         if (s0 + d < steps) compute(s0 + d, p[d], f[d]);
     }
+    uint32_t kmask = 0x7fffu;
+    if constexpr (MASK) {
+      uint32_t bits = 0;
+#pragma unroll
+      for (int r = 0; r < 4; ++r) {
+        uint32_t o = 0;
+#pragma unroll
+        for (int q = 0; q < NL; ++q)
+#pragma unroll
+          for (int v = 0; v < V; ++v) o |= __float_as_uint(acc[q][v][r]);
+        const uint64_t b = wave_ballot((o & 0x7fffffffu) != 0u);
+#pragma unroll
+        for (int s4 = 0; s4 < 4; ++s4)
+          if ((b >> (16 * s4)) & 0xffffull) bits |= 1u << (4 * s4 + r);
+      }
+      kmask = bits & 0x7fffu;
+      if (lane == 0) mask[m] = static_cast<uint16_t>(kmask);
+    }
     float* out = A + m * (KP_K * C) + V * col;
 #pragma unroll
     for (int r = 0; r < 4; ++r) {
       const int k = 4 * sub + r;
-      if (k < KP_K) {
+      if (k < KP_K && ((kmask >> k) & 1u)) {
 #pragma unroll
         for (int q = 0; q < NL; ++q) {
           float a[V];
@@ -604,12 +623,17 @@
 template <typename IdxT>
 static int launch_aggregate(const float* s_feats, const uint8_t* s_pos, const float* q_pts, const float* s_pts, const IdxT* idx, int64_t M,
                             int64_t Ns, int H, int C, const KPoints& kp, float sigma, float* A, float* nn, const int32_t* order, int vf,
-                            hipStream_t st) {
+                            uint16_t* mask, hipStream_t st) {
   dim3 grid(grid_for_xcd(M, KP_WAVES)), block(KP_WAVES * 64);
   const bool off32 = Ns * C < (int64_t(1) << 30) && M * H < (int64_t(1) << 30) && !g_agg_force_off64;
-#define LCR_AGG(CC)                                                                                                                          \
-  if (off32) LCR_LAUNCH_TIMED((k_kpconv_aggregate_vec<IdxT, CC, true>), grid, block, 0, st, s_feats, s_pos, q_pts, s_pts, idx, M, Ns, H, kp, sigma, A, nn, order, vf); \
-  else LCR_LAUNCH_TIMED((k_kpconv_aggregate_vec<IdxT, CC, false>), grid, block, 0, st, s_feats, s_pos, q_pts, s_pts, idx, M, Ns, H, kp, sigma, A, nn, order, vf);      \
+#define LCR_AGG_M(CC, O32, MK) \
+  LCR_LAUNCH_TIMED((k_kpconv_aggregate_vec<IdxT, CC, O32, MK>), grid, block, 0, st, s_feats, s_pos, q_pts, s_pts, idx, M, Ns, H, kp, sigma, A, nn, order, vf, mask)
+#define LCR_AGG(CC)                            \
+  if (mask) {                                  \
+    if (off32) LCR_AGG_M(CC, true, true);      \
+    else LCR_AGG_M(CC, false, true);           \
+  } else if (off32) LCR_AGG_M(CC, true, false); \
+  else LCR_AGG_M(CC, false, false);            \
   break
   switch (C) {
     case 32: LCR_AGG(32);
@@ -619,6 +643,7 @@
     default: set_error("lcr_kpconv_aggregate: C must be 32, 64, 128 or 256 (got %d)", C); return LCR_EARG;
   }
 #undef LCR_AGG
+#undef LCR_AGG_M
   return check_launch("lcr_kpconv_aggregate");
 }
 
@@ -637,6 +662,13 @@
 extern "C" int lcr_kpconv_aggregate_ex(const float* s_feats, const uint8_t* s_pos, const float* q_pts, const float* s_pts, const void* idx,
                                        int idx_is_64, int64_t M, int64_t Ns, int H, int C, const float* kernel_points_host, float sigma,
                                        float* A, float* nn, const int32_t* order, int flags, void* stream) {
+  return lcr_kpconv_aggregate_mask(s_feats, s_pos, q_pts, s_pts, idx, idx_is_64, M, Ns, H, C, kernel_points_host, sigma, A, nn, nullptr, order, flags,
+                                   stream);
+}
+
+extern "C" int lcr_kpconv_aggregate_mask(const float* s_feats, const uint8_t* s_pos, const float* q_pts, const float* s_pts, const void* idx,
+                                         int idx_is_64, int64_t M, int64_t Ns, int H, int C, const float* kernel_points_host, float sigma,
+                                         float* A, float* nn, uint16_t* mask, const int32_t* order, int flags, void* stream) {
   if (!s_feats || !s_pos || !q_pts || !s_pts || !idx || !kernel_points_host || !A || !nn || M < 0 || Ns < 0 || H < 1 || H > KP_HMAX ||
       !(sigma > 0.f)) {
     set_error("lcr_kpconv_aggregate: bad argument (H must be in [1,%d])", KP_HMAX);
@@ -647,8 +679,8 @@
   hipStream_t st = static_cast<hipStream_t>(stream);
   KernelTimerScope timed(KT_AGGREGATE, st, M, Ns, H, C, idx_is_64 ? 8 : 4);
   const int vf = (flags & LCR_KP_VALID_FIRST) ? 1 : 0;
-  return idx_is_64 ? launch_aggregate(s_feats, s_pos, q_pts, s_pts, static_cast<const int64_t*>(idx), M, Ns, H, C, kp, sigma, A, nn, order, vf, st)
-                   : launch_aggregate(s_feats, s_pos, q_pts, s_pts, static_cast<const int32_t*>(idx), M, Ns, H, C, kp, sigma, A, nn, order, vf, st);
+  return idx_is_64 ? launch_aggregate(s_feats, s_pos, q_pts, s_pts, static_cast<const int64_t*>(idx), M, Ns, H, C, kp, sigma, A, nn, order, vf, mask, st)
+                   : launch_aggregate(s_feats, s_pos, q_pts, s_pts, static_cast<const int32_t*>(idx), M, Ns, H, C, kp, sigma, A, nn, order, vf, mask, st);
 }
 
 extern "C" int lcr_kpconv_fused(const float* s_feats, const uint8_t* s_pos, const float* q_pts, const float* s_pts, const void* idx,
diff --git a/lcr-net_amd/functional.py b/lcr-net_amd/functional.py
--- a/lcr-net_amd/functional.py
+++ b/lcr-net_amd/functional.py
@@ -109,7 +109,9 @@
     return torch.zeros((GN_REPLICAS, S, groups, 2), dtype=torch.float64, device=device)
 
 
-def gemm(a, b, trans_b=False, trans_a=False, bias=None, rowdiv=None, seg_len=None, groups=0):
+def gemm(a, b, trans_b=False, trans_a=False, bias=None, rowdiv=None, seg_len=None, groups=0, row_mask=None):
+    if row_mask is not None:
+        return _gemm_masked(a, b, trans_b, trans_a, bias, rowdiv, seg_len, groups, row_mask)
     _lib.require_cuda(a, b)
     assert a.dtype == torch.float32 and b.dtype == torch.float32 and a.is_contiguous() and b.is_contiguous()
     M, K = (a.shape[1], a.shape[0]) if trans_a else (a.shape[0], a.shape[1])
@@ -129,6 +131,37 @@
     return c, stats
 
 
+def kpconv_mask_ok(M, N, K, split):
+    return bool(_lib.lib().lcr_kpconv_mask_ok(int(M), int(N), int(K), int(bool(split))))
+
+
+def _mask_args(a, row_mask):
+    M, K = a.shape
+    assert row_mask.dtype == torch.int16 and row_mask.is_contiguous() and row_mask.numel() == M and row_mask.device == a.device
+    assert K % 15 == 0
+    return K // 15
+
+
+def _gemm_masked(a, b, trans_b, trans_a, bias, rowdiv, seg_len, groups, row_mask):
+    _lib.require_cuda(a, b)
+    assert trans_b and not trans_a, "the masked form takes A [M,K] and B [N,K]"
+    assert a.dtype == torch.float32 and b.dtype == torch.float32 and a.is_contiguous() and b.is_contiguous()
+    block_k = _mask_args(a, row_mask)
+    M, K = a.shape
+    N = b.shape[0]
+    assert b.shape[1] == K, "inner dimensions differ"
+    c = torch.empty((M, N), dtype=torch.float32, device=a.device)
+    stats, S = None, 0
+    if groups:
+        seg_len = _seg(seg_len, M, a.device)
+        S = seg_len.numel()
+        stats = _zero_stats(S, groups, a.device)
+    _timed("gemm", lambda: _lib.check(_lib.lib().lcr_gemm_f32_masked(
+        _lib.ptr(a), _lib.ptr(b), _lib.ptr(c), M, N, K, _lib.ptr(bias), _lib.ptr(rowdiv), _lib.ptr(seg_len) if groups else None, S,
+        int(groups), _lib.ptr(stats), _lib.ptr(row_mask), block_k, _lib.stream_ptr(a.device)), "lcr_gemm_f32_masked"), meta=(M, N, K))
+    return c, stats
+
+
 _GEMM_SPLIT = [os.environ.get("LCR_GEMM_SPLIT", "1") not in ("", "0")]
 
 
@@ -199,7 +232,7 @@
     return t[:, :tiles.lcr_n].contiguous().view(torch.bfloat16).float()
 
 
-def gemm_bsplit(a, planes, bias=None, rowdiv=None, seg_len=None, groups=0):
+def gemm_bsplit(a, planes, bias=None, rowdiv=None, seg_len=None, groups=0, row_mask=None):
     _lib.require_cuda(a, planes)
     assert a.dtype == torch.float32 and a.is_contiguous() and planes.dtype == torch.int16 and planes.is_contiguous() and planes.dim() == 5
     M, K = a.shape
@@ -211,6 +244,12 @@
         seg_len = _seg(seg_len, M, a.device)
         S = seg_len.numel()
         stats = _zero_stats(S, groups, a.device)
+    if row_mask is not None:
+        block_k = _mask_args(a, row_mask)
+        _lib.check(_lib.lib().lcr_gemm_f32_bsplit_masked(_lib.ptr(a), _lib.ptr(planes), _lib.ptr(c), M, N, K, _lib.ptr(bias), _lib.ptr(rowdiv),
+                                                         _lib.ptr(seg_len) if groups else None, S, int(groups), _lib.ptr(stats),
+                                                         _lib.ptr(row_mask), block_k, _lib.stream_ptr(a.device)), "lcr_gemm_f32_bsplit_masked")
+        return c, stats
     _lib.check(_lib.lib().lcr_gemm_f32_bsplit(_lib.ptr(a), _lib.ptr(planes), _lib.ptr(c), M, N, K, _lib.ptr(bias), _lib.ptr(rowdiv),
                                               _lib.ptr(seg_len) if groups else None, S, int(groups), _lib.ptr(stats), _lib.stream_ptr(a.device)),
                "lcr_gemm_f32_bsplit")
@@ -273,7 +312,7 @@
     return kp
 
 
-def kpconv_aggregate(s_feats, s_pos, q_points, s_points, idx, kernel_points_host, sigma, order=None):
+def kpconv_aggregate(s_feats, s_pos, q_points, s_points, idx, kernel_points_host, sigma, order=None, emit_mask=False):
     _lib.require_cuda(s_feats, q_points, s_points, idx)
     M, H = idx.shape
     Ns, C = s_feats.shape
@@ -281,6 +320,13 @@
     A = torch.empty((M, 15 * C), dtype=torch.float32, device=s_feats.device)
     nn = torch.empty((M,), dtype=torch.float32, device=s_feats.device)
     kp = _kp_host(kernel_points_host)
+    if emit_mask:
+        mask = torch.empty((M,), dtype=torch.int16, device=s_feats.device)
+        _timed("kpconv_aggregate", lambda: _lib.check(_lib.lib().lcr_kpconv_aggregate_mask(
+            _lib.ptr(s_feats), _lib.ptr(s_pos), _lib.ptr(q_points), _lib.ptr(s_points), _lib.ptr(idx), _idx_args(idx), M, Ns, H, C,
+            ctypes.c_void_p(kp.ctypes.data), float(sigma), _lib.ptr(A), _lib.ptr(nn), _lib.ptr(mask), _lib.ptr(order), 0,
+            _lib.stream_ptr(s_feats.device)), "lcr_kpconv_aggregate_mask"), meta=(M, Ns, H, C, idx.element_size()))
+        return A, nn, mask
     _timed("kpconv_aggregate", lambda: _lib.check(_lib.lib().lcr_kpconv_aggregate(
         _lib.ptr(s_feats), _lib.ptr(s_pos), _lib.ptr(q_points), _lib.ptr(s_points), _lib.ptr(idx), _idx_args(idx), M, Ns, H, C,
         ctypes.c_void_p(kp.ctypes.data), float(sigma), _lib.ptr(A), _lib.ptr(nn), _lib.ptr(order), _lib.stream_ptr(s_feats.device)),
diff --git a/lcr-net_amd/modules/kpconv/kpconv.py b/lcr-net_amd/modules/kpconv/kpconv.py
--- a/lcr-net_amd/modules/kpconv/kpconv.py
+++ b/lcr-net_amd/modules/kpconv/kpconv.py
@@ -77,11 +77,16 @@
                 and (seg_len is None or seg_len.numel() <= 64)):
             return F.kpconv_fused(s_feats, s_pos, q_points, s_points, neighbor_indices, kp, self.sigma, self.weights, self.bias,
                                   seg_len=seg_len, groups=groups, order=order)
-        A, nn_cnt = F.kpconv_aggregate(s_feats, s_pos, q_points, s_points, neighbor_indices, kp, self.sigma, order=order)
         wt = self.weights_t()
-        if F.gemm_split_enabled() and F.gemm_split_ok(wt.shape[0], wt.shape[1]):
-            return F.gemm_bsplit(A, self.weights_t_split(), bias=self.bias, rowdiv=nn_cnt, seg_len=seg_len, groups=groups)
-        return F.gemm(A, wt, trans_b=True, bias=self.bias, rowdiv=nn_cnt, seg_len=seg_len, groups=groups)
+        split = F.gemm_split_enabled() and F.gemm_split_ok(wt.shape[0], wt.shape[1])
+        M = neighbor_indices.shape[0]
+        if F.kpconv_mask_ok(M, wt.shape[0], wt.shape[1], split):
+            A, nn_cnt, mask = F.kpconv_aggregate(s_feats, s_pos, q_points, s_points, neighbor_indices, kp, self.sigma, order=order, emit_mask=True)
+        else:
+            (A, nn_cnt), mask = F.kpconv_aggregate(s_feats, s_pos, q_points, s_points, neighbor_indices, kp, self.sigma, order=order), None
+        if split:
+            return F.gemm_bsplit(A, self.weights_t_split(), bias=self.bias, rowdiv=nn_cnt, seg_len=seg_len, groups=groups, row_mask=mask)
+        return F.gemm(A, wt, trans_b=True, bias=self.bias, rowdiv=nn_cnt, seg_len=seg_len, groups=groups, row_mask=mask)
 
     def forward(self, s_feats, q_points, s_points, neighbor_indices):
         return self.forward_raw(s_feats, q_points, s_points, neighbor_indices)[0]
```

Measured after the change: 2997 scans/s, median of 6. 3.9% higher.
